# kcat/openal-soft

Hardware: AMD Instinct MI355X
Metric: mixed voices/sec @48kHz 1024-sample update, HRTF stereo; fraction of HBM roofline (higher is better)
Workload: dtype f32

## Files before the change

### include/oalgpu.h

```cpp
#ifndef OALGPU_H
#define OALGPU_H

#include <stddef.h>
#include <stdint.h>

#ifdef __cplusplus
extern "C" {
#endif
#if defined(__GNUC__)
#pragma GCC visibility push(default)
#endif

#define OALGPU_BUFFER_LINE_SIZE 1024
#define OALGPU_MAX_RESAMPLER_PADDING 48
#define OALGPU_MAX_RESAMPLER_EDGE 24
#define OALGPU_HRTF_HISTORY_LENGTH 64
#define OALGPU_HRIR_LENGTH 128
#define OALGPU_MAX_SENDS 6
#define OALGPU_MAX_OUTPUT_CHANNELS 32
#define OALGPU_MAX_AMBI_CHANNELS 25
#define OALGPU_MIXER_FRAC_BITS 16

typedef enum oalgpu_error {
    OALGPU_OK = 0,
// ... 23 lines not shown
typedef enum oalgpu_biquad_type {
    OALGPU_BIQUAD_HIGHSHELF, OALGPU_BIQUAD_LOWSHELF, OALGPU_BIQUAD_PEAKING, OALGPU_BIQUAD_LOWPASS,
    OALGPU_BIQUAD_HIGHPASS, OALGPU_BIQUAD_BANDPASS
} oalgpu_biquad_type;

typedef enum oalgpu_math_mode { OALGPU_MATH_EXACT = 0, OALGPU_MATH_FAST = 1 } oalgpu_math_mode;

const char *oalgpu_version(void);
const char *oalgpu_last_error(void);
int oalgpu_device_count(void);

typedef struct oalgpu_bsinc_table {
    float scaleBase, scaleRange;
    uint32_t m[16];
    uint32_t filterOffset[16];
    const float *tab;
    size_t tablen;
} oalgpu_bsinc_table;
int oalgpu_bsinc_table_get(int which , oalgpu_bsinc_table *out);
int oalgpu_cubic_table_get(int which , float *out);

typedef struct oalgpu_interp_state {
    int32_t kind;
    int32_t table;
    float sf;
    uint32_t m, l;
    uint32_t filter_offset;
} oalgpu_interp_state;
int oalgpu_prepare_resampler(int resampler, uint32_t increment, oalgpu_interp_state *out);

typedef struct oalgpu_biquad {
    float z1, z2;
    float b0, b1, b2, a1, a2;
    float tb0, tb1, tb2, ta1, ta2;
    int32_t counter;
} oalgpu_biquad;
void oalgpu_biquad_reset(oalgpu_biquad *f);
void oalgpu_biquad_set_params_from_slope(oalgpu_biquad *f, int type, float f0norm, float gain,
    float slope);

int oalgpu_resample(int device, int mode, int resampler, uint32_t increment, const float *src,
    size_t srclen, uint32_t frac, float *dst, size_t n);
int oalgpu_mix(int device, const float *in, size_t n, float *out, size_t nlines,
    float *current_gains, const float *target_gains, size_t counter, size_t outpos);
int oalgpu_mix_hrtf(int device, int mode, const float *in, float *accum, uint32_t irsize,
    const float *coeffs, const uint32_t delay[2], float gain, float gainstep, size_t n);
int oalgpu_mix_hrtf_blend(int device, int mode, const float *in, float *accum, uint32_t irsize,
    const float *oldcoeffs, const uint32_t olddelay[2], float oldgain, const float *newcoeffs,
    const uint32_t newdelay[2], float newgainstep, size_t n);
typedef struct oalgpu_splitter { float coeff, lp_z1, lp_z2, ap_z1; } oalgpu_splitter;
void oalgpu_splitter_init(oalgpu_splitter *s, float f0norm);
int oalgpu_mix_direct_hrtf(int device, int mode, float *left, float *right, const float *in,
    size_t nch, float *accum, oalgpu_splitter *splitters, const float *hfscales,
    const float *chan_coeffs, size_t irsize, size_t n);
int oalgpu_biquad_dual_process(int device, oalgpu_biquad *f0, oalgpu_biquad *f1, const float *src,
    float *dst, size_t n);

typedef struct oalgpu_context oalgpu_context;

typedef struct oalgpu_context_desc {
    int32_t  device;
    int32_t  math_mode;
    uint32_t sample_rate;
    uint32_t num_dry_channels;
    uint32_t num_real_channels;
    uint32_t num_aux_sends;
    uint32_t num_slots;
    uint32_t wet_channels;
    int32_t  hrtf;
    uint32_t max_voices;
    uint32_t max_buffers;
    uint32_t voices_per_group;
    uint32_t flags;
} oalgpu_context_desc;
#define OALGPU_CTX_FIR_VALU 1u
#define OALGPU_CTX_PROFILE  2u
#define OALGPU_CTX_STREAM_ROWS 8u
#define OALGPU_CTX_APPLY_IN_VOICE_KERNEL 16u
#define OALGPU_CTX_FUSED_REDUCE 32u
#define OALGPU_CTX_RESIDENT 64u
#define OALGPU_CTX_SLICE_LINES 128u
#define OALGPU_CTX_WAVE_PAIRS 256u
#define OALGPU_CTX_ROW_SLICES 512u
#define OALGPU_CTX_SERIAL   4u

int  oalgpu_context_create(const oalgpu_context_desc *desc, oalgpu_context **out);
void oalgpu_context_destroy(oalgpu_context *ctx);

int oalgpu_hrtf_load_mhr(oalgpu_context *ctx, const void *data, size_t size);
int oalgpu_hrtf_load_store(oalgpu_context *ctx, uint32_t sample_rate, uint32_t ir_size, const float *field_distance,
    const uint8_t *field_evcount, uint32_t num_fields, const uint16_t *elev_azcount, const uint16_t *elev_iroffset,
    uint32_t num_elevs, const float *coeffs, const uint8_t *delays, uint32_t num_irs);
typedef struct oalgpu_hrtf_info {
    uint32_t sample_rate, ir_size, num_fields, num_elevs, num_irs;
} oalgpu_hrtf_info;
int oalgpu_hrtf_info_get(oalgpu_context *ctx, oalgpu_hrtf_info *out);
int oalgpu_hrtf_raw(oalgpu_context *ctx, float *field_distance, uint8_t *field_evcount,
    uint16_t *elev_azcount, uint16_t *elev_iroffset, float *coeffs, uint8_t *delays);
int oalgpu_hrtf_get_coeffs(oalgpu_context *ctx, const float *dirs, size_t count, float *coeffs,
    uint32_t *delays);
int oalgpu_set_direct_hrtf(oalgpu_context *ctx, const float *chan_coeffs ,
    const float *hfscales, float xover_norm, uint32_t irsize);
int oalgpu_set_direct_hrtf_from_store(oalgpu_context *ctx, const float *points, const float *matrix, uint32_t num_points,
    const float *order_hf_gain, float xover_freq, uint32_t ir_size, int per_hrir_min);
int oalgpu_hrtf_parse_host(const void *mhr, size_t size, uint32_t device_rate, oalgpu_hrtf_info *info, float *coeffs, uint8_t *delays);
int oalgpu_hrtf_blend_host(const void *mhr, size_t size, uint32_t device_rate, const float *dirs, size_t count,
    uint32_t *idx, float *w, float *pass, uint32_t *delays);
int oalgpu_hrtf_build_direct_host(const void *mhr, size_t size, uint32_t device_rate, uint32_t ir_size, int per_hrir_min,
    const float *points, const float *matrix, uint32_t num_points, uint32_t num_chans, float xover_freq, const float *order_hf_gain,
    float *out_coeffs, float *out_hfscales, float *out_xover_norm, uint32_t *out_irsize);

int oalgpu_buffer_register(oalgpu_context *ctx, const void *data, int fmt_type,
    uint32_t frame_step, uint32_t sample_len, uint32_t loop_start, uint32_t loop_end);
int oalgpu_buffer_release(oalgpu_context *ctx, int buffer);
int oalgpu_buffer_info(oalgpu_context *ctx, int buffer, int32_t *live, int32_t *release_pending, uint32_t *references);

int oalgpu_buffer_channel_view(oalgpu_context *ctx, int buffer, uint32_t channel);

typedef struct oalgpu_voice_desc {
    int32_t  buffer;
    int32_t  looping;
    int32_t  position;
    uint32_t position_frac;
    uint32_t frequency;
} oalgpu_voice_desc;
int oalgpu_voice_init(oalgpu_context *ctx, uint32_t voice, const oalgpu_voice_desc *desc);
int oalgpu_context_set_nfc(oalgpu_context *ctx, float w1, const uint32_t channels_per_order[5]);
int oalgpu_voice_set_nfc(oalgpu_context *ctx, uint32_t voice, float w0);

int oalgpu_voice_set_ambi_scale(oalgpu_context *ctx, uint32_t voice, float xover_norm, float hf_scale,
    float lf_scale);

typedef struct oalgpu_filter_params {
    int32_t active;
    float gain_hf, hf_norm;
    float gain_lf, lf_norm;
} oalgpu_filter_params;

typedef struct oalgpu_voice_params {
    uint32_t step;
    int32_t  resampler;
    oalgpu_filter_params direct_filter;
    float    dry_gains[OALGPU_MAX_OUTPUT_CHANNELS];
    float    hrtf_ev, hrtf_az, hrtf_dist, hrtf_spread;
    float    hrtf_gain;
    int32_t  send_slot[OALGPU_MAX_SENDS];
    oalgpu_filter_params send_filter[OALGPU_MAX_SENDS];
    float    send_gains[OALGPU_MAX_SENDS][OALGPU_MAX_AMBI_CHANNELS];
} oalgpu_voice_params;
#define OALGPU_HRTF_KEEP_TARGET (-1.0f)
int oalgpu_voice_set_hrtf_targets(oalgpu_context *ctx, const uint32_t *voices, const float *coeffs, const uint32_t *delays,
    const float *gains, size_t count);

typedef struct oalgpu_voice_pan {
    float dir[3];
    float spread;
    float dry_gain;
    float send_gain[OALGPU_MAX_SENDS];
} oalgpu_voice_pan;
int oalgpu_context_set_ambi_map(oalgpu_context *ctx, const uint8_t *index, const float *scale);
int oalgpu_slot_set_ambi_map(oalgpu_context *ctx, uint32_t slot, const uint8_t *index, const float *scale);
int oalgpu_voice_set_pan(oalgpu_context *ctx, const uint32_t *voices, const oalgpu_voice_pan *pans, size_t count);

int oalgpu_buffer_queue_link(oalgpu_context *ctx, int buffer, int next_buffer);
int oalgpu_voice_init_queue(oalgpu_context *ctx, uint32_t voice, int first_buffer, int looping, int32_t position,
    uint32_t position_frac);
// ... 288 lines not shown
```

### openal-soft_amd/csrc/api.hip

```cpp
#include "api_context.hpp"
namespace oalgpu {

thread_local std::string gLastError;

int Fail(int code, const std::string &msg)
{
    gLastError = msg;
    return code;
}

void ParkResidentContexts(int device);

int UseDevice(int device)
{
    int count = 0;
    if(hipGetDeviceCount(&count) != hipSuccess || count <= 0)
        return Fail(OALGPU_ERR_NO_DEVICE, "no HIP device available (the product has no CPU path)");
    if(device < 0 || device >= count) return Fail(OALGPU_ERR_INVALID, "device ordinal out of range");
    HIP_TRY(hipSetDevice(device));
    ParkResidentContexts(device);
    return OALGPU_OK;
}

}
// ... 54 lines not shown
        cb.state = OALGPU_VOICE_STOPPED;
        cb.retired = true;
        c->cbOfVoice[voice] = -1;
    }
}

void NoteCallbackSteps(oalgpu_context *c, const uint32_t *voices, const oalgpu_voice_params *params, size_t count)
{
    if(c->cbVoices.empty()) return;
    for(size_t i = 0; i < count; ++i)
        if(voices[i] < c->cbOfVoice.size() && c->cbOfVoice[voices[i]] >= 0)
            c->cbVoices[size_t(c->cbOfVoice[voices[i]])].step = params[i].step;
}

int FlushInits(oalgpu_context *c)
{
    if(c->initPending.empty()) return OALGPU_OK;
    const size_t n = c->initPending.size();
    if(int rc = StageRecords(c->stream, c->initDev, c->initPending.data(), n)) return rc;
    LaunchInitVoices(c->stream, c->L, c->initDev.p, uint32_t(n));
    HIP_TRY(hipGetLastError());
    HIP_TRY(hipStreamSynchronize(c->stream));
    c->initPending.clear();
    return OALGPU_OK;
}

static void SetRowsGroups(oalgpu_context *c);

uint32_t DeviceComputeUnits(int device)
{
    hipDeviceProp_t prop{};
    if(hipGetDeviceProperties(&prop, device) == hipSuccess && prop.multiProcessorCount > 0) return uint32_t(prop.multiProcessorCount);
    (void)hipGetLastError();
    return 256u;
}

int oalgpu_context_create(const oalgpu_context_desc *desc, oalgpu_context **out)
{
    if(!desc || !out) return Fail(OALGPU_ERR_INVALID, "null argument");
    *out = nullptr;
    if(desc->max_voices == 0 || desc->num_dry_channels == 0 || desc->num_dry_channels > OALGPU_MAX_OUTPUT_CHANNELS
        || desc->num_aux_sends > OALGPU_MAX_SENDS || desc->wet_channels > OALGPU_MAX_AMBI_CHANNELS
        || (desc->num_aux_sends && (desc->num_slots == 0 || desc->wet_channels == 0)))
        return Fail(OALGPU_ERR_INVALID, "oalgpu_context_create: bad descriptor");
    const uint32_t mixLines = (desc->hrtf ? 0u : desc->num_dry_channels) + desc->num_slots * desc->wet_channels;
    if(mixLines > 32) return Fail(OALGPU_ERR_CAPACITY, "more than 32 mixing lines (dry + wet) are not supported yet");
    if(int rc = UseDevice(desc->device)) return rc;

    auto c = std::make_unique<oalgpu_context>();
    c->desc = *desc;
    c->exact = desc->math_mode == OALGPU_MATH_EXACT;
    int prioLeast = 0, prioGreatest = 0;
    HIP_TRY(hipDeviceGetStreamPriorityRange(&prioLeast, &prioGreatest));
    HIP_TRY(hipStreamCreateWithPriority(&c->stream, hipStreamDefault, prioGreatest));
    HIP_TRY(hipEventCreate(&c->evStart)); HIP_TRY(hipEventCreate(&c->evVoice)); HIP_TRY(hipEventCreate(&c->evEnd));
    HIP_TRY(hipStreamCreateWithPriority(&c->postStream, hipStreamDefault, prioLeast));
    for(hipEvent_t *e : {&c->evVoiceDone[0], &c->evVoiceDone[1], &c->evReduceDone[0], &c->evReduceDone[1], &c->evPostDone})
        HIP_TRY(hipEventCreateWithFlags(e, hipEventDisableTiming | hipEventDisableSystemFence));

    DeviceLayout &L = c->L;
    L.numVoices = desc->max_voices;
    L.numDry = desc->num_dry_channels; L.numReal = desc->num_real_channels;
    L.numSends = desc->num_aux_sends; L.numSlots = desc->num_slots; L.wetChannels = desc->wet_channels;
    L.hrtf = desc->hrtf ? 1u : 0u;
    L.irSize = 0; L.irStride = 8;
    L.mixLines = mixLines;
    c->slotConv.assign(desc->num_slots, nullptr);
    c->slotReverb.assign(desc->num_slots, nullptr);
    c->slotEffect.assign(desc->num_slots, nullptr);
    c->slotTarget.assign(desc->num_slots, -1);
    c->slotDepth.assign(desc->num_slots, 0u);
    c->slotOrder.resize(desc->num_slots);
    for(uint32_t i = 0; i < desc->num_slots; ++i) c->slotOrder[i] = i;
    HIP_TRY(c->reverbTicket.alloc(1)); HIP_TRY(c->reverbTicket.zero());
    uint32_t vpg = desc->voices_per_group;
    if(vpg == 0)
    {
        vpg = std::max<uint32_t>(2u, (desc->max_voices + 1023u) / 1024u);
    }
    L.voicesPerGroup = vpg;
    L.numGroups = std::max<uint32_t>(1u, (desc->max_voices + vpg - 1u) / vpg);
    L.waveVoices = 0;
    L.firMfma = (desc->flags & OALGPU_CTX_FIR_VALU) ? 0u : 1u;
    c->serialOnly = (desc->flags & OALGPU_CTX_SERIAL) != 0;
    c->res.enabled = (desc->flags & OALGPU_CTX_RESIDENT) != 0 && !(desc->flags & (OALGPU_CTX_PROFILE | OALGPU_CTX_SERIAL));
    c->useWave = WaveKernelApplies(c->exact, L);
    if(c->useWave)
    {
        L.waveVoices = desc->voices_per_group ? std::max<uint32_t>(1u, (desc->voices_per_group + 3u) / 4u)
            : std::max<uint32_t>(1u, (desc->max_voices + 2047u) / 2048u);
        L.numGroups = std::max<uint32_t>(1u, WaveKernelGroups(L));
    }
    const TableBlob &blob = Blob();
    HIP_TRY(c->tables.alloc(blob.data.size())); HIP_TRY(c->tables.upload(blob.data.data(), blob.data.size()));
    L.tables = c->tables.p;
    HIP_TRY(c->buffers.alloc(std::max<uint32_t>(desc->max_buffers, 1u))); HIP_TRY(c->buffers.zero());
    L.buffers = c->buffers.p;
    c->buf.reset(desc->max_buffers, desc->max_voices);
    c->cbOfVoice.assign(std::max<uint32_t>(desc->max_voices, 1u), -1);

    const size_t nv = desc->max_voices;
    HIP_TRY(c->ctl.alloc(nv)); HIP_TRY(c->ctl.zero()); L.ctl = c->ctl.p;
    HIP_TRY(c->prev.alloc(nv * kMaxPad)); HIP_TRY(c->prev.zero()); L.prev = c->prev.p;
    HIP_TRY(c->dfilt.alloc(nv * 2)); HIP_TRY(c->dfilt.zero()); L.dfilt = c->dfilt.p;
    HIP_TRY(c->hist.alloc(nv * kHist)); HIP_TRY(c->hist.zero()); L.hist = c->hist.p;
    HIP_TRY(c->gainCur.alloc(nv * L.numDry)); HIP_TRY(c->gainCur.zero()); L.gainCur = c->gainCur.p;
    HIP_TRY(c->gainTgt.alloc(nv * L.numDry)); HIP_TRY(c->gainTgt.zero()); L.gainTgt = c->gainTgt.p;
    HIP_TRY(c->sfilt.alloc(nv * L.numSends * 2)); HIP_TRY(c->sfilt.zero()); L.sfilt = c->sfilt.p;
    HIP_TRY(c->sendCur.alloc(nv * L.numSends * L.wetChannels)); HIP_TRY(c->sendCur.zero()); L.sendCur = c->sendCur.p;
    HIP_TRY(c->sendTgt.alloc(nv * L.numSends * L.wetChannels)); HIP_TRY(c->sendTgt.zero()); L.sendTgt = c->sendTgt.p;
    HIP_TRY(c->ambi.alloc(nv)); HIP_TRY(c->ambi.zero()); L.ambi = c->ambi.p;
    HIP_TRY(c->startDelay.alloc(nv)); HIP_TRY(c->startDelay.zero()); L.startDelay = c->startDelay.p;
    {
        std::vector<AmbiMapEntry> ident(std::max<size_t>(L.numDry, size_t{L.numSlots} * L.wetChannels) + 1);
        for(size_t i = 0; i < ident.size(); ++i) ident[i] = AmbiMapEntry{uint32_t(i < OALGPU_MAX_AMBI_CHANNELS ? i : 0), 1.0f};
        HIP_TRY(c->dryMap.alloc(L.numDry)); HIP_TRY(c->dryMap.upload(ident.data(), L.numDry));
        HIP_TRY(c->wetMaps.alloc(size_t{L.numSlots} * L.wetChannels));
        for(uint32_t s = 0; s < L.numSlots; ++s)
            HIP_TRY(hipMemcpy(c->wetMaps.p + size_t{s} * L.wetChannels, ident.data(), L.wetChannels * sizeof(AmbiMapEntry), hipMemcpyHostToDevice));
    }
    HIP_TRY(c->queueDone.alloc(nv)); HIP_TRY(c->queueDone.zero()); L.queueDone = c->queueDone.p;
    L.numLineGroups = L.numGroups;
    c->groupsAllocated = L.numGroups;
    if(c->useWave && L.hrtf && L.firMfma && !(desc->flags & OALGPU_CTX_WAVE_PAIRS))
    {
        const uint32_t w = Wave16WavesFor(desc->max_voices, DeviceComputeUnits(desc->device));
        c->groupsAllocated = std::max<uint32_t>(c->groupsAllocated, (desc->max_voices + w - 1u) / w);
    }
    L.streams = nullptr; L.lineGains = nullptr; L.lineStride = 0; L.streamsPerVoice = 0;
    L.nfc = nullptr; L.nfcOrders = 0;
    L.hrirs = nullptr;
    for(uint32_t &n : L.chansPerOrder) n = 0;
    L.accLines = 0;
    L.wave16 = 0;
    L.rows8 = 0; L.rowsVpg = 0;
    if(c->useWave && !(desc->flags & OALGPU_CTX_STREAM_ROWS))
    {
        L.accLines = WaveKernelAccLines(L);
        if(!L.accLines && RowsKernelApplies(L))
            L.rows8 = 1;
    }
    if(c->useWave && (!L.hrtf || L.numSends))
    {
        L.lineStride = L.mixLines <= 8 ? 8u : (L.mixLines <= 16 ? 16u : 32u);
        L.streamsPerVoice = 2u + L.numSends;
    }
    if(c->useWave && (!L.hrtf || L.numSends) && !L.accLines && !L.rows8) { if(int rc = AllocStreamRows(c.get())) return rc; }
    const size_t groups = c->groupsAllocated;
    HIP_TRY(c->partLines.alloc(groups * L.mixLines * kLine)); L.partLines = c->partLines.p;
    HIP_TRY(c->partLines2.alloc(c->useWave && (L.streams || L.accLines || L.rows8) ? groups * L.mixLines * kLine : 0));
    c->partLinesBuf[0] = c->partLines.p; c->partLinesBuf[1] = c->partLines2.p;
    HIP_TRY(c->partHrtf.alloc(L.hrtf ? groups * (kLine + kHrirLen) * 2 : 0)); L.partHrtf = c->partHrtf.p;
    HIP_TRY(c->partHrtf2.alloc(c->useWave && L.hrtf ? groups * (kLine + kHrirLen) * 2 : 0));
    c->partHrtfBuf[0] = c->partHrtf.p; c->partHrtfBuf[1] = c->partHrtf2.p;
    HIP_TRY(c->bus.alloc(BusFloats(L))); HIP_TRY(c->bus.zero()); L.bus = c->bus.p;
    if(desc->flags & OALGPU_CTX_PROFILE)
    {
        HIP_TRY(c->phaseTimes.alloc(nv * 16)); HIP_TRY(c->phaseTimes.zero());
        c->prof.times = c->phaseTimes.p;
    }
    L.hrtfOld = nullptr; L.hrtfTgt = nullptr;

    HIP_TRY(c->dSplit.alloc(L.numDry)); HIP_TRY(c->dSplit.zero());
    HIP_TRY(c->dSplit2.alloc(L.numDry)); HIP_TRY(c->dSplit2.zero());
    HIP_TRY(c->carryBuf.alloc(size_t{kLine + kHrirLen} * 2)); HIP_TRY(c->carryBuf.zero());
    HIP_TRY(c->postArrived.alloc(1)); HIP_TRY(c->postArrived.zero());
    HIP_TRY(c->dHfScale.alloc(L.numDry)); HIP_TRY(c->dHfScale.zero());
    HIP_TRY(c->dCoeffs.alloc(size_t{L.numDry} * kHrirLen * 2)); HIP_TRY(c->dCoeffs.zero());
    HIP_TRY(c->dTemp.alloc(size_t{L.numDry} * kLine + (kLine + kHrirLen) * 2));
    if(L.rows8) SetRowsGroups(c.get());
    *out = c.release();
    return OALGPU_OK;
}

static void DetachForDestroy(oalgpu_context *ctx);

void oalgpu_context_destroy(oalgpu_context *ctx)
{
    if(!ctx) return;
    (void)UseDevice(ctx->desc.device);
    if(ctx->attachedTo || !ctx->attached.empty()) DetachForDestroy(ctx);
    if(ctx->res.pendingBlock) { ctx->res.pendingBlock->heldBy = nullptr; ctx->res.pendingBlock = nullptr; }
    (void)FlushPendingMix(ctx);
    (void)hipStreamSynchronize(ctx->stream);
    if(ctx->res.reduceStream) (void)hipStreamSynchronize(ctx->res.reduceStream);
    if(ctx->postStream) (void)hipStreamSynchronize(ctx->postStream);
    delete ctx->comm;
    for(auto &cb : ctx->cbVoices)
        for(int k = 0; k < 2; ++k)
        {
            if(cb.pinned[k]) (void)hipHostFree(cb.pinned[k]);
            if(cb.copied[k]) (void)hipEventDestroy(cb.copied[k]);
        }
    delete ctx;
}

int AllocStreamRows(oalgpu_context *c)
{
    DeviceLayout &L = c->L;
    const size_t nv = L.numVoices;
    HIP_TRY(c->streams.alloc(nv * L.streamsPerVoice * kLine)); HIP_TRY(c->streams.zero()); L.streams = c->streams.p;
    HIP_TRY(c->lineGains.alloc(nv * L.streamsPerVoice * LineBlockDwords(L.lineStride))); HIP_TRY(c->lineGains.zero());
    L.lineGains = c->lineGains.p;
    return OALGPU_OK;
}

static float *SlotWetBus(const DeviceLayout &L, uint32_t slot) { return L.bus + BusWetOffset(L) + size_t{slot} * L.wetChannels * kLine; }
static float *SlotDestination(const oalgpu_context *c, uint32_t slot)
{
    const int32_t target = c->slotTarget[slot];
    return target >= 0 ? SlotWetBus(c->L, uint32_t(target)) : c->L.bus;
}
static int RunEffects(oalgpu_context *c, hipStream_t s, uint32_t samples_to_do)
{
    const DeviceLayout &L = c->L;
    for(uint32_t first = 0; first < L.numSlots; )
    {
        const uint32_t depth = c->slotDepth[c->slotOrder[first]];
        uint32_t last = first;
        while(last < L.numSlots && c->slotDepth[c->slotOrder[last]] == depth) ++last;
        for(uint32_t i = first; i < last; ++i)
        {
            const uint32_t slot = c->slotOrder[i];
            const float *wet = SlotWetBus(L, slot);
            if(oalgpu_convolution *conv = c->slotConv[slot])
            {
                if(int rc = oalgpu_convolution_process_device(conv, s, wet, SlotDestination(c, slot), samples_to_do)) return rc;
            }
            if(oalgpu_effect *fx = c->slotEffect[slot])
            {
                if(int rc = oalgpu_effect_process_device(fx, s, wet, SlotDestination(c, slot), samples_to_do)) return rc;
            }
        }
        oalgpu_reverb *revs[kRvBatchMax];
        const float *wets[kRvBatchMax];
        float *outs[kRvBatchMax];
        uint32_t count = 0;
        auto flush = [&]() -> int
        {
            if(!count) return OALGPU_OK;
            const int rc = oalgpu_reverb_process_batch_device(revs, wets, count, outs, samples_to_do, s, c->reverbTicket.p);
            count = 0;
            return rc;
        };
// ... 926 lines not shown
```

### openal-soft_amd/csrc/api_context.hpp

```cpp
#pragma once
#include "../../include/oalgpu.h"
#ifdef OALGPU_MEASUREMENT
#include "../../tools/measure/oalgpu_measure.h"
#endif

#include <hip/hip_runtime.h>
#include <hip/hip_ext.h>
#include <rccl/rccl.h>
#include <dlfcn.h>
#include <fcntl.h>
#include <sys/mman.h>
#include <sys/stat.h>
#include <unistd.h>

#include <algorithm>
#include <atomic>
#include <chrono>
#include <functional>
#include <thread>
#include <cstdio>
#include <cstdlib>
#include <cstring>
#include <memory>
#include <mutex>
// ... 38 lines not shown
    }
    uint32_t filterBase(const oalgpu_interp_state &st) const
    {
        switch(st.kind)
        {
        case 2: return cubicBase[st.table ? 1 : 0];
        case 3: case 4: return bsincBase[st.table == 12 ? 0 : st.table == 24 ? 1 : 2] + st.filter_offset;
        default: return 0;
        }
    }
};
inline const TableBlob &Blob() { static const TableBlob b; return b; }

}

enum class PostKind : uint32_t { None, AmbiDec, Stabilizer, Bs2b, Uhj, Tsme };

struct BusTransport;
struct oalgpu_context {
    oalgpu_context_desc desc{};
    bool exact{true};
    hipStream_t stream{nullptr};
    bool ownStream{true};
    hipEvent_t evStart{nullptr}, evVoice{nullptr}, evEnd{nullptr};
    hipStream_t postStream{nullptr};
    hipEvent_t evVoiceDone[2]{nullptr, nullptr}, evReduceDone[2]{nullptr, nullptr}, evPostDone{nullptr};
    uint32_t parity{0};
    bool postPending{false};
    struct { bool active{false}; uint32_t samples{0}; int post{0}; } pendingMix;
    static constexpr uint32_t kIoSlots = 4;
    oalgpu_voice_move *panHost[kIoSlots]{};
    size_t panCap{0};
    hipEvent_t panApplied[kIoSlots]{};
    uint32_t panNext{0};
    float *outHost[kIoSlots]{};
    hipEvent_t outDone[kIoSlots]{};
    uint32_t outNext{0};
    size_t outFloats{0};
    bool panInBar{false};
    static constexpr uint32_t kEvCap = 1024;
    uint32_t *evHost[kIoSlots]{};
    hipEvent_t evDone[kIoSlots]{};
    uint32_t evNext{0};
    DevBuf<uint32_t> evSnapshot, evCounters;
    bool outRing{false}, outRingWritten{false};
    bool outViaRing[kIoSlots]{};
    uint32_t outSeq{0}, outSlotSeq[kIoSlots]{};
    uint32_t outArrivedTotal{0};
    bool fuseReduce{false}, reduceHeld{false};
    DeviceLayout heldL{};
    uint32_t heldParity{0};
    DevBuf<uint32_t> reducedCount;
    uint32_t reducedEpoch{0};
    hipEvent_t lastPostEvent{nullptr};
    uint64_t updatesSubmitted{0}, updatesKnownDone{0};
    uint64_t reduceUpdate[2]{0, 0}, panUpdate[kIoSlots]{}, outUpdate[kIoSlots]{};
    uint32_t *outFlags{nullptr};
    DevBuf<uint32_t> outArrived;
    float *partHrtfBuf[2]{nullptr, nullptr};
    float *partLinesBuf[2]{nullptr, nullptr};
    bool timing{false}, timed{false};
    DeviceLayout L{};
    HrtfStoreDev hrtfDev{};
    HrtfData hrtfHost;
    bool hrtfLoaded{false};
    uint32_t hrtfGeneration{0};
    bool carryAccum{true};
    bool useWave{false};
    uint32_t groupsAllocated{0};
    std::vector<oalgpu_convolution*> slotConv;
    std::vector<oalgpu_reverb*> slotReverb;
    std::vector<oalgpu_effect*> slotEffect;
    DevBuf<uint32_t> reverbTicket;
    std::vector<int32_t> slotTarget;
    std::vector<uint32_t> slotOrder, slotDepth;

    DevBuf<float> tables;
    DevBuf<BufferItem> buffers;
    DevBuf<uint32_t> startDelay;
    DevBuf<uint32_t> queueDone;
    BufferTable buf;
    DevBuf<VoiceCtl> ctl;
    DevBuf<float> prev, hrtfOld, hrtfTgt, hist, gainCur, gainTgt, sendCur, sendTgt;
    DevBuf<BiquadSlot> dfilt, sfilt;
    DevBuf<float> partLines, partLines2, partHrtf, partHrtf2, bus, streams;
    DevBuf<uint32_t> lineGains;
    DevBuf<AmbiScaleState> ambi;
    DevBuf<NfcState> nfc;
    NfcDesign nfcDevice{};
    DevBuf<unsigned long long> phaseTimes;
    WaveProf prof{nullptr, 0u};
    const WaveProf *profArg() const { return prof.times ? &prof : nullptr; }
    DevBuf<AmbiMapEntry> dryMap, wetMaps;
    DevBuf<PanRecord> panRecs;
    std::vector<VoiceCtl> ctlHost;
    std::vector<uint32_t> doneHost;
    DevBuf<TargetRecord> tgtRecs;
    DevBuf<float> tgtCoeffs;
    bool serialOnly{false};
    struct BusTransport *comm{nullptr};
    int commRank{0}, commWorld{1};
    oalgpu_context *attachedTo{nullptr};
    std::vector<int32_t> attachMap;
    hipEvent_t evBusFinal{nullptr};
    std::vector<oalgpu_context*> attached;
    DevBuf<BusMergeHead> mergeHeads;
    DevBuf<BusMergeRow> mergeRows;
    uint32_t mergeLines{0};
    hipEvent_t evMerged{nullptr};
    bool mergeInFlight{false};
    PostKind post{PostKind::None};
    bool decDual{false};
    uint32_t decOut{0};
    DevBuf<float> decGainsHf, decGainsLf, decBands;
    DevBuf<SplitterState> decSplit;
    int outType{6};
    float ditherDepth{0.0f};
    uint32_t ditherSeed{22222};
    bool limOn{false};
    LimiterConsts lim{};
    DevBuf<float> limState;
    int encQuality{-1};
    DevBuf<float> encTaps, encState;
    uint32_t stabLeft{0}, stabRight{0}, stabCenter{0};
    StabilizerConsts stab{};
    DevBuf<float> stabState;
    uint32_t cfLeft{0}, cfRight{0};
    CrossfeedConsts cf{};
    DevBuf<float> cfState;
    uint32_t distLines{0};
    DevBuf<uint32_t> distDelays;
    DevBuf<float> distGains, distHist;
    DevBuf<unsigned char> pcm;
    DevBuf<float> hFieldDist, hCoeffs;
    DevBuf<uint8_t> hEvCount, hDelays;
    DevBuf<uint16_t> hAzCount, hIrOffset;
    DevBuf<SplitterState> dSplit, dSplit2;
    uint32_t dSplitCur{0};
    DevBuf<float> carryBuf;
    float dSplitCoeff{0.0f};
    float runPower[4]{1.0f, 0.0f, 1.0f, 1.0f};
    uint32_t runPowerSeg{0};
    DevBuf<uint32_t> postArrived;
    uint32_t postEpoch{0};
    const ParamRecord *nextRecs{nullptr};
    const int32_t *nextMap{nullptr};
    const float *nextRows{nullptr};
    bool carryInBuf{false};
    DevBuf<float> dHfScale, dCoeffs, dTemp;
    uint32_t dIrSize{0};
    bool directSet{false};
    DevBuf<ParamRecord> paramDev;
    std::vector<ParamRecord> paramHost;
    DevBuf<VoiceInitRecord> initDev;
    std::vector<VoiceInitRecord> initPending;
    struct CbVoice {
        uint32_t voice{0}; int32_t buffer{-1}; uint32_t frameBytes{4}, capacityFrames{0};
        oalgpu_callback_fn fn{nullptr}; void *user{nullptr};
        std::vector<char> data;
        uint32_t numBlocks{0}, blockOffset{0};
        bool stopped{false};
        int32_t position{0}; uint32_t frac{0}, step{0};
        int state{OALGPU_VOICE_PLAYING}; bool hasBuffer{true};
        char *pinned[2]{nullptr, nullptr}; hipEvent_t copied[2]{nullptr, nullptr}; uint32_t slot{0};
        size_t allocBytes{0};
        bool retired{false};
// ... 115 lines not shown
```

### openal-soft_amd/csrc/api_hrtf.hip

```cpp
#include "api_context.hpp"

static uint32_t ChooseWave16(const oalgpu_context *c, const DeviceLayout &T)
{
    const bool want16 = !(c->desc.flags & OALGPU_CTX_WAVE_PAIRS) && Wave16Applies(T)
        && (T.numSends == 0 || !(c->desc.flags & (OALGPU_CTX_STREAM_ROWS | OALGPU_CTX_PROFILE)));
    if(!want16) return 0u;
    if(!c->desc.voices_per_group) return Wave16WavesFor(T.numVoices, DeviceComputeUnits(c->desc.device));
    for(uint32_t w : {4u, 8u, 16u})
        if((T.numVoices + w - 1u) / w <= c->groupsAllocated) return w;
    return 0u;
}

static int InstallHrtfData(oalgpu_context *c, HrtfData &&parsed)
{
    if(parsed.sampleRate != c->desc.sample_rate) ResampleHrtfData(parsed, c->desc.sample_rate);
    DeviceLayout T = c->L;
    T.irSize = parsed.irSize;
    T.irStride = (parsed.irSize + 15u) & ~15u;
    const bool toStreamRows = T.accLines && WaveKernelAccLines(T) == 0;
    if(toStreamRows) T.accLines = 0;
    if(c->useWave)
    {
        T.wave16 = ChooseWave16(c, T);
        if(std::max<uint32_t>(1u, WaveKernelGroups(T)) > c->groupsAllocated)
            return Fail(OALGPU_ERR_INVALID, "internal: the voice kernel's grid outgrew the partial buses");
    }
    if(int rc = oalgpu_sync(c)) return rc;
    c->hrtfHost = std::move(parsed);
    const HrtfData &h = c->hrtfHost;
    HIP_TRY(c->hFieldDist.alloc(h.fieldDistance.size())); HIP_TRY(c->hFieldDist.upload(h.fieldDistance.data(), h.fieldDistance.size()));
    HIP_TRY(c->hEvCount.alloc(h.fieldEvCount.size())); HIP_TRY(c->hEvCount.upload(h.fieldEvCount.data(), h.fieldEvCount.size()));
    HIP_TRY(c->hAzCount.alloc(h.elevAzCount.size())); HIP_TRY(c->hAzCount.upload(h.elevAzCount.data(), h.elevAzCount.size()));
    HIP_TRY(c->hIrOffset.alloc(h.elevIrOffset.size())); HIP_TRY(c->hIrOffset.upload(h.elevIrOffset.data(), h.elevIrOffset.size()));
    HIP_TRY(c->hCoeffs.alloc(h.coeffs.size())); HIP_TRY(c->hCoeffs.upload(h.coeffs.data(), h.coeffs.size()));
    HIP_TRY(c->hDelays.alloc(h.delays.size())); HIP_TRY(c->hDelays.upload(h.delays.data(), h.delays.size()));
    HrtfStoreDev &d = c->hrtfDev;
    d.irSize = h.irSize; d.numFields = uint32_t(h.fieldDistance.size()); d.numElevs = uint32_t(h.elevAzCount.size());
    d.numIrs = h.numIrs();
    d.fieldDistance = c->hFieldDist.p; d.fieldEvCount = c->hEvCount.p; d.elevAzCount = c->hAzCount.p;
    d.elevIrOffset = c->hIrOffset.p; d.coeffs = c->hCoeffs.p; d.delays = c->hDelays.p;
    c->hrtfLoaded = true;
    ++c->hrtfGeneration;

    DeviceLayout &L = c->L;
    L.hrirs = c->hCoeffs.p;
    L.irSize = h.irSize;
    L.irStride = T.irStride;
    if(L.hrtf)
    {
        const size_t n = size_t{L.numVoices} * L.irStride * 2;
        HIP_TRY(c->hrtfOld.alloc(n)); HIP_TRY(c->hrtfOld.zero()); L.hrtfOld = c->hrtfOld.p;
        HIP_TRY(c->hrtfTgt.alloc(n)); HIP_TRY(c->hrtfTgt.zero()); L.hrtfTgt = c->hrtfTgt.p;
        if(!c->directSet) c->dIrSize = h.irSize;
    }
    if(toStreamRows)
    {
        L.accLines = 0;
        if(int rc = AllocStreamRows(c)) return rc;
    }
    if(c->useWave)
    {
        L.wave16 = T.wave16;
        if(L.wave16 && L.numSends)
        {
            L.accLines = 0;
            if(!L.streams) { if(int rc = AllocStreamRows(c)) return rc; }
        }
        const uint32_t groups = std::max<uint32_t>(1u, WaveKernelGroups(L));
        L.numGroups = groups; L.numLineGroups = groups;
        if(L.wave16 && (L.wave16 != 16u || L.numSends)) c->res.enabled = false;
    }
    return OALGPU_OK;
}

int oalgpu_hrtf_load_mhr(oalgpu_context *c, const void *data, size_t size)
{
    if(!c || !data) return Fail(OALGPU_ERR_INVALID, "null argument");
    if(int rc = UseCtx(c)) return rc;
    HrtfData parsed;
    const std::string err = ParseMhr(data, size, parsed);
    if(!err.empty()) return Fail(OALGPU_ERR_INVALID, "mhr: " + err);
    return InstallHrtfData(c, std::move(parsed));
}

int oalgpu_hrtf_load_store(oalgpu_context *c, uint32_t sample_rate, uint32_t ir_size, const float *field_distance,
    const uint8_t *field_evcount, uint32_t num_fields, const uint16_t *elev_azcount, const uint16_t *elev_iroffset,
    uint32_t num_elevs, const float *coeffs, const uint8_t *delays, uint32_t num_irs)
{
    if(!c || !field_distance || !field_evcount || !elev_azcount || !elev_iroffset || !coeffs || !delays)
        return Fail(OALGPU_ERR_INVALID, "null argument");
    if(sample_rate == 0 || ir_size < 8 || ir_size > kHrirLen || num_fields == 0 || num_elevs == 0 || num_irs == 0)
        return Fail(OALGPU_ERR_INVALID, "oalgpu_hrtf_load_store: bad sizes");
    uint32_t evs = 0;
    for(uint32_t f = 0; f < num_fields; ++f)
    {
        if(field_evcount[f] < 2) return Fail(OALGPU_ERR_INVALID, "oalgpu_hrtf_load_store: a field needs at least two elevations");
        evs += field_evcount[f];
    }
    if(evs != num_elevs) return Fail(OALGPU_ERR_INVALID, "oalgpu_hrtf_load_store: the fields' elevation counts do not add up to num_elevs");
    for(uint32_t e = 0; e < num_elevs; ++e)
        if(elev_azcount[e] == 0 || uint32_t(elev_iroffset[e]) + elev_azcount[e] > num_irs)
            return Fail(OALGPU_ERR_INVALID, "oalgpu_hrtf_load_store: an elevation's HRIRs lie outside the store");
    if(int rc = UseCtx(c)) return rc;
    HrtfData h;
    h.sampleRate = sample_rate; h.irSize = ir_size;
    h.fieldDistance.assign(field_distance, field_distance + num_fields);
    h.fieldEvCount.assign(field_evcount, field_evcount + num_fields);
    h.elevAzCount.assign(elev_azcount, elev_azcount + num_elevs);
    h.elevIrOffset.assign(elev_iroffset, elev_iroffset + num_elevs);
    h.coeffs.assign(coeffs, coeffs + size_t{num_irs} * kHrirLen * 2);
    h.delays.assign(delays, delays + size_t{num_irs} * 2);
    return InstallHrtfData(c, std::move(h));
}

int oalgpu_hrtf_info_get(oalgpu_context *c, oalgpu_hrtf_info *out)
{
    if(!c || !out) return Fail(OALGPU_ERR_INVALID, "null argument");
    if(!c->hrtfLoaded) return Fail(OALGPU_ERR_NO_HRTF, "no HRTF data set loaded");
    const HrtfData &h = c->hrtfHost;
    out->sample_rate = h.sampleRate; out->ir_size = h.irSize;
    out->num_fields = uint32_t(h.fieldDistance.size()); out->num_elevs = uint32_t(h.elevAzCount.size());
    out->num_irs = h.numIrs();
    return OALGPU_OK;
}

int oalgpu_hrtf_raw(oalgpu_context *c, float *field_distance, uint8_t *field_evcount, uint16_t *elev_azcount,
    uint16_t *elev_iroffset, float *coeffs, uint8_t *delays)
{
    if(!c) return Fail(OALGPU_ERR_INVALID, "null argument");
    if(!c->hrtfLoaded) return Fail(OALGPU_ERR_NO_HRTF, "no HRTF data set loaded");
    const HrtfData &h = c->hrtfHost;
    std::copy(h.fieldDistance.begin(), h.fieldDistance.end(), field_distance);
    std::copy(h.fieldEvCount.begin(), h.fieldEvCount.end(), field_evcount);
    std::copy(h.elevAzCount.begin(), h.elevAzCount.end(), elev_azcount);
    std::copy(h.elevIrOffset.begin(), h.elevIrOffset.end(), elev_iroffset);
// ... 125 lines not shown
```

### openal-soft_amd/csrc/api_voices.hip

```cpp
#include "api_context.hpp"

int BeginVoiceCall(oalgpu_context *c, bool argsOk, const char *who, bool sync)
{
    if(!argsOk) return Fail(OALGPU_ERR_INVALID, std::string(who) + ": bad arguments");
    if(int rc = UseCtx(c)) return rc;
    if(int rc = FlushInits(c)) return rc;
    return sync ? oalgpu_sync(c) : OALGPU_OK;
}

void PendStart(oalgpu_context *c, const VoiceInitRecord &rec)
{
    auto &p = c->initPending;
    p.erase(std::remove_if(p.begin(), p.end(), [&](const VoiceInitRecord &r) { return r.voice == rec.voice; }), p.end());
    p.push_back(rec);
}

static int StartVoice(oalgpu_context *c, const char *who, bool queue, uint32_t voice, int buffer, int looping, int32_t position,
    uint32_t position_frac)
{
    if(c) { if(int rc = FlushPendingMix(c)) return rc; }
    if(c && c->res.pendingBlock) { if(int rc = UseCtx(c)) return rc; }
    if(!VoiceOk(c, voice) || !c->buf.usable(buffer) || position_frac >= kFracOne)
        return Fail(OALGPU_ERR_INVALID, std::string(who) + ": bad arguments");
    if(c->L.hrtf && !c->hrtfLoaded) return Fail(OALGPU_ERR_NO_HRTF, "HRTF context without a data set");
// ... 151 lines not shown
            std::memcpy(r.sendGains[s], p.send_gains[s], sizeof(r.sendGains[s]));
        }
        r.hrtfDir[0] = p.hrtf_ev; r.hrtfDir[1] = p.hrtf_az; r.hrtfDir[2] = p.hrtf_dist; r.hrtfDir[3] = p.hrtf_spread;
        r.hrtfGain = p.hrtf_gain;
        if(c->L.hrtf && p.hrtf_dist < 0.0f && p.hrtf_dist != OALGPU_HRTF_KEEP_TARGET)
            return Fail(OALGPU_ERR_INVALID, "voice parameters: hrtf_dist < 0 is reserved (OALGPU_HRTF_KEEP_TARGET = -1)");
        r.keepHrtf = (c->L.hrtf && p.hrtf_dist == OALGPU_HRTF_KEEP_TARGET) ? 1u : 0u;
        if(c->L.hrtf && c->hrtfLoaded && !r.keepHrtf)
        {
            const HrirBlend b = HrtfBlendFor(hostStore, p.hrtf_ev, p.hrtf_az, p.hrtf_dist, p.hrtf_spread);
            for(int k = 0; k < 4; ++k) { r.hrtfIdx[k] = b.idx[k]; r.hrtfW[k] = b.w[k]; }
            r.hrtfPass = b.passthru;
            r.hrtfDelay[0] = b.delay[0]; r.hrtfDelay[1] = b.delay[1];
        }
        std::memcpy(r.dryGains, p.dry_gains, sizeof(r.dryGains));
    }
    return OALGPU_OK;
}

int oalgpu_voice_set_params(oalgpu_context *c, const uint32_t *voices, const oalgpu_voice_params *params, size_t count)
{
    if(!c || !voices || !params) return Fail(OALGPU_ERR_INVALID, "null argument");
    if(count == 0) return OALGPU_OK;
    if(c->L.hrtf && !c->hrtfLoaded) return Fail(OALGPU_ERR_NO_HRTF, "HRTF context without a data set");
    if(int rc = BeginVoiceCall(c)) return rc;
    if(int rc = BuildParamRecords(c, voices, params, count, c->paramHost)) return rc;
    NoteCallbackSteps(c, voices, params, count);
    if(int rc = StageRecords(c->stream, c->paramDev, c->paramHost.data(), count)) return rc;
    LaunchApplyParams(c->stream, c->L, c->paramDev.p, uint32_t(count));
    HIP_TRY(hipGetLastError());
    HIP_TRY(hipStreamSynchronize(c->stream));
    return OALGPU_OK;
}

int oalgpu_voice_set_hrtf_targets(oalgpu_context *c, const uint32_t *voices, const float *coeffs, const uint32_t *delays,
    const float *gains, size_t count)
{
    if(!c || !voices || !coeffs || !delays || !gains) return Fail(OALGPU_ERR_INVALID, "null argument");
    if(count == 0) return OALGPU_OK;
    if(!c->L.hrtf) return Fail(OALGPU_ERR_INVALID, "oalgpu_voice_set_hrtf_targets: HRTF contexts only");
    if(!c->hrtfLoaded) return Fail(OALGPU_ERR_NO_HRTF, "HRTF context without a data set");
    if(int rc = BeginVoiceCall(c)) return rc;
    std::vector<TargetRecord> recs(count);
    for(size_t i = 0; i < count; ++i)
    {
        if(voices[i] >= c->L.numVoices || delays[2 * i] > 63u || delays[2 * i + 1] > 63u)
            return Fail(OALGPU_ERR_INVALID, "oalgpu_voice_set_hrtf_targets: bad voice index or delay (MaxHrirDelay = 63)");
        recs[i] = TargetRecord{voices[i], {delays[2 * i], delays[2 * i + 1]}, gains[i]};
    }
    if(int rc = StageRecords(c->stream, c->tgtRecs, recs.data(), count)) return rc;
    if(int rc = StageRecords(c->stream, c->tgtCoeffs, coeffs, count * kHrirLen * 2)) return rc;
    LaunchApplyTargets(c->stream, c->L, c->tgtRecs.p, c->tgtCoeffs.p, uint32_t(count));
    HIP_TRY(hipGetLastError());
    HIP_TRY(hipStreamSynchronize(c->stream));
    return OALGPU_OK;
}

int oalgpu_param_block_create(oalgpu_context *c, const uint32_t *voices, const oalgpu_voice_params *params,
    size_t count, oalgpu_param_block **out)
{
    if(!c || !voices || !params || !out || count == 0) return Fail(OALGPU_ERR_INVALID, "oalgpu_param_block_create: bad arguments");
    *out = nullptr;
    if(c->L.hrtf && !c->hrtfLoaded) return Fail(OALGPU_ERR_NO_HRTF, "oalgpu_param_block_create: HRTF context without a data set");
    if(int rc = UseCtx(c)) return rc;
    std::vector<ParamRecord> recs;
    if(int rc = BuildParamRecords(c, voices, params, count, recs)) return rc;
    auto b = std::make_unique<oalgpu_param_block>();
    b->count = uint32_t(count);
    b->device = c->desc.device;
    b->hrtfGeneration = c->hrtfGeneration;
    HIP_TRY(b->recs.alloc(count));
    HIP_TRY(b->recs.upload(recs.data(), count));
    {
        std::vector<int32_t> map(c->L.numVoices, -1);
        bool unique = true;
        for(size_t i = 0; i < count; ++i) { unique = unique && map[voices[i]] < 0; map[voices[i]] = int32_t(i); }
        if(unique)
        {
            HIP_TRY(b->voiceToRec.alloc(map.size()));
            HIP_TRY(b->voiceToRec.upload(map.data(), map.size()));
            b->mapVoices = uint32_t(map.size());
            if((c->res.enabled || (c->desc.flags & OALGPU_CTX_APPLY_IN_VOICE_KERNEL)) && c->L.hrtf && c->L.hrirs && c->L.irStride <= 64u)
            {
                HIP_TRY(b->rows.alloc(count * size_t{c->L.irStride} * 2));
                HIP_TRY(b->rows.zero());
                LaunchBlendRows(c->stream, c->L, b->recs.p, uint32_t(count), b->rows.p);
                HIP_TRY(hipGetLastError());
                HIP_TRY(hipStreamSynchronize(c->stream));
            }
        }
    }
    for(size_t i = 0; i < count; ++i)
        if(c->cbOfVoice[voices[i]] >= 0) b->cbSteps.emplace_back(voices[i], params[i].step);
    *out = b.release();
    return OALGPU_OK;
}

int oalgpu_param_block_apply(oalgpu_context *c, oalgpu_param_block *b)
{
    if(!c || !b) return Fail(OALGPU_ERR_INVALID, "null argument");
    if(c->L.hrtf && !c->hrtfLoaded) return Fail(OALGPU_ERR_NO_HRTF, "HRTF context without a data set");
    if(c->L.hrtf && b->hrtfGeneration != c->hrtfGeneration)
        return Fail(OALGPU_ERR_INVALID, "oalgpu_param_block_apply: the block was built against another HRTF data set (its HRIR indices are that store's); create it again");
    if(!c->res.cooldown && ResidentWanted(c, 1) && !c->res.pendingBlock && b->mapVoices == c->L.numVoices && b->cbSteps.empty() && b->rows.p)
    {
        c->res.pendingBlock = b;
        b->heldBy = c;
        return OALGPU_OK;
    }
    if(c->pendingMix.active && b->mapVoices == c->L.numVoices && WaveKernelAppliesRecords(c->L) && c->initPending.empty())
    {
        if(int rc = UseDevice(c->desc.device)) return rc;
        if(int rc = FlushPendingMix(c, b)) return rc;
    }
    else
    {
    if(int rc = BeginVoiceCall(c)) return rc;
    LaunchApplyParams(c->stream, c->L, b->recs.p, b->count);
    HIP_TRY(hipGetLastError());
    }
    for(const auto &vs : b->cbSteps)
        if(vs.first < c->cbOfVoice.size() && c->cbOfVoice[vs.first] >= 0) c->cbVoices[size_t(c->cbOfVoice[vs.first])].step = vs.second;
    return OALGPU_OK;
}

void oalgpu_param_block_destroy(oalgpu_param_block *b)
{
    if(!b) return;
    (void)UseDevice(b->device);
    if(b->heldBy && b->heldBy->res.pendingBlock == b) (void)FlushResidentBlock(b->heldBy);
    delete b;
}

namespace {
__global__ void ProbeReadKernel(const uint32_t *src, uint32_t *dst, uint32_t n)
{
    const uint32_t i = threadIdx.x;
    if(i < n) dst[i] = src[i] + __hip_atomic_load(src + i, __ATOMIC_RELAXED, __HIP_MEMORY_SCOPE_SYSTEM);
}
bool HostCanTouch(void *p, size_t bytes)
{
    int fd[2];
    if(pipe(fd) != 0) return false;
    bool ok = write(fd[1], p, bytes) == ssize_t(bytes);
    if(ok) ok = read(fd[0], p, bytes) == ssize_t(bytes);
    close(fd[0]); close(fd[1]);
    return ok;
}
}
bool HostStoresReachDevice(oalgpu_context *c)
{
    hipDeviceProp_t prop{};
    if(hipGetDeviceProperties(&prop, c->desc.device) != hipSuccess || !prop.isLargeBar) return false;
    uint32_t *probe = nullptr, *seen = nullptr;
    if(hipExtMallocWithFlags(reinterpret_cast<void**>(&probe), 256, hipDeviceMallocFinegrained) != hipSuccess) { (void)hipGetLastError(); return false; }
    if(hipMalloc(reinterpret_cast<void**>(&seen), 256) != hipSuccess) { (void)hipGetLastError(); (void)hipFree(probe); return false; }
    bool ok = HostCanTouch(probe, 256);
    for(uint32_t round = 0; ok && round < 2; ++round)
    {
        const uint32_t pat = round ? 0xc0de0000u : 0x5eed0000u;
        for(uint32_t i = 0; i < 64; ++i) probe[i] = pat + i;
        __builtin_ia32_sfence();
        uint32_t back[64] = {};
        hipLaunchKernelGGL(ProbeReadKernel, dim3(1), dim3(64), 0, c->stream, probe, seen, 64u);
        if(hipGetLastError() != hipSuccess || hipMemcpyAsync(back, seen, sizeof(back), hipMemcpyDeviceToHost, c->stream) != hipSuccess
            || hipStreamSynchronize(c->stream) != hipSuccess) { (void)hipGetLastError(); ok = false; }
        for(uint32_t i = 0; ok && i < 64; ++i) ok = back[i] == 2u * (pat + i);
// ... 104 lines not shown
```

### openal-soft_amd/csrc/dev_wave.hpp

```cpp
#pragma once
#include "kernels.hpp"

#pragma clang fp contract(off)

namespace oalgpu {

typedef float f2 __attribute__((ext_vector_type(2)));
typedef const f2 __attribute__((address_space(4))) cf2;
typedef const uint32_t __attribute__((address_space(4))) cu32;
typedef float f16 __attribute__((ext_vector_type(16)));
typedef const f16 __attribute__((address_space(4))) cf16;

#if defined(__HIP_DEVICE_COMPILE__)
#define OALGPU_SINGLE_DS_OPS __attribute__((target("no-load-store-opt")))
#else
#define OALGPU_SINGLE_DS_OPS
#endif

__device__ __forceinline__ f2 pkfma(f2 a, f2 b, f2 c) { return __builtin_elementwise_fma(a, b, c); }
__device__ __forceinline__ f2 splat(float v) { f2 r = {v, v}; return r; }

__device__ __forceinline__ void WaveSync()
{
    __builtin_amdgcn_fence(__ATOMIC_RELEASE, "wavefront");
    __builtin_amdgcn_wave_barrier();
    __builtin_amdgcn_fence(__ATOMIC_ACQUIRE, "wavefront");
}

typedef uint32_t u4 __attribute__((ext_vector_type(4)));
typedef const u4 __attribute__((address_space(4))) cu4;

__device__ __forceinline__ VoiceCtl LoadCtlScalar(const VoiceCtl *p)
{
    union { VoiceCtl c; u4 q[sizeof(VoiceCtl) / 16]; } u;
    cu4 *src = (cu4*)(uintptr_t)p;
#pragma unroll
    for(size_t k = 0; k < sizeof(VoiceCtl) / 16; ++k) u.q[k] = src[k];
    return u.c;
}


struct Sp3 { float a, b, c; };

template<bool HFONLY>
__device__ __forceinline__ float SplitStep(Sp3 &s, float x, float apCoeff, float lpCoeff, float hf, float lf)
{
    const float d0 = (x - s.a) * lpCoeff;
    const float lpY0 = s.a + d0;
    s.a = HFONLY ? __builtin_fmaf(d0, lpCoeff, lpY0) : lpY0 + d0;
    const float d1 = (lpY0 - s.b) * lpCoeff;
    const float lpY1 = s.b + d1;
    s.b = lpY1 + d1;
    const float apY = __builtin_fmaf(x, apCoeff, s.c);
    s.c = __builtin_fmaf(-apY, apCoeff, x);
    return __builtin_fmaf(apY - lpY1, hf, HFONLY ? lpY1 : lpY1 * lf);
}

struct Mat3 { Sp3 c0, c1, c2; };
__device__ __forceinline__ Sp3 MatVec3(const Mat3 &m, const Sp3 &v)
{
    Sp3 r;
    r.a = __builtin_fmaf(m.c2.a, v.c, __builtin_fmaf(m.c1.a, v.b, m.c0.a * v.a));
    r.b = __builtin_fmaf(m.c2.b, v.c, __builtin_fmaf(m.c1.b, v.b, m.c0.b * v.a));
    r.c = __builtin_fmaf(m.c2.c, v.c, __builtin_fmaf(m.c1.c, v.b, m.c0.c * v.a));
    return r;
}
__device__ __forceinline__ Mat3 MatMul3(const Mat3 &a, const Mat3 &b)
{ return Mat3{MatVec3(a, b.c0), MatVec3(a, b.c1), MatVec3(a, b.c2)}; }

template<bool HFONLY>
__device__ __forceinline__ void SplitterScan(SplitterState &st, float *buf, uint32_t n, float hf, float lf, uint32_t lane)
{
    const float apCoeff = st.coeff, lpCoeff = st.coeff * 0.5f + 0.5f;
    const uint32_t seg = ((n + 63u) / 64u) | 1u;
    const uint32_t begin = lane * seg < n ? lane * seg : n;
    const uint32_t end = (begin + seg < n) ? begin + seg : n;
    Mat3 M{{1, 0, 0}, {0, 1, 0}, {0, 0, 1}};
    for(uint32_t i = 0; i < seg; ++i)
    {
        SplitStep<HFONLY>(M.c0, 0.0f, apCoeff, lpCoeff, hf, lf); SplitStep<HFONLY>(M.c1, 0.0f, apCoeff, lpCoeff, hf, lf);
        SplitStep<HFONLY>(M.c2, 0.0f, apCoeff, lpCoeff, hf, lf);
    }
    Sp3 q{0, 0, 0};
    for(uint32_t i = begin; i < end; ++i) SplitStep<HFONLY>(q, buf[i], apCoeff, lpCoeff, hf, lf);
    Sp3 e = q;
    Sp3 s0{st.lpZ1, st.lpZ2, st.apZ1};
    Mat3 P = M;
#pragma unroll
    for(int step = 0; step < 6; ++step)
    {
        const int d = 1 << step;
        Sp3 o;
        o.a = __shfl_up(e.a, d); o.b = __shfl_up(e.b, d); o.c = __shfl_up(e.c, d);
        const Sp3 mo = MatVec3(P, o);
        if(int(lane) >= d) { e.a += mo.a; e.b += mo.b; e.c += mo.c; }
        const Sp3 ms = MatVec3(P, s0);
        if(lane & uint32_t(d)) s0 = ms;
        if(step < 5) P = MatMul3(P, P);
    }
    Sp3 prevE;
    prevE.a = __shfl_up(e.a, 1); prevE.b = __shfl_up(e.b, 1); prevE.c = __shfl_up(e.c, 1);
    Sp3 start = s0;
    if(lane > 0) { start.a += prevE.a; start.b += prevE.b; start.c += prevE.c; }
    for(uint32_t i = begin; i < end; ++i) buf[i] = SplitStep<HFONLY>(start, buf[i], apCoeff, lpCoeff, hf, lf);
    const int lastLane = int((n - 1u) / seg);
    st.lpZ1 = __shfl(start.a, lastLane); st.lpZ2 = __shfl(start.b, lastLane); st.apZ1 = __shfl(start.c, lastLane);
}

struct Tri3 { float p, q, r, s; };
__device__ __forceinline__ Sp3 TriVec(const Tri3 &m, const Sp3 &v)
{ return Sp3{m.p * v.a, __builtin_fmaf(m.q, v.a, m.r * v.b), m.s * v.c}; }
// ... 90 lines not shown
    st.apZ1 = __builtin_bit_cast(float, __builtin_amdgcn_readlane(__builtin_bit_cast(int, start.c), lastLane));
}

template<int R, int TAPS, typename X>
__device__ __forceinline__ void FirMainPk(f2 (&acc)[R], const X *xw, cf16 *co16)
{
    static_assert(TAPS % 8 == 0, "taps come in blocks of 8");
    X w[R + 3];
#pragma unroll
    for(int k = 0; k < R + 3; ++k) w[k] = xw[k - 3];
    X wn[4];
#pragma unroll
    for(int k = 0; k < 4; ++k) wn[k] = (TAPS > 4) ? xw[-4 - 3 + k] : w[k];
    f16 cnext = co16[0];
#pragma unroll
    for(int b8 = 0; b8 < TAPS / 8; ++b8)
    {
        const f16 c16 = cnext;
        if(b8 + 1 < TAPS / 8) cnext = co16[b8 + 1];
#pragma unroll
        for(int h = 0; h < 2; ++h)
        {
            const int b = 2 * b8 + h;
            X wnn[4];
#pragma unroll
            for(int k = 0; k < 4; ++k) wnn[k] = (b + 2 < TAPS / 4) ? xw[-4 * (b + 2) - 3 + k] : wn[k];
#pragma unroll
            for(int jj = 0; jj < 4; ++jj)
            {
                const f2 c = {c16[(4 * h + jj) * 2], c16[(4 * h + jj) * 2 + 1]};
#pragma unroll
                for(int r = 0; r < R; ++r)
                {
                    if constexpr(sizeof(X) == sizeof(f2)) acc[r] = pkfma(c, w[r + 3 - jj], acc[r]);
                    else acc[r] = pkfma(c, splat(w[r + 3 - jj]), acc[r]);
                }
            }
            if(b + 1 < TAPS / 4)
            {
#pragma unroll
                for(int k = R + 2; k >= 4; --k) w[k] = w[k - 4];
#pragma unroll
                for(int k = 0; k < 4; ++k) { w[k] = wn[k]; wn[k] = wnn[k]; }
            }
        }
    }
}

typedef float f4 __attribute__((ext_vector_type(4)));
typedef _Float16 h8 __attribute__((ext_vector_type(8)));

constexpr int kXhHalves = 64 + 1024 + 80;
constexpr int kXhDw = kXhHalves / 2;
constexpr int kHrHalves = 120;
constexpr int kHrDw = kHrHalves / 2;
static_assert(kXhDw % 4 == 0 && kHrDw % 4 == 0, "16-byte rows");

__device__ __forceinline__ void HalfScale(uint32_t maxBits, float &scale, float &inv)
{
    int32_t sb = 268 - int32_t(maxBits >> 23);
    sb = sb < 67 ? 67 : (sb > 187 ? 187 : sb);
    scale = __builtin_bit_cast(float, uint32_t(sb) << 23);
    inv = __builtin_bit_cast(float, uint32_t(254 - sb) << 23);
}
__device__ __forceinline__ void SplitHalf2(float v0, float v1, uint32_t &hi, uint32_t &lo)
{
    const auto h = __builtin_amdgcn_cvt_pkrtz(v0, v1);
    hi = __builtin_bit_cast(uint32_t, h);
    lo = __builtin_bit_cast(uint32_t, __builtin_amdgcn_cvt_pkrtz(__builtin_fmaf(float(h[0]), -1.0f, v0), __builtin_fmaf(float(h[1]), -1.0f, v1)));
}
__device__ __forceinline__ uint32_t WaveMaxBits(uint32_t v)
{
#define OALGPU_DPP_MAX(ctrl) do { const uint32_t o = uint32_t(__builtin_amdgcn_update_dpp(0, int(v), ctrl, 0xF, 0xF, true)); v = o > v ? o : v; } while(0)
    OALGPU_DPP_MAX(0xB1);
    OALGPU_DPP_MAX(0x4E);
    OALGPU_DPP_MAX(0x141);
    OALGPU_DPP_MAX(0x140);
#undef OALGPU_DPP_MAX
    const uint32_t a = uint32_t(__builtin_amdgcn_readlane(int(v), 0)), b = uint32_t(__builtin_amdgcn_readlane(int(v), 16));
    const uint32_t c = uint32_t(__builtin_amdgcn_readlane(int(v), 32)), d = uint32_t(__builtin_amdgcn_readlane(int(v), 48));
    const uint32_t ab = a > b ? a : b, cd = c > d ? c : d;
    return ab > cd ? ab : cd;
}

constexpr int kBqSeg = 17;
struct S2 { float a, b; };

__device__ __forceinline__ float BqStep(S2 &s, float x, float b0, float b1, float b2, float a1, float a2)
{
    const float y = __builtin_fmaf(x, b0, s.a);
    s.a = __builtin_fmaf(x, b1, __builtin_fmaf(-y, a1, s.b));
    s.b = __builtin_fmaf(x, b2, -y * a2);
    return y;
}
__device__ __forceinline__ S2 Mv2(S2 c0, S2 c1, S2 v)
{ return S2{__builtin_fmaf(c1.a, v.b, c0.a * v.a), __builtin_fmaf(c1.b, v.b, c0.b * v.a)}; }

__device__ __forceinline__ float DppRowShr(float v, int d)
{
    const int x = __builtin_bit_cast(int, v);
    int r;
    switch(d)
    {
    case 1: r = __builtin_amdgcn_update_dpp(0, x, 0x111, 0xF, 0xF, true); break;
    case 2: r = __builtin_amdgcn_update_dpp(0, x, 0x112, 0xF, 0xF, true); break;
    case 4: r = __builtin_amdgcn_update_dpp(0, x, 0x114, 0xF, 0xF, true); break;
    default: r = __builtin_amdgcn_update_dpp(0, x, 0x118, 0xF, 0xF, true); break;
    }
    return __builtin_bit_cast(float, r);
}
__device__ __forceinline__ float DppRowShrF(float v, int d) { return DppRowShr(v, d); }
__device__ __forceinline__ S2 ScanLinear2Row(S2 e, S2 m0, S2 m1, uint32_t lane, S2 &q0, S2 &q1)
{
    S2 p0 = m0, p1 = m1;
    q0 = S2{1.0f, 0.0f}; q1 = S2{0.0f, 1.0f};
    const uint32_t exp = (lane & 15u) + 1u;
#pragma unroll
    for(int step = 0; step < 4; ++step)
    {
        const int d = 1 << step;
        const S2 o{DppRowShr(e.a, d), DppRowShr(e.b, d)};
        const S2 mo = Mv2(p0, p1, o);
        e.a += mo.a; e.b += mo.b;
        const S2 r0 = Mv2(p0, p1, q0), r1 = Mv2(p0, p1, q1);
        if(exp & uint32_t(d)) { q0 = r0; q1 = r1; }
        const S2 n0 = Mv2(p0, p1, p0), n1 = Mv2(p0, p1, p1); p0 = n0; p1 = n1;
    }
    if(exp == 16u) { q0 = p0; q1 = p1; }
    return e;
}
__device__ __forceinline__ S2 ScanLinear2(S2 e, S2 m0, S2 m1, uint32_t lane)
{
    S2 q0, q1;
    e = ScanLinear2Row(e, m0, m1, lane, q0, q1);
#pragma unroll
    for(int r = 1; r < 4; ++r)
    {
        const S2 c{__builtin_bit_cast(float, __builtin_amdgcn_readlane(__builtin_bit_cast(int, e.a), 16 * r - 1)),
            __builtin_bit_cast(float, __builtin_amdgcn_readlane(__builtin_bit_cast(int, e.b), 16 * r - 1))};
        const S2 mc = Mv2(q0, q1, c);
        if((lane >> 4) == uint32_t(r)) { e.a += mc.a; e.b += mc.b; }
    }
    return e;
}


template<int TILES = 5, bool LOW8 = false, bool AHEAD = true>
__device__ __forceinline__ void FirMfmaH(f4 (&acc)[2][5], const uint32_t (&xh)[2][2][kXhDw], const uint32_t (&hr)[2][2][kHrDw],
    float inv, uint32_t lane)
{
    const uint32_t i = lane & 15u, g = lane >> 4;
    const uint32_t u0 = 16u - i + 8u * g, shift = (u0 & 1u) * 2u, ud = u0 >> 1;
    const f4 vinv = {inv, inv, inv, inv};
#pragma unroll
    for(int e = 0; e < 2; ++e)
    {
        if constexpr (!AHEAD) __builtin_amdgcn_sched_barrier(0);
        h8 A[2][3];
#pragma unroll
        for(int s = 0; s < 2; ++s)
#pragma unroll
            for(int c = 0; c < 3; ++c)
            {
                const uint32_t *p = hr[e][s] + ud + 16 * c;
                const uint32_t q0 = p[0], q1 = p[1], q2 = p[2], q3 = p[3], q4 = p[4];
                const u4 q = {__builtin_amdgcn_alignbyte(q1, q0, shift), __builtin_amdgcn_alignbyte(q2, q1, shift),
// ... 51 lines not shown
```

### openal-soft_amd/csrc/kernels.hpp

```cpp
#pragma once
#include <hip/hip_runtime.h>
#include <stdint.h>

#include "dev_hrtf.hpp"
#include "dev_mix.hpp"
#include "dev_resample.hpp"
#include "dev_voice.hpp"
#include "../host/limiter_params.hpp"
#include "../host/uhj_params.hpp"
#include "../host/stabilizer_params.hpp"
#include "../host/crossfeed_params.hpp"

namespace oalgpu {

enum VoiceFlagBits : uint32_t {
    kFlagFading = 1u << 0,
    kFlagHasHrtf = 1u << 1,
    kFlagDirectFilter = 1u << 2,
    kFlagHrtfDirty = 1u << 3,
    kFlagAmbiScale = 1u << 4,
    kFlagNfc = 1u << 5,
    kFlagQueue = 1u << 7,
    kFlagDelayed = 1u << 6,
    kFlagSendFilterShift = 8
};

struct alignas(16) VoiceCtl {
    int32_t playState;
    int32_t position;
    uint32_t positionFrac;
    int32_t curBuffer;
    int32_t loopBuffer;
    uint32_t step;
    int32_t rsKind;
    uint32_t rsM, rsL;
    float rsSf;
    uint32_t rsFilterOffset;
    uint32_t flags;
    int32_t sendSlot[6];
    uint32_t hrtfOldDelay[2];
    float hrtfOldGain;
    uint32_t hrtfTgtDelay[2];
    float hrtfTgtGain;
    BufferItem buf;
};
static_assert(sizeof(VoiceCtl) == 128, "VoiceCtl is one 128-byte line");

struct alignas(16) AmbiScaleState { float coeff, lpZ1, lpZ2, apZ1, hfScale, lfScale; uint32_t pad[2]; };

struct alignas(16) NfcState { float a[5][5], b[5][5], z[5][4]; uint32_t pad[10]; };
static_assert(sizeof(NfcState) == 320, "NfcState");

struct alignas(16) BiquadSlot { BiquadState f; uint32_t pad[3]; };
static_assert(sizeof(BiquadSlot) == 64, "BiquadSlot");

__host__ __device__ inline uint32_t LineBlockDwords(uint32_t lineStride) { return 3u * lineStride + 8u; }

struct ParamRecord {
    uint32_t voice;
    uint32_t step;
    int32_t rsKind;
    uint32_t rsM, rsL;
    float rsSf;
    uint32_t rsFilterOffset;
    uint32_t flags;
    int32_t sendSlot[6];
    float dirLp[5], dirHp[5];
    float sendLp[6][5], sendHp[6][5];
    float hrtfDir[4];
    float hrtfGain;
    float dryGains[32];
    float sendGains[6][25];
    uint32_t hrtfIdx[4];
    float hrtfW[4];
    float hrtfPass;
    uint32_t hrtfDelay[2];
    uint32_t keepHrtf;
};

struct DeviceLayout {
    uint32_t numVoices, numDry, numReal, numSends, numSlots, wetChannels;
    uint32_t hrtf, irSize, irStride;
    uint32_t voicesPerGroup, numGroups;
    uint32_t waveVoices;
    uint32_t firMfma;
    uint32_t mixLines;
    uint32_t accLines;
    uint32_t rows8, rowsVpg;
    uint32_t wave16;
    const float *tables;
    const BufferItem *buffers;
    VoiceCtl *ctl;
    float *prev;
    BiquadSlot *dfilt;
    float *hrtfOld, *hrtfTgt, *hist;
    float *gainCur, *gainTgt;
    BiquadSlot *sfilt;
    float *sendCur, *sendTgt;
    AmbiScaleState *ambi;
    uint32_t *startDelay;
    uint32_t *queueDone;
    NfcState *nfc;
    uint32_t chansPerOrder[5];
    uint32_t nfcOrders;
    float *partLines, *partHrtf;
    float *streams;
    uint32_t *lineGains;
    uint32_t numLineGroups;
    uint32_t lineStride;
    uint32_t streamsPerVoice;
    float *bus;
    const float *hrirs;
};

__host__ __device__ inline size_t BusWetOffset(const DeviceLayout &L) { return size_t{L.numDry + L.numReal} * kLine; }
__host__ __device__ inline size_t BusAccumOffset(const DeviceLayout &L)
{ return BusWetOffset(L) + size_t{L.numSlots} * L.wetChannels * kLine; }
__host__ __device__ inline size_t BusFloats(const DeviceLayout &L)
{ return BusAccumOffset(L) + size_t{kLine + kHrirLen} * 2; }

__device__ __forceinline__ void ApplyHrtfTargetWave(const DeviceLayout &L, uint32_t v, const uint32_t (&idx)[4], const float (&w)[4],
    float pass, uint32_t lane)
{
    const uint32_t i0 = idx[0], i1 = idx[1], i2 = idx[2], i3 = idx[3];
    const float w0 = w[0], w1 = w[1], w2 = w[2], w3 = w[3];
    const uint32_t live = ((L.irSize + 1u) & ~1u) * 2u;
    for(uint32_t e = lane; e < L.irStride * 2; e += 64)
    {
        float x = (e < 2) ? pass : 0.0f;
        x = L.hrirs[size_t{i0} * (kHrirLen * 2) + e] * w0 + x;
        x = L.hrirs[size_t{i1} * (kHrirLen * 2) + e] * w1 + x;
        x = L.hrirs[size_t{i2} * (kHrirLen * 2) + e] * w2 + x;
        x = L.hrirs[size_t{i3} * (kHrirLen * 2) + e] * w3 + x;
        __builtin_nontemporal_store((e < live) ? x : 0.0f, &L.hrtfTgt[size_t{v} * L.irStride * 2 + e]);
    }
}

__device__ __forceinline__ void ApplyRecordWave(const DeviceLayout &L, const ParamRecord &r, uint32_t lane)
{
    const uint32_t v = r.voice;
    VoiceCtl &ctl = L.ctl[v];
    if(lane == 0)
    {
        ctl.step = r.step;
        ctl.rsKind = r.rsKind; ctl.rsM = r.rsM; ctl.rsL = r.rsL; ctl.rsSf = r.rsSf;
        ctl.rsFilterOffset = r.rsFilterOffset;
        const uint32_t keep = ctl.flags & (kFlagFading | kFlagHasHrtf | kFlagAmbiScale | kFlagNfc | kFlagDelayed | kFlagQueue
            | (r.keepHrtf ? uint32_t(kFlagHrtfDirty) : 0u));
        ctl.flags = keep | (r.flags & ~(kFlagFading | kFlagHasHrtf | kFlagHrtfDirty | kFlagAmbiScale | kFlagNfc | kFlagDelayed | kFlagQueue))
            | (L.hrtf ? (kFlagHasHrtf | (r.keepHrtf ? 0u : uint32_t(kFlagHrtfDirty))) : 0u);
        for(int i = 0; i < 6; ++i) ctl.sendSlot[i] = (uint32_t(i) < L.numSends) ? r.sendSlot[i] : -1;
        if(L.hrtf && !r.keepHrtf)
        {
            ctl.hrtfTgtDelay[0] = r.hrtfDelay[0]; ctl.hrtfTgtDelay[1] = r.hrtfDelay[1];
            ctl.hrtfTgtGain = r.hrtfGain;
        }
    }
    if(lane == 1) BiquadSetTarget(L.dfilt[size_t{v} * 2 + 0].f, r.dirLp);
    if(lane == 2) BiquadSetTarget(L.dfilt[size_t{v} * 2 + 1].f, r.dirHp);
    if(lane >= 8 && lane < 8 + 2 * L.numSends)
    {
        const uint32_t i = (lane - 8) >> 1, hp = (lane - 8) & 1u;
        BiquadSetTarget(L.sfilt[(size_t{v} * L.numSends + i) * 2 + hp].f, hp ? r.sendHp[i] : r.sendLp[i]);
    }
    if(L.hrtf) { if(!r.keepHrtf) ApplyHrtfTargetWave(L, v, r.hrtfIdx, r.hrtfW, r.hrtfPass, lane); }
    else if(lane < L.numDry)
        L.gainTgt[size_t{v} * L.numDry + lane] = r.dryGains[lane];
    for(uint32_t k = lane; k < L.numSends * L.wetChannels; k += 64)
        L.sendTgt[size_t{v} * L.numSends * L.wetChannels + k] = r.sendGains[k / L.wetChannels][k % L.wetChannels];
}

struct VoiceInitRecord { uint32_t voice; int32_t buffer, looping, position; uint32_t positionFrac; int32_t queue; };

constexpr uint32_t kResidentSets = 4;
constexpr uint32_t kResidentSlots = 16;
constexpr uint32_t kResidentDepth = 8;
constexpr unsigned long long kResidentWatchdogTicks = 200000000ull;

struct ResidentSlot { unsigned long long recs, map, rows; uint32_t samples, pad; };
struct alignas(64) ResidentDoor {
    uint32_t seq;
    uint32_t exitSeq[4];
    uint32_t pad[11];
    ResidentSlot slot[kResidentSlots];
};
enum ResidentCounter : uint32_t {
    kRcArrive0 = 0,
    kRcRedRead = 4,
    kRcRedDone = 5,
    kRcPostDone = 6,
    kRcStarted = 7,
    kRcWaitDoor = 8,
    kRcWaitRed = 9,
    kRcWaitArrive = 10,
    kRcWaitPost = 11,
    kRcWaitRedDone = 12,
    kRcWaitSplit = 13,
    kRcInstall = 14,
    kRcBusy = 15,
    kRcTop = 16,
    kRcCount = 17
};
enum ResidentHostFlag : uint32_t { kRhResident = 0, kRhError = 1, kRhProgress = 2,
    kRhFault = 3,
    kRhCount = 4 };
struct ResidentArgs {
    const ResidentDoor *door;
    uint32_t *counters;
    uint32_t *hostFlags;
    float *partBase;
    uint32_t setStride;
    uint32_t base, endSeq;
    uint32_t redPerUpdate;
    uint32_t startedTarget, launchId;
};

void LaunchResample(hipStream_t s, bool exact, const ResampleSpec &spec, const float *src, uint32_t frac,
    uint32_t increment, float *dst, uint32_t n);
// ... 188 lines not shown
```

### openal-soft_amd/csrc/voice_kernel.hip

```cpp
#include <hip/hip_ext.h>
#include "kernels.hpp"

#pragma clang fp contract(off)

namespace oalgpu {
namespace {

constexpr int kThreads = 256;
constexpr int kWaves = kThreads / 64;
constexpr int kInLen = kHist + kLine;
constexpr int kXPad = 128;
constexpr int kXLen = kXPad + kLine + kXPad;
constexpr int kXOldLen = kXPad + 256;
constexpr int kTabFloats = 3328;

struct alignas(16) SharedMem {
    float rdata[kResampleDataSize + 8];
    float in[kInLen];
    float filt[kWaves][kInLen];
    float xl[kXLen], xr[kXLen];
    float xol[kXOldLen], xor_[kXOldLen];
    float tab[kTabFloats];
    float coT[kHrirLen * 2], coO[kHrirLen * 2];
    float gCur[7][32], gTgt[7][32];
    int32_t sendSlot[8];
    int32_t best;
};

}

__global__ void __launch_bounds__(64) ApplyParamsKernel(DeviceLayout L, const ParamRecord *__restrict__ recs)
{
    ApplyRecordWave(L, recs[blockIdx.x], threadIdx.x);
}

__global__ void SetAmbiScaleKernel(DeviceLayout L, uint32_t v, AmbiScaleState st)
{
    L.ambi[v] = st;
    L.ctl[v].flags |= kFlagAmbiScale;
}

__global__ void SetStartDelayKernel(DeviceLayout L, uint32_t v, uint32_t samples)
{
    L.startDelay[v] = samples;
    if(samples) L.ctl[v].flags |= kFlagDelayed;
    else L.ctl[v].flags &= ~kFlagDelayed;
}

__global__ void SetVoiceWindowKernel(DeviceLayout L, uint32_t v, int32_t buffer, uint32_t sampleLen, int32_t position)
{
    const_cast<BufferItem*>(L.buffers)[buffer].sampleLen = sampleLen;
    L.ctl[v].buf.sampleLen = sampleLen;
    L.ctl[v].position = position;
}

void LaunchSetVoiceWindow(hipStream_t s, const DeviceLayout &L, uint32_t voice, int32_t buffer, uint32_t sampleLen, int32_t position)
{ hipLaunchKernelGGL(SetVoiceWindowKernel, dim3(1), dim3(1), 0, s, L, voice, buffer, sampleLen, position); }

__global__ void __launch_bounds__(256) VoiceEventsKernel(DeviceLayout L, uint32_t *snapshot, uint32_t *hostSlot, uint32_t capacity, uint32_t *counters)
{
    const uint32_t v = blockIdx.x * 256u + threadIdx.x;
    if(v < L.numVoices)
    {
        const VoiceCtl &c = L.ctl[v];
        const uint32_t st = uint32_t(c.playState), cb = uint32_t(c.curBuffer), qd = L.queueDone[v];
        uint32_t *snap = snapshot + size_t{v} * 3;
        if(snap[0] != st || snap[1] != cb || snap[2] != qd)
        {
            const bool started = st == uint32_t(OALGPU_VOICE_PLAYING) && int32_t(cb) >= 0 && snap[0] != uint32_t(OALGPU_VOICE_PLAYING);
            const bool idle = st == uint32_t(OALGPU_VOICE_STOPPED) && snap[0] == uint32_t(OALGPU_VOICE_STOPPED);
            snap[0] = st; snap[1] = cb; snap[2] = qd;
            const uint32_t idx = (started || idle) ? 0xffffffffu : atomicAdd(&counters[0], 1u);
            if(idx < capacity)
            {
                uint32_t *e = hostSlot + 4u + size_t{idx} * 8u;
                e[0] = v; e[1] = st; e[2] = cb; e[3] = qd; e[4] = uint32_t(c.position); e[5] = c.positionFrac;
                e[6] = (c.flags & kFlagFading) ? 1u : 0u; e[7] = 0u;
            }
        }
    }
    __syncthreads();
    if(threadIdx.x == 0)
    {
        __threadfence_system();
        const uint32_t done = atomicAdd(&counters[1], 1u);
        if(done + 1u == gridDim.x)
        {
            const uint32_t n = atomicExch(&counters[0], 0u);
            counters[1] = 0u;
            hostSlot[0] = n;
            __threadfence_system();
        }
    }
}

void LaunchVoiceEvents(hipStream_t s, const DeviceLayout &L, uint32_t *snapshot, uint32_t *hostSlot, uint32_t capacity, uint32_t *counters)
{
    hipLaunchKernelGGL(VoiceEventsKernel, dim3((L.numVoices + 255u) / 256u), dim3(256), 0, s, L, snapshot, hostSlot, capacity, counters);
}

void LaunchSetStartDelay(hipStream_t s, const DeviceLayout &L, uint32_t voice, uint32_t samples)
{ hipLaunchKernelGGL(SetStartDelayKernel, dim3(1), dim3(1), 0, s, L, voice, samples); }

void LaunchSetAmbiScale(hipStream_t s, const DeviceLayout &L, uint32_t voice, const AmbiScaleState &st)
{ hipLaunchKernelGGL(SetAmbiScaleKernel, dim3(1), dim3(1), 0, s, L, voice, st); }

__global__ void SetNfcKernel(DeviceLayout L, uint32_t v, NfcState st)
{
    const uint32_t t = threadIdx.x;
    float *dst = reinterpret_cast<float*>(&L.nfc[v]);
    const float *src = reinterpret_cast<const float*>(&st);
    if(t < 50) dst[t] = src[t];
    if(t == 0) L.ctl[v].flags |= kFlagNfc;
}

void LaunchSetNfc(hipStream_t s, const DeviceLayout &L, uint32_t voice, const NfcState &coeffs)
{ hipLaunchKernelGGL(SetNfcKernel, dim3(1), dim3(64), 0, s, L, voice, coeffs); }

__global__ void __launch_bounds__(64) InitVoicesKernel(DeviceLayout L, const VoiceInitRecord *__restrict__ recs)
{
    const VoiceInitRecord r = recs[blockIdx.x];
    const uint32_t v = r.voice, t = threadIdx.x;
    BiquadState def{};
    def.b0 = 1.0f; def.tb0 = 1.0f; def.counter = -1;
    if(t == 0)
    {
        VoiceCtl c{};
        c.playState = OALGPU_VOICE_PLAYING;
        c.position = r.position;
        c.positionFrac = r.positionFrac;
        c.curBuffer = r.buffer;
        c.loopBuffer = r.looping ? r.buffer : -1;
        c.flags = (L.hrtf ? kFlagHasHrtf : 0u) | (r.queue ? kFlagQueue : 0u);
        L.queueDone[v] = 0u;
        for(int i = 0; i < 6; ++i) c.sendSlot[i] = -1;
        if(r.buffer >= 0) c.buf = L.buffers[r.buffer];
        L.ctl[v] = c;
        L.dfilt[size_t{v} * 2 + 0].f = def;
        L.dfilt[size_t{v} * 2 + 1].f = def;
    }
    if(t < kMaxPad) L.prev[size_t{v} * kMaxPad + t] = 0.0f;
    if(L.nfc && t < 20) reinterpret_cast<float*>(L.nfc[v].z)[t] = 0.0f;
    if(L.hrtf)
    {
        L.hist[size_t{v} * kHist + t] = 0.0f;
        for(uint32_t k = t; k < L.irStride * 2; k += 64)
        {
            L.hrtfOld[size_t{v} * L.irStride * 2 + k] = 0.0f;
            L.hrtfTgt[size_t{v} * L.irStride * 2 + k] = 0.0f;
        }
    }
    else if(t < L.numDry)
    {
        L.gainCur[size_t{v} * L.numDry + t] = 0.0f;
        L.gainTgt[size_t{v} * L.numDry + t] = 0.0f;
    }
    if(t < L.numSends * 2) L.sfilt[size_t{v} * L.numSends * 2 + t].f = def;
    for(uint32_t k = t; k < L.numSends * L.wetChannels; k += 64)
    {
        L.sendCur[size_t{v} * L.numSends * L.wetChannels + k] = 0.0f;
        L.sendTgt[size_t{v} * L.numSends * L.wetChannels + k] = 0.0f;
    }
}

void LaunchInitVoices(hipStream_t s, const DeviceLayout &L, const VoiceInitRecord *recs, uint32_t count)
{
    if(count) hipLaunchKernelGGL(InitVoicesKernel, dim3(count), dim3(64), 0, s, L, recs);
}

__global__ void __launch_bounds__(64) BlendRowsKernel(DeviceLayout L, const ParamRecord *__restrict__ recs, float *__restrict__ rows)
{
    const ParamRecord &r = recs[blockIdx.x];
    if(r.keepHrtf) return;
    const uint32_t lane = threadIdx.x;
    const uint32_t i0 = r.hrtfIdx[0], i1 = r.hrtfIdx[1], i2 = r.hrtfIdx[2], i3 = r.hrtfIdx[3];
    const float w0 = r.hrtfW[0], w1 = r.hrtfW[1], w2 = r.hrtfW[2], w3 = r.hrtfW[3];
    const uint32_t live = ((L.irSize + 1u) & ~1u) * 2u;
    for(uint32_t e = lane; e < L.irStride * 2; e += 64)
    {
        float x = (e < 2) ? r.hrtfPass : 0.0f;
        x = L.hrirs[size_t{i0} * (kHrirLen * 2) + e] * w0 + x;
        x = L.hrirs[size_t{i1} * (kHrirLen * 2) + e] * w1 + x;
        x = L.hrirs[size_t{i2} * (kHrirLen * 2) + e] * w2 + x;
        x = L.hrirs[size_t{i3} * (kHrirLen * 2) + e] * w3 + x;
        rows[size_t{blockIdx.x} * L.irStride * 2 + e] = (e < live) ? x : 0.0f;
    }
}
void LaunchBlendRows(hipStream_t s, const DeviceLayout &L, const ParamRecord *recs, uint32_t count, float *rows)
{
    if(count) hipLaunchKernelGGL(BlendRowsKernel, dim3(count), dim3(64), 0, s, L, recs, rows);
}

void LaunchApplyParams(hipStream_t s, const DeviceLayout &L, const ParamRecord *recs, uint32_t count)
{
    if(count) hipLaunchKernelGGL(ApplyParamsKernel, dim3(count), dim3(64), 0, s, L, recs);
}

struct RawMove { uint32_t voice; float ev, az, dist, spread, gain; };
static_assert(sizeof(RawMove) == sizeof(oalgpu_voice_move), "RawMove mirrors oalgpu_voice_move");
__global__ void __launch_bounds__(64) ApplyMovesKernel(DeviceLayout L, HrtfStoreDev st, const RawMove *__restrict__ moves)
{
    const RawMove m = moves[blockIdx.x];
    const uint32_t v = m.voice, lane = threadIdx.x;
    const HrirBlend b = HrtfBlendFor(st, m.ev, m.az, m.dist, m.spread);
    if(lane == 0)
    {
        VoiceCtl &ctl = L.ctl[v];
        ctl.flags |= kFlagHasHrtf | kFlagHrtfDirty;
        ctl.hrtfTgtDelay[0] = b.delay[0]; ctl.hrtfTgtDelay[1] = b.delay[1];
        ctl.hrtfTgtGain = m.gain;
    }
    ApplyHrtfTargetWave(L, v, b.idx, b.w, b.passthru, lane);
}

void LaunchApplyMoves(hipStream_t s, const DeviceLayout &L, const HrtfStoreDev &st, const void *moves, uint32_t count, hipEvent_t evDone)
{
    if(count) hipExtLaunchKernelGGL(ApplyMovesKernel, dim3(count), dim3(64), 0, s, nullptr, evDone, 0u, L, st, static_cast<const RawMove*>(moves));
}

__global__ void __launch_bounds__(64) ApplyTargetsKernel(DeviceLayout L, const TargetRecord *__restrict__ recs,
    const float *__restrict__ coeffs)
{
    const TargetRecord &r = recs[blockIdx.x];
    const uint32_t v = r.voice, lane = threadIdx.x;
    if(lane == 0)
    {
        VoiceCtl &ctl = L.ctl[v];
        ctl.flags |= kFlagHasHrtf | kFlagHrtfDirty;
        ctl.hrtfTgtDelay[0] = r.delay[0]; ctl.hrtfTgtDelay[1] = r.delay[1];
        ctl.hrtfTgtGain = r.gain;
    }
    const uint32_t live = ((L.irSize + 1u) & ~1u) * 2u;
    const float *src = coeffs + size_t{blockIdx.x} * (kHrirLen * 2);
    for(uint32_t e = lane; e < L.irStride * 2; e += 64)
        L.hrtfTgt[size_t{v} * L.irStride * 2 + e] = (e < live) ? src[e] : 0.0f;
}

void LaunchApplyTargets(hipStream_t s, const DeviceLayout &L, const TargetRecord *recs, const float *coeffs, uint32_t count)
{
    if(count) hipLaunchKernelGGL(ApplyTargetsKernel, dim3(count), dim3(64), 0, s, L, recs, coeffs);
}

namespace {

__device__ __forceinline__ bool TableFitsLds(int kind, uint32_t m)
{
    if(kind == 2) return true;
    if(kind == 3) return 32u * (2u * m + 4u) <= uint32_t(kTabFloats);
    if(kind == 4) return 64u * (2u * m + 4u) <= uint32_t(kTabFloats);
    return false;
}

__device__ __forceinline__ TabLayout LdsTabLayout(uint32_t m) { return TabLayout{2u * m + 4u, 32u * (2u * m + 4u), 12u}; }

__device__ __forceinline__ void StageTable(SharedMem &sm, const float *__restrict__ filter, int kind, uint32_t m)
{
    const uint32_t t = threadIdx.x;
    if(kind == 2)
    {
        for(uint32_t k = t; k < 256u; k += kThreads) sm.tab[(k >> 3) * 12u + (k & 7u)] = filter[k];
    }
    else
    {
        const uint32_t row = 2u * m, stride = row + 4u;
        const uint32_t blocks = kind == 4 ? 2u : 1u;
        for(uint32_t b = 0; b < blocks; ++b)
            for(uint32_t k = t; k < 32u * row; k += kThreads)
                sm.tab[b * 32u * stride + (k / row) * stride + (k % row)] = filter[b * 32u * row + k];
    }
}

template<bool EXACT>
__device__ __forceinline__ void LoadResampled(SharedMem &sm, const DeviceLayout &L, uint32_t v, const VoiceCtl &ctl,
    bool playing, int32_t intPos, uint32_t fracPos, uint32_t increment, uint32_t samplesToLoad,
    uint32_t samplesToMix, int32_t bufferItem, bool looping, uint32_t &stagedTable, uint32_t mixOffset = 0)
{
    const uint32_t t = threadIdx.x;
    float *rdata = sm.rdata;
    float *srcBuffer = rdata + kMaxEdge;
    float *mixing = sm.in + kHist + mixOffset;
    if(t < kMaxPad) rdata[t] = L.prev[size_t{v} * kMaxPad + t];
    const float *filter = L.tables + ctl.rsFilterOffset;
    const int kind = ctl.rsKind;
    const uint32_t rsM = ctl.rsM, rsL = ctl.rsL;
    const float rsSf = ctl.rsSf;
    const bool resamples = !(increment == kFracOne && fracPos == 0) || samplesToLoad > 1200u;
    const bool useLds = kind >= 2 && TableFitsLds(kind, rsM);
    const uint32_t tableKey = ctl.rsFilterOffset * 8u + uint32_t(kind);
    if(useLds && resamples && stagedTable != tableKey)
    {
        __syncthreads();
        StageTable(sm, filter, kind, rsM);
        stagedTable = tableKey;
    }
    __syncthreads();

    for(uint32_t loaded = 0; loaded < samplesToLoad;)
    {
        uint32_t bdst, bsrc;
        CalcBufferSize(fracPos, increment, samplesToLoad - loaded, bdst, bsrc);
        uint32_t srcDelay = 0;
        bool silent = false;
        if(intPos < 0)
        {
            srcDelay = uint32_t(-intPos);
            if(srcDelay >= bsrc)
            {
                for(uint32_t k = t; k < bdst; k += kThreads) mixing[loaded + k] = 0.0f;
                for(uint32_t k = t; k < bsrc; k += kThreads) srcBuffer[k] = 0.0f;
                silent = true;
            }
            else
                for(uint32_t k = t; k < srcDelay; k += kThreads) srcBuffer[k] = 0.0f;
        }
        if(silent)
        {
            __syncthreads();
            loaded += bdst;
// ... 377 lines not shown
                    const float oldGain = counter ? ctl.hrtfOldGain : ctl.hrtfTgtGain;
                    uint32_t fademix = 0;
                    float blendGain = targetGain;
                    if(counter)
                    {
                        fademix = N < counter ? N : counter;
                        if(counter > fademix)
                            blendGain = lerpf(oldGain, targetGain, float(fademix) / float(counter));
                    }
                    const float newStep = fademix ? blendGain / float(fademix) : 0.0f;
                    const float gainAfterBlend = fademix ? blendGain : oldGain;
                    const uint32_t todo = N - fademix;
                    float endGain = targetGain;
                    if(todo && counter > N)
                        endGain = lerpf(gainAfterBlend, targetGain, float(todo) / float(counter - fademix));
                    const float mainStep = todo ? (endGain - gainAfterBlend) / float(todo) : 0.0f;
                    const bool oldOn = fademix && oldGain > kGainSilence;
                    const bool newOn = fademix && newStep * float(fademix) > kGainSilence;
                    const uint32_t odL = ctl.hrtfOldDelay[0], odR = ctl.hrtfOldDelay[1];
                    const uint32_t dL = ctl.hrtfTgtDelay[0], dR = ctl.hrtfTgtDelay[1];
                    const float *oldCo = sm.coO;
                    const float *tgtCo = sm.coT;

                    if constexpr(EXACT)
                    {
#pragma unroll
                        for(int k = 0; k < 5; ++k)
                        {
                            const uint32_t o = t + 256u * k;
                            if(o >= kLine + kHrirLen) continue;
                            if(oldOn)
                                HrtfGatherFrame<true, kGainOldFade>(eL[k], eR[k], inbuf, oldCo, irEff, odL, odR, 0.0f,
                                    oldGain / float(fademix), fademix, o);
                            if(newOn)
                                HrtfGatherFrame<true, kGainNewFade>(eL[k], eR[k], inbuf, tgtCo, irEff, dL, dR, 0.0f, newStep,
                                    fademix, o);
                            if(todo && o >= fademix)
                                HrtfGatherFrame<true, kGainRamp>(eL[k], eR[k], inbuf + fademix, tgtCo, irEff, dL, dR,
                                    gainAfterBlend, mainStep, todo, o - fademix);
                        }
                    }
                    else
                    {
                        for(uint32_t i = t; i < N; i += kThreads)
                        {
                            float g;
                            if(i < fademix) g = newOn ? newStep * float(i) : 0.0f;
                            else g = gainAfterBlend + mainStep * float(i - fademix);
                            sm.xl[kXPad + i] = inbuf[kHist - dL + i] * g;
                            sm.xr[kXPad + i] = inbuf[kHist - dR + i] * g;
                        }
                        if(t < 64)
                        {
                            float lv = 0.0f, rv = 0.0f;
                            if(oldOn && t < fademix)
                            {
                                const float g = (oldGain / float(fademix)) * float(fademix - t);
                                lv = inbuf[kHist - odL + t] * g;
                                rv = inbuf[kHist - odR + t] * g;
                            }
                            sm.xol[kXPad + t] = lv;
                            sm.xor_[kXPad + t] = rv;
                        }
                        __syncthreads();
                        FirMain(hL, hR, sm.xl, sm.xr, tgtCo, irStride, 4 * t);
                        {
                            const uint32_t ear = t >> 7, fr = t & 127;
                            const float *xe = ear ? sm.xr : sm.xl;
                            hTail = FirOne(hTail, xe + kXPad + kLine + fr, tgtCo, irStride, ear);
                            if(oldOn)
                            {
                                const float *xo = ear ? sm.xor_ : sm.xol;
                                hOld0 = FirOne(hOld0, xo + kXPad + fr, oldCo, irStride, ear);
                                if(irStride > 64) hOld1 = FirOne(hOld1, xo + kXPad + 128 + fr, oldCo, irStride, ear);
                            }
                        }
                    }
                    __syncthreads();
                    if((counter == 0 || fademix) && t < irStride * 2)
                        L.hrtfOld[size_t{v} * irStride * 2 + t] = tgtCo[t];
                    if(t == 0)
                    {
                        VoiceCtl &c = L.ctl[v];
                        if(counter == 0 || fademix) { c.hrtfOldDelay[0] = dL; c.hrtfOldDelay[1] = dR; }
                        c.hrtfOldGain = todo ? endGain : gainAfterBlend;
                    }
                    continue;
                }

                const float *curSnap = sm.gCur[tg2], *tgtSnap = sm.gTgt[tg2];
                auto mixOnto = [&](const float *src, uint32_t lineBase, uint32_t nlines, uint32_t gainOff, float *cur)
                {
                    float s4[4];
#pragma unroll
                    for(int k = 0; k < 4; ++k) s4[k] = (t + 256u * k < N) ? src[t + 256u * k] : 0.0f;
#pragma unroll
                    for(int c = 0; c < LINES; ++c)
                    {
                        const uint32_t rel = uint32_t(c) - lineBase;
                        if(uint32_t(c) < lineBase || rel >= nlines) continue;
                        const float tg = playing ? tgtSnap[gainOff + rel] : 0.0f;
                        const float cu = counter ? curSnap[gainOff + rel] : tg;
                        const MixLineGain g = PrepareMixLine(cu, tg, counter, N);
#pragma unroll
                        for(int k = 0; k < 4; ++k)
                        {
                            const uint32_t p = t + 256u * k;
                            if(p < N && MixLineActive(g, p)) lineAcc[c][k] = lineAcc[c][k] + MixLineValue(g, s4[k], p);
                        }
                        if(t == 0) cur[gainOff + rel] = g.newCur;
                    }
                };
                if(isDirect)
                {
                    float *cur = L.gainCur + size_t{v} * numDry;
                    const bool nfcV = L.nfc && (ctl.flags & kFlagNfc);
                    mixOnto(samples, 0u, nfcV ? 1u : numDry, 0u, cur);
                    if(nfcV)
                    {
                        uint32_t line = 1;
                        for(uint32_t o = 1; o <= L.nfcOrders; ++o)
                        {
                            const uint32_t cnt = L.chansPerOrder[o];
                            __syncthreads();
                            if(t == 0) NfcSerial(L.nfc[v], o, samples, sm.xl, N);
                            __syncthreads();
                            mixOnto(sm.xl, line, cnt, line, cur);
                            line += cnt;
                        }
                    }
                }
                else
                {
                    const int32_t slot = sm.sendSlot[si];
                    if(slot < 0) continue;
                    mixOnto(samples, (L.hrtf ? 0u : numDry) + uint32_t(slot) * wetCh, wetCh, 0u,
                        L.sendCur + (size_t{v} * numSends + si) * wetCh);
                }
            }
            __syncthreads();
        }

        if(t == 0)
        {
            VoiceCtl &c = L.ctl[v];
            c.flags = (ctl.flags | kFlagFading) & ~(((counter == 0 || N) ? kFlagHrtfDirty : 0u) | kFlagDelayed);
            if(!playing) c.playState = OALGPU_VOICE_STOPPED;
            else
            {
                bufPosFrac += increment * samplesToMix;
                const uint32_t samplesDone = bufPosFrac >> kFracBits;
                bufPosInt = AddSat(bufPosInt, int32_t(samplesDone));
                bufPosFrac &= kFracMask;
                if(bufferItem >= 0 && bufPosInt > 0 && (ctl.flags & kFlagQueue))
                {
                    uint32_t buffersDone = 0;
                    const int32_t before = bufferItem;
                    AdvanceQueue(L.buffers, bufferItem, ctl.loopBuffer, bufPosInt, buffersDone);
                    if(buffersDone) L.queueDone[v] += buffersDone;
                    if(bufferItem >= 0 && bufferItem != before) c.buf = L.buffers[bufferItem];
                }
                else if(bufferItem >= 0 && bufPosInt > 0)
                {
                    const BufferItem &b = L.buffers[bufferItem];
                    if(loopItem >= 0)
                    {
                        uint32_t pos = uint32_t(bufPosInt);
// ... 222 lines not shown
```

### openal-soft_amd/csrc/voice_wave.hip

```cpp
#include <hip/hip_ext.h>
#include "wave_common.hpp"

#pragma clang fp contract(off)

#ifndef OALGPU_WAVE_MIN_WG
#define OALGPU_WAVE_MIN_WG 2
#endif

namespace oalgpu {
namespace {
struct RowLineGain {
    float gain{0.0f}, cur{0.0f}, step{0.0f};
    uint32_t fadeLen{0};
    __device__ __forceinline__ void add(const MixLineGain &g)
    {
        const float constant = g.steady ? g.tgt : 0.0f;
        gain += constant;
        if(g.fadeLen) { cur += g.cur; step += g.step; fadeLen = g.fadeLen; }
        else cur += constant;
    }
};
__device__ __forceinline__ void StoreRowBlock(uint32_t *blk, uint32_t ls, uint32_t lane, const RowLineGain &r, bool live)
{
    uint32_t maxFade = r.fadeLen;
// ... 113 lines not shown
                rrN[k] = __builtin_amdgcn_readfirstlane(list[(b + k < nLive) ? b + k : (nLive ? nLive - 1u : 0u)]);
                sN[k] = *reinterpret_cast<const float4*>(rows + size_t{rrN[k]} * kLine);
            }
        };
        if(nLive) loadBatch(0u);
        for(uint32_t b = 0; b < nLive; b += kRowBatch)
        {
            uint32_t rr[kRowBatch];
            float4 s[kRowBatch];
#pragma unroll
            for(uint32_t k = 0; k < kRowBatch; ++k) { rr[k] = rrN[k]; s[k] = sN[k]; }
            if(b + kRowBatch < nLive) loadBatch(b + kRowBatch);
#pragma unroll
            for(uint32_t k = 0; k < kRowBatch; ++k)
            {
                if(b + k >= nLive) break;
                const uint32_t *blk = gl + rr[k] * kBlk;
                const uint2 fl = *reinterpret_cast<const uint2*>(blk + 3u * S);
                const uint32_t mask = __builtin_amdgcn_readfirstlane(fl.x), len = __builtin_amdgcn_readfirstlane(fl.y);
                const float sv[4] = {s[k].x, s[k].y, s[k].z, s[k].w};
#pragma unroll
                for(int z = 0; z < S / 8; ++z)
                {
                    if(!((mask >> z) & 1u)) continue;
                    const float4 g0 = *reinterpret_cast<const float4*>(blk + 8 * z), g1 = *reinterpret_cast<const float4*>(blk + 8 * z + 4);
                    const float gv[8] = {g0.x, g0.y, g0.z, g0.w, g1.x, g1.y, g1.z, g1.w};
#pragma unroll
                    for(int c = 0; c < 8; ++c)
#pragma unroll
                        for(int j = 0; j < 4; ++j) acc[8 * z + c][j] = __builtin_fmaf(sv[j], gv[c], acc[8 * z + c][j]);
                    if(wave == 0u && len != 0u)
                    {
                        const float4 a0 = *reinterpret_cast<const float4*>(blk + S + 8 * z), a1 = *reinterpret_cast<const float4*>(blk + S + 8 * z + 4);
                        const float4 b0 = *reinterpret_cast<const float4*>(blk + 2 * S + 8 * z), b1 = *reinterpret_cast<const float4*>(blk + 2 * S + 8 * z + 4);
                        const float av[8] = {a0.x, a0.y, a0.z, a0.w, a1.x, a1.y, a1.z, a1.w};
                        const float bv[8] = {b0.x, b0.y, b0.z, b0.w, b1.x, b1.y, b1.z, b1.w};
#pragma unroll
                        for(int j = 0; j < 4; ++j)
                        {
                            const uint32_t fr = 4u * t + uint32_t(j);
                            const float sr = (fr < len) ? sv[j] : 0.0f;
                            const float ff = float(fr);
#pragma unroll
                            for(int c = 0; c < 8; ++c) acc[8 * z + c][j] = __builtin_fmaf(sr, av[c] + bv[c] * ff, acc[8 * z + c][j]);
                        }
                    }
                }
            }
        }
    }
    float *pl = L.partLines + size_t{group} * L.mixLines * kLine + 4u * t;
#pragma unroll
    for(int c = 0; c < S; ++c)
    {
        if(uint32_t(c) >= L.mixLines) continue;
        float4 o;
        o.x = (4u * t < N) ? acc[c][0] : 0.0f; o.y = (4u * t + 1u < N) ? acc[c][1] : 0.0f;
        o.z = (4u * t + 2u < N) ? acc[c][2] : 0.0f; o.w = (4u * t + 3u < N) ? acc[c][3] : 0.0f;
        StorePartial(reinterpret_cast<f4*>(pl + size_t(c) * kLine), f4{o.x, o.y, o.z, o.w});
    }
}

template<int S>
__global__ void __launch_bounds__(kWThreads) StreamRowsMixKernel(DeviceLayout L, uint32_t samplesToDo, uint32_t vpg)
{
    __shared__ uint32_t lds[kMixListMax + 4u + kMixGainDwords];
    const uint32_t group = blockIdx.x, v0 = group * vpg;
    const uint32_t nv = v0 < L.numVoices ? ((L.numVoices - v0 < vpg) ? L.numVoices - v0 : vpg) : 0u;
    WgMixRows<S, 4u>(lds, L, group, v0, nv, threadIdx.x, samplesToDo);
}

struct WaveArgsHrtf {
    uint32_t numVoices, waveVoices, irStride, pad;
    const float *tables;
    const BufferItem *buffers;
    VoiceCtl *ctl;
    float *prev;
    BiquadSlot *dfilt;
    float *hrtfOld, *hrtfTgt, *hist;
    AmbiScaleState *ambi;
    uint32_t *startDelay, *queueDone;
    float *partHrtf;
    const float *hrirs;
    explicit WaveArgsHrtf(const DeviceLayout &L) : numVoices{L.numVoices}, waveVoices{L.waveVoices}, irStride{L.irStride}, pad{L.irSize},
        tables{L.tables}, buffers{L.buffers}, ctl{L.ctl}, prev{L.prev}, dfilt{L.dfilt}, hrtfOld{L.hrtfOld}, hrtfTgt{L.hrtfTgt},
        hist{L.hist}, ambi{L.ambi}, startDelay{L.startDelay}, queueDone{L.queueDone}, partHrtf{L.partHrtf}, hrirs{L.hrirs} { }
};

struct NextBlock { const ParamRecord *recs; const int32_t *map; const float *rows; ResidentArgs res; };

[[maybe_unused]] __device__ __forceinline__ uint32_t ResLoadSys(const uint32_t *p) { return __hip_atomic_load(p, __ATOMIC_RELAXED, __HIP_MEMORY_SCOPE_SYSTEM); }
[[maybe_unused]] __device__ __forceinline__ unsigned long long ResLoadSys(const unsigned long long *p) { return __hip_atomic_load(p, __ATOMIC_RELAXED, __HIP_MEMORY_SCOPE_SYSTEM); }
[[maybe_unused]] __device__ __forceinline__ uint32_t ResLoadDev(const uint32_t *p) { return __hip_atomic_load(p, __ATOMIC_RELAXED, __HIP_MEMORY_SCOPE_AGENT); }
[[maybe_unused]] __device__ __forceinline__ void StorePartialCoherent(f2 *p, f2 v)
{
    __hip_atomic_store(reinterpret_cast<unsigned long long*>(p), __builtin_bit_cast(unsigned long long, v), __ATOMIC_RELAXED, __HIP_MEMORY_SCOPE_AGENT);
}
template<class F>
__device__ __forceinline__ bool ResWait(F ready, uint32_t *waited = nullptr)
{
    if(ready()) return true;
    const unsigned long long t0 = __builtin_amdgcn_s_memrealtime();
    bool ok = false;
    for(uint32_t spins = 0;; ++spins)
    {
        if(spins < 32u) __builtin_amdgcn_s_sleep(2); else __builtin_amdgcn_s_sleep(24);
        if(ready()) { ok = true; break; }
        if((spins & 15u) == 15u && __builtin_amdgcn_s_memrealtime() - t0 > kResidentWatchdogTicks) break;
    }
    if(waited) __hip_atomic_fetch_add(waited, uint32_t(__builtin_amdgcn_s_memrealtime() - t0), __ATOMIC_RELAXED, __HIP_MEMORY_SCOPE_AGENT);
    return ok;
}
__device__ __forceinline__ void ApplyRecordLean(const WaveArgsHrtf &L, const ParamRecord &r, uint32_t lane)
{
    const uint32_t v = r.voice;
    VoiceCtl &ctl = L.ctl[v];
    if(lane == 0)
    {
        ctl.step = r.step;
        ctl.rsKind = r.rsKind; ctl.rsM = r.rsM; ctl.rsL = r.rsL; ctl.rsSf = r.rsSf;
        ctl.rsFilterOffset = r.rsFilterOffset;
        const uint32_t keep = ctl.flags & (kFlagFading | kFlagHasHrtf | kFlagAmbiScale | kFlagNfc | kFlagDelayed | kFlagQueue
            | (r.keepHrtf ? uint32_t(kFlagHrtfDirty) : 0u));
        ctl.flags = keep | (r.flags & ~(kFlagFading | kFlagHasHrtf | kFlagHrtfDirty | kFlagAmbiScale | kFlagNfc | kFlagDelayed | kFlagQueue))
            | kFlagHasHrtf | (r.keepHrtf ? 0u : uint32_t(kFlagHrtfDirty));
        for(int i = 0; i < 6; ++i) ctl.sendSlot[i] = -1;
        if(!r.keepHrtf)
        {
            ctl.hrtfTgtDelay[0] = r.hrtfDelay[0]; ctl.hrtfTgtDelay[1] = r.hrtfDelay[1];
            ctl.hrtfTgtGain = r.hrtfGain;
        }
    }
    if(lane == 1) BiquadSetTarget(L.dfilt[size_t{v} * 2 + 0].f, r.dirLp);
    if(lane == 2) BiquadSetTarget(L.dfilt[size_t{v} * 2 + 1].f, r.dirHp);
    if(!r.keepHrtf)
    {
        const uint32_t i0 = r.hrtfIdx[0], i1 = r.hrtfIdx[1], i2 = r.hrtfIdx[2], i3 = r.hrtfIdx[3];
        const float w0 = r.hrtfW[0], w1 = r.hrtfW[1], w2 = r.hrtfW[2], w3 = r.hrtfW[3], pass = r.hrtfPass;
        const uint32_t live = ((L.pad + 1u) & ~1u) * 2u;
        for(uint32_t e = lane; e < L.irStride * 2; e += 64)
        {
            float x = (e < 2) ? pass : 0.0f;
            x = L.hrirs[size_t{i0} * (kHrirLen * 2) + e] * w0 + x;
            x = L.hrirs[size_t{i1} * (kHrirLen * 2) + e] * w1 + x;
            x = L.hrirs[size_t{i2} * (kHrirLen * 2) + e] * w2 + x;
            x = L.hrirs[size_t{i3} * (kHrirLen * 2) + e] * w3 + x;
            L.hrtfTgt[size_t{v} * L.irStride * 2 + e] = (e < live) ? x : 0.0f;
        }
    }
}
__device__ __forceinline__ void ApplyNextRecord(const WaveArgsHrtf &L, const ParamRecord &r, uint32_t lane) { ApplyRecordLean(L, r, lane); }
__device__ __forceinline__ void ApplyNextRecord(const DeviceLayout &L, const ParamRecord &r, uint32_t lane) { ApplyRecordWave(L, r, lane); }

struct RecScalars {
    uint32_t step; int32_t rsKind; uint32_t rsM, rsL; float rsSf; uint32_t rsFilterOffset, flags, keepHrtf, delay0, delay1; float gain;
    float lp[5], hp[5];
};
__device__ __forceinline__ RecScalars LoadRecScalars(const ParamRecord &r)
{
    RecScalars o;
    o.step = r.step; o.rsKind = r.rsKind; o.rsM = r.rsM; o.rsL = r.rsL; o.rsSf = r.rsSf; o.rsFilterOffset = r.rsFilterOffset;
    o.flags = r.flags; o.keepHrtf = r.keepHrtf; o.delay0 = r.hrtfDelay[0]; o.delay1 = r.hrtfDelay[1]; o.gain = r.hrtfGain;
#pragma unroll
    for(int k = 0; k < 5; ++k) { o.lp[k] = r.dirLp[k]; o.hp[k] = r.dirHp[k]; }
    return o;
}
__device__ __forceinline__ void InstallPair(const WaveArgsHrtf &L, const int32_t *__restrict__ map, const ParamRecord *__restrict__ recs,
    const float *__restrict__ rows, uint32_t vA, uint32_t vB, bool hasB, uint32_t lane)
{
    const int32_t mA = map[vA], mB = map[hasB ? vB : vA];
    const int32_t riA = __builtin_amdgcn_readfirstlane(mA), riBr = __builtin_amdgcn_readfirstlane(mB);
    const int32_t riB = hasB ? riBr : -1;
    if(riA < 0 && riB < 0) return;
    const bool doA = riA >= 0, doB = riB >= 0;
    const uint32_t irStride = L.irStride;
    RecScalars sA{}, sB{};
    f2 rowA = {0.0f, 0.0f}, rowB = {0.0f, 0.0f};
    uint32_t flA = 0u, flB = 0u;
    if(doA)
    {
        sA = LoadRecScalars(recs[riA]);
        if(lane < irStride) rowA = reinterpret_cast<const f2*>(rows + size_t{uint32_t(riA)} * irStride * 2u)[lane];
        if(lane == 0) flA = L.ctl[vA].flags;
    }
    if(doB)
    {
        sB = LoadRecScalars(recs[riB]);
        if(lane < irStride) rowB = reinterpret_cast<const f2*>(rows + size_t{uint32_t(riB)} * irStride * 2u)[lane];
        if(lane == 0) flB = L.ctl[vB].flags;
    }
    const bool fLane = lane >= 1u && lane <= 4u;
    const bool fB = lane >= 3u, fHp = ((lane - 1u) & 1u) != 0u;
    const bool fOn = fLane && (fB ? doB : doA);
    BiquadState *fp = &L.dfilt[size_t{fB ? vB : vA} * 2u + (fHp ? 1u : 0u)].f;
    float tb0 = 0.0f, tb1 = 0.0f, tb2 = 0.0f, ta1 = 0.0f, ta2 = 0.0f;
    int32_t fcounter = 0;
    if(fOn) { tb0 = fp->tb0; tb1 = fp->tb1; tb2 = fp->tb2; ta1 = fp->ta1; ta2 = fp->ta2; fcounter = fp->counter; }
    auto installCtl = [&](uint32_t v, const RecScalars &r, uint32_t flagsOld, f2 row)
    {
        VoiceCtl &ctl = L.ctl[v];
        if(lane == 0)
        {
            ctl.step = r.step;
            ctl.rsKind = r.rsKind; ctl.rsM = r.rsM; ctl.rsL = r.rsL; ctl.rsSf = r.rsSf;
            ctl.rsFilterOffset = r.rsFilterOffset;
            const uint32_t keep = flagsOld & (kFlagFading | kFlagHasHrtf | kFlagAmbiScale | kFlagNfc | kFlagDelayed | kFlagQueue
                | (r.keepHrtf ? uint32_t(kFlagHrtfDirty) : 0u));
            ctl.flags = keep | (r.flags & ~(kFlagFading | kFlagHasHrtf | kFlagHrtfDirty | kFlagAmbiScale | kFlagNfc | kFlagDelayed | kFlagQueue))
                | kFlagHasHrtf | (r.keepHrtf ? 0u : uint32_t(kFlagHrtfDirty));
            for(int i = 0; i < 6; ++i) ctl.sendSlot[i] = -1;
            if(!r.keepHrtf)
            {
                ctl.hrtfTgtDelay[0] = r.delay0; ctl.hrtfTgtDelay[1] = r.delay1;
                ctl.hrtfTgtGain = r.gain;
            }
        }
        if(!r.keepHrtf && lane < irStride) reinterpret_cast<f2*>(L.hrtfTgt + size_t{v} * irStride * 2u)[lane] = row;
    };
    if(doA) installCtl(vA, sA, flA, rowA);
    if(doB) installCtl(vB, sB, flB, rowB);
    if(fOn)
    {
        float c[5];
#pragma unroll
        for(int k = 0; k < 5; ++k) c[k] = fB ? (fHp ? sB.hp[k] : sB.lp[k]) : (fHp ? sA.hp[k] : sA.lp[k]);
        bool changed = !(fabsf(c[0] - tb0) <= 0.015625f);
        changed |= !(fabsf(c[1] - tb1) <= 0.015625f);
        changed |= !(fabsf(c[2] - tb2) <= 0.015625f);
        changed |= !(fabsf(c[3] - ta1) <= 0.015625f);
        changed |= !(fabsf(c[4] - ta2) <= 0.015625f);
        fp->tb0 = c[0]; fp->tb1 = c[1]; fp->tb2 = c[2]; fp->ta1 = c[3]; fp->ta2 = c[4];
        const bool snap = changed ? !(fcounter >= 0) : (fcounter <= 0);
        if(changed && fcounter >= 0) fp->counter = 256;
        if(snap) { fp->counter = 0; fp->b0 = c[0]; fp->b1 = c[1]; fp->b2 = c[2]; fp->a1 = c[3]; fp->a2 = c[4]; }
    }
}

template<int R, int TAPS, int NL, bool SENDS, bool MF = false, bool PROF = false, class LT = DeviceLayout, int ACCL = 0, bool RES = false>
__global__ void OALGPU_SINGLE_DS_OPS __launch_bounds__(kWThreads, OALGPU_WAVE_MIN_WG) VoiceWaveKernel(LT L, uint32_t samplesToDo, WaveProf prof, NextBlock next)
{
    static_assert(!RES || (MF && NL == 0 && !SENDS && !PROF && ACCL == 0 && std::is_same<LT, WaveArgsHrtf>::value), "the resident launch is the HRTF hot path's");
    static_assert(std::is_same<LT, DeviceLayout>::value || (NL == 0 && !SENDS), "the lean argument block is the HRTF variants'");
    static_assert(ACCL == 0 || NL > 0 || SENDS, "line accumulators belong to kernels that mix onto lines");
    static_assert(!MF || (R == 17 && TAPS == 64 && NL == 0), "the matrix-pipe FIR is the 64-tap HRTF form");
    using WL = WaveLds<R, TAPS, MF>;
    __shared__ WgLds<R, TAPS, MF> sm;
    const uint32_t t = threadIdx.x;
    const uint32_t lane0 = t & 63u;
    const uint32_t wave = __builtin_amdgcn_readfirstlane(t >> 6);
    const uint32_t group = blockIdx.x;
    const uint32_t vpw = L.waveVoices;
    const uint32_t irStride = L.irStride;
    WL &w = sm.w[wave];
    uint32_t N = samplesToDo;
    if constexpr (std::is_same<LT, WaveArgsHrtf>::value)
        asm volatile("; argument block resident" :: "s"(L.tables), "s"(L.buffers), "s"(L.ctl), "s"(L.prev), "s"(L.dfilt), "s"(L.hrtfOld),
            "s"(L.hrtfTgt), "s"(L.hist), "s"(L.ambi), "s"(L.startDelay), "s"(L.queueDone), "s"(L.partHrtf), "s"(L.hrirs),
            "s"(next.recs), "s"(next.map), "s"(L.numVoices), "s"(L.waveVoices), "s"(L.irStride), "s"(L.pad), "s"(samplesToDo), "s"(gridDim.x));

    const uint32_t vBegin = group * kWWaves * vpw + (wave & 1u) + 2u * (wave >> 1) * vpw;
    const uint32_t vEnd = (vBegin + 2u * vpw < L.numVoices) ? vBegin + 2u * vpw : L.numVoices;
    const uint32_t vCount = vBegin < vEnd ? (vEnd - vBegin + 1u) / 2u : 0u;
    auto waveStamp = [&](int slot)
    {
        if constexpr (PROF)
        {
            if(prof.times && lane0 == 0)
                prof.times[size_t{L.numVoices} * 8 + size_t{group * kWWaves + wave} * 8 + slot] = __builtin_readcyclecounter();
        }
    };
    const uint32_t ablate = PROF ? prof.ablate : 0u;
    waveStamp(0);
    const bool rev = group >= (gridDim.x + 1u) / 2u;
    auto voiceAt = [&](uint32_t j) { return vBegin + 2u * (rev ? vCount - 1u - j : j); };

    uint32_t upd = 0u, updBase = 0u;
    if constexpr (RES)
    {
        const ResidentArgs &RA = next.res;
        upd = updBase = RA.base;
        if(t == 0)
        {
            const uint32_t old = __hip_atomic_fetch_add(RA.counters + 16u * kRcStarted, 1u, __ATOMIC_RELAXED, __HIP_MEMORY_SCOPE_AGENT);
            if(old + 1u == RA.startedTarget)
                __hip_atomic_store(RA.hostFlags + 16u * kRhResident, RA.launchId, __ATOMIC_RELAXED, __HIP_MEMORY_SCOPE_SYSTEM);
        }
    }
    for(;;)
    {
    uint32_t tU = t, laneU = lane0;
    if constexpr (RES) asm volatile("" : "+v"(tU), "+v"(laneU));
    const uint32_t t = tU, lane0 = laneU;
    bool stageRows = true;
    if constexpr (RES)
    {
        const ResidentArgs &RA = next.res;
        if(t == 0)
        {
            const unsigned long long tTop = __builtin_amdgcn_s_memrealtime();
            uint32_t go = 0u, fault = 0u;
            unsigned long long recs = 0ull, map = 0ull, rowsP = 0ull;
            uint32_t smp = 0u;
            if(upd != RA.endSeq)
// ... 702 lines not shown
                        const f2 xi = w.xo[i];
#pragma unroll
                        for(int q = 0; q < WL::kQ; ++q) accO[q] = pkfma(w.cold[64 + lane + 64 * q - i], xi, accO[q]);
                    }
                }
            }
        }

        if(haveNext)
        {
            WaveSync();
            if(planN.prefetch)
            {
                const bool isShort = bufN.fmt == OALGPU_FMT_SHORT;
                if(lane < kMaxPad) { w.rd[lane] = prevN; if(lane) w.rd2[lane - 1u] = prevN; }
#pragma unroll
                for(int i = 0; i < kPre; ++i)
                {
                    const float sv = GatherDecode(preN[i], isShort);
                    w.rd[kMaxEdge + lane + 64u * uint32_t(i)] = sv;
                    w.rd2[kMaxEdge - 1u + lane + 64u * uint32_t(i)] = sv;
                }
            }
            if constexpr (NL == 0)
            {
                w.in[lane] = histN;
                if constexpr (MF)
                {
                    float sh;
                    HalfScale(WaveMaxBits(__builtin_bit_cast(uint32_t, __builtin_fmaxf(__builtin_fabsf(hN.x), __builtin_fabsf(hN.y)))), sh, invH);
                    invH = __builtin_bit_cast(float, __builtin_amdgcn_readfirstlane(__builtin_bit_cast(int, invH)));
                    uint32_t hi, lo;
                    SplitHalf2(hN.x * sh, hN.y * sh, hi, lo);
                    uint16_t *hz = reinterpret_cast<uint16_t*>(&w.hr[0][0][0]);
                    const uint32_t u = 80u - lane;
                    hz[0 * kHrHalves + u] = uint16_t(hi); hz[1 * kHrHalves + u] = uint16_t(lo);
                    hz[2 * kHrHalves + u] = uint16_t(hi >> 16); hz[3 * kHrHalves + u] = uint16_t(lo >> 16);
                }
                if(dirtyN)
                {
                    if constexpr (MF)
                    {
                        float sh;
                        HalfScale(WaveMaxBits(__builtin_bit_cast(uint32_t, __builtin_fmaxf(__builtin_fabsf(oldN[0].x), __builtin_fabsf(oldN[0].y)))), sh, invHO);
                        invHO = __builtin_bit_cast(float, __builtin_amdgcn_readfirstlane(__builtin_bit_cast(int, invHO)));
                        uint32_t hi, lo;
                        SplitHalf2(oldN[0].x * sh, oldN[0].y * sh, hi, lo);
                        uint16_t *hz = reinterpret_cast<uint16_t*>(&w.hro[0][0][0]);
                        const uint32_t u = 80u - lane;
                        hz[0 * kHrHalves + u] = uint16_t(hi); hz[1 * kHrHalves + u] = uint16_t(lo);
                        hz[2 * kHrHalves + u] = uint16_t(hi >> 16); hz[3 * kHrHalves + u] = uint16_t(lo >> 16);
                    }
                    else
                    {
#pragma unroll
                    for(int q = 0; q < TAPS / 64; ++q) w.cold[64 + lane + 64 * q] = oldN[q];
                    }
                }
            }
            if constexpr (SENDS) fstC = fstN;
            else if(lane < 32u) w.fst[lane] = fstN;
            {
                const uint32_t li = lane & 15u;
                const uint32_t bits = __builtin_bit_cast(uint32_t, fstN);
                const float ahead = __builtin_bit_cast(float, __builtin_amdgcn_update_dpp(0, int(bits), 0x105, 0xF, 0xF, true));
                bool ok = true;
                if(li < 2u) ok = fstN == 0.0f;
                else if(li < 7u) ok = fstN == ahead;
                else if(li == 12u) ok = bits == 0u;
                fstClean = __ballot(!ok && lane < 32u) == 0ull;
            }
            WaveSync();
        }

        if(first) waveStamp(1);
        if(active)
        {
            stamp(5);
            if(NL == 0 && dirty && (counter == 0 || fademix))
            {
                const float *tg = L.hrtfTgt + size_t{v} * irStride * 2;
                float *od = L.hrtfOld + size_t{v} * irStride * 2;
                for(uint32_t k = lane; k < irStride * 2; k += 64) od[k] = tg[k];
            }
            if(lane == 0)
            {
                VoiceCtl &c = L.ctl[v];
                if(NL == 0)
                {
                    if(counter == 0 || fademix) { c.hrtfOldDelay[0] = tail.tgtDelay[0]; c.hrtfOldDelay[1] = tail.tgtDelay[1]; }
                    c.hrtfOldGain = todo ? endGain : gainAfterBlend;
                }
                uint32_t flags = (head.flags | kFlagFading) & ~kFlagDelayed;
                if(NL > 0 || counter == 0 || fademix) flags &= ~kFlagHrtfDirty;
                c.flags = flags;
                if(!playing) c.playState = OALGPU_VOICE_STOPPED;
                else
                {
                    int32_t bufPosInt = head.position;
                    uint32_t bufPosFrac = head.positionFrac + head.step * (N - outPos);
                    const uint32_t samplesDone = bufPosFrac >> kFracBits;
                    bufPosInt = AddSat(bufPosInt, int32_t(samplesDone));
                    bufPosFrac &= kFracMask;
                    if(bufferItem >= 0 && bufPosInt > 0 && (head.flags & kFlagQueue))
                    {
                        uint32_t buffersDone = 0;
                        const int32_t before = bufferItem;
                        AdvanceQueue(L.buffers, bufferItem, head.loopBuffer, bufPosInt, buffersDone);
                        if(buffersDone) L.queueDone[v] += buffersDone;
                        if(bufferItem >= 0 && bufferItem != before) c.buf = L.buffers[bufferItem];
                    }
                    else if(bufferItem >= 0 && bufPosInt > 0)
                    {
                        if(looping)
                        {
                            uint32_t pos = uint32_t(bufPosInt);
                            if(pos >= buf.loopEnd)
                            {
                                pos = ((pos - buf.loopStart) % (buf.loopEnd - buf.loopStart)) + buf.loopStart;
                                bufPosInt = int32_t(pos);
                            }
                        }
                        else if(uint32_t(bufPosInt) >= buf.sampleLen)
                            bufferItem = -1;
                    }
                    c.position = bufPosInt;
                    c.positionFrac = bufPosFrac;
                    c.curBuffer = bufferItem;
                    if(bufferItem < 0)
                    {
                        c.loopBuffer = -1;
                        c.playState = OALGPU_VOICE_STOPPING;
                    }
                }
            }
            WaveSync();
            stamp(6);
        }
    }

    waveStamp(2);
    auto mixRows = [&]()
    {
        if constexpr (NL > 0 || SENDS)
        {
        static_assert(sizeof(sm) >= (kMixListMax + 4u + kMixGainDwords) * sizeof(uint32_t), "the row mix stages its gain blocks in the voices' LDS");
        uint32_t *lds = reinterpret_cast<uint32_t*>(&sm);
        const uint32_t vWg = group * kWWaves * vpw;
        const uint32_t nvWg = vWg < L.numVoices ? ((vWg + kWWaves * vpw < L.numVoices) ? kWWaves * vpw : L.numVoices - vWg) : 0u;
        if(L.lineStride <= 8u) WgMixRows<8>(lds, L, group, vWg, nvWg, t, N);
        else if(L.lineStride <= 16u) WgMixRows<16>(lds, L, group, vWg, nvWg, t, N);
        else WgMixRows<32>(lds, L, group, vWg, nvWg, t, N);
        waveStamp(3);
        }
    };
    auto dumpLines = [&]()
    {
        if constexpr (ACCL > 0)
        {
        auto areaOf = [&](int ww) { return MF ? reinterpret_cast<f2*>(&sm.w[ww].xh[0][0][0]) : sm.w[ww].x2; };
        static_assert(!MF || sizeof(w.xh) >= size_t(WL::kFrames) * sizeof(f2), "a line pair fits in the FIR-input area");
        const uint32_t nlines = L.mixLines;
        float *pl = L.partLines + size_t{group} * nlines * kLine;
#pragma unroll
        for(int c = 0; c < ACCL; c += 2)
        {
// ... 226 lines not shown
```

### openal-soft_amd/csrc/voice_wave16.hip

```cpp
#define OALGPU_WAVE_NO_LAUNCHER
#include "voice_wave.hip"

#pragma clang fp contract(off)

namespace oalgpu {
namespace {

constexpr int kW16Outs = kLine / 64;

constexpr int kW16Rd = 1184;
constexpr int kW16Rd2 = kMaxEdge + kPre * 64 + 8;
constexpr int kW16Area = kResampleDataSize + kLine;
static_assert(kW16Rd % 64 == 32 && kW16Rd >= kMaxPad + kPre * 64 + 8, "rd2 sits half the banks away from rd");
static_assert(kW16Rd + kW16Rd2 <= kW16Area, "the twice-parked window fits");
static_assert(kResampleDataSize >= kLine + 64, "a send's filter scan parks the unfiltered samples in the window's area");
constexpr int kW16DumpF2 = 64 * 17 + 68;
static_assert(kW16DumpF2 * 2 <= kW16Area, "the dump fits");
struct W16PhaseB {
    uint32_t xh[2][kXhDw];
    uint32_t hr[2][kHrDw];
    uint32_t hro[2][kHrDw];
    float in0[2 * kHist];
};
static_assert(sizeof(W16PhaseB) <= size_t(kW16Area) * 4, "phase B fits the area (nothing of it is written before the sample line is back in registers)");
// ... 54 lines not shown
#pragma unroll
            for(int q = 0; q < NP; ++q) S[set][q] = f2{s[2 * (g * NP + q)], s[2 * (g * NP + q) + 1]};
        }
    };
    const uint32_t tb = frac0 + lane * increment;
    load(0, tb, 0);
#pragma unroll
    for(int j = 0; j < kW16Outs; ++j)
    {
        outs[j] = 0.0f;
        if(uint32_t(64 * j) < bdst)
        {
            const uint32_t tt0 = tb + uint32_t(j) * tstep;
            const uint32_t tt = tt0 < tlast ? tt0 : tlast;
            const f2 pf = splat(float(tt & 2047u) * (1.0f / 2048.0f));
            f2 r0 = {0.0f, 0.0f}, r1 = {0.0f, 0.0f};
#pragma unroll
            for(int g = 0; g < G; ++g)
            {
                const int u = j * G + g, nx = u + 1;
                if(nx < kW16Outs * G) load(nx & 1, tb + uint32_t(nx / G) * tstep, nx % G);
#pragma unroll
                for(int q = 0; q < NP; ++q)
                {
                    const f2 c = pkfma(pf, P[u & 1][q], F[u & 1][q]);
                    if(q & 1) r1 = pkfma(c, S[u & 1][q], r1);
                    else r0 = pkfma(c, S[u & 1][q], r0);
                }
            }
            outs[j] = (r0.x + r0.y) + (r1.x + r1.y);
        }
    }
}

template<int TILES, bool LOW8>
__device__ __forceinline__ void FirMfmaEar(f4 (&acc)[5], const uint32_t (&xh)[2][kXhDw], const uint32_t (&hr)[2][kHrDw], float inv, uint32_t lane)
{
    const uint32_t i = lane & 15u, g = lane >> 4;
    const uint32_t u0 = 16u - i + 8u * g, shift = (u0 & 1u) * 2u, ud = u0 >> 1;
    const f4 vinv = {inv, inv, inv, inv};
    h8 A[2][3];
#pragma unroll
    for(int s = 0; s < 2; ++s)
#pragma unroll
        for(int c = 0; c < 3; ++c)
        {
            const uint32_t *p = hr[s] + ud + 16 * c;
            const uint32_t q0 = p[0], q1 = p[1], q2 = p[2], q3 = p[3], q4 = p[4];
            const u4 q = {__builtin_amdgcn_alignbyte(q1, q0, shift), __builtin_amdgcn_alignbyte(q2, q1, shift),
                __builtin_amdgcn_alignbyte(q3, q2, shift), __builtin_amdgcn_alignbyte(q4, q3, shift)};
            A[s][c] = __builtin_bit_cast(h8, q);
        }
#pragma unroll
    for(int T = 0; T < TILES; ++T)
    {
        __builtin_amdgcn_sched_barrier(0);
        const uint32_t j = (T == 4 && i > 3u) ? 3u : i;
        h8 B[2][3];
#pragma unroll
        for(int s = 0; s < 2; ++s)
        {
            const u4 *p = reinterpret_cast<const u4*>(xh[s]) + 32 * T + 2u * j + g;
#pragma unroll
            for(int c = 0; c < 3; ++c) B[s][c] = __builtin_bit_cast(h8, p[4 * c]);
        }
        f4 ta = {0.0f, 0.0f, 0.0f, 0.0f}, tb = ta, tc = ta;
#pragma unroll
        for(int c = 0; c < 3; ++c)
        {
            ta = __builtin_amdgcn_mfma_f32_16x16x32_f16(A[1][c], B[0][c], ta, 0, 0, 0);
            tb = __builtin_amdgcn_mfma_f32_16x16x32_f16(A[0][c], B[1][c], tb, 0, 0, 0);
            tc = __builtin_amdgcn_mfma_f32_16x16x32_f16(A[0][c], B[0][c], tc, 0, 0, 0);
        }
        f4 sum = __builtin_elementwise_fma((ta + tb) + tc, vinv, acc[T]);
        asm volatile("" : "+v"(sum));
        if(!LOW8 || i < 8u) acc[T] = sum;
        __builtin_amdgcn_sched_barrier(0);
    }
}

__device__ __forceinline__ float W16ReadLaneF(float v, int l)
{ return __builtin_bit_cast(float, __builtin_amdgcn_readlane(__builtin_bit_cast(int, v), l)); }

__device__ __forceinline__ float W16StageResponse(uint32_t (&hr)[2][kHrDw], float h, uint32_t lane)
{
    float sh, inv;
    HalfScale(WaveMaxBits(__builtin_bit_cast(uint32_t, __builtin_fabsf(h))), sh, inv);
    uint32_t hi, lo;
    SplitHalf2(h * sh, 0.0f, hi, lo);
    uint32_t *hz32 = &hr[0][0];
    for(uint32_t k = lane; k < uint32_t(2 * kHrDw); k += 64) hz32[k] = 0u;
    uint16_t *hz = reinterpret_cast<uint16_t*>(&hr[0][0]);
    const uint32_t u = 80u - lane;
    hz[0 * kHrHalves + u] = uint16_t(hi); hz[1 * kHrHalves + u] = uint16_t(lo);
    return __builtin_bit_cast(float, __builtin_amdgcn_readfirstlane(__builtin_bit_cast(int, inv)));
}

__device__ __forceinline__ uint32_t W16VoiceOf(uint32_t group, uint32_t wave, uint32_t waves)
{
    const uint32_t a = wave >> 2, b = wave & 3u;
    return group * waves + 4u * a + ((a + b) & 3u);
}

struct Next16 { const ParamRecord *recs; const int32_t *map; const float *rows; ResidentArgs res; };
struct W16Sends {
    BiquadSlot *sfilt; const float *sendTgt; float *sendCur; float *streams; uint32_t *lineGains;
    uint32_t numSends, wetCh, lineStride, spv;
};

template<bool PROF, int WAVES, bool SENDS = false, bool RES = false>
__global__ void OALGPU_SINGLE_DS_OPS __launch_bounds__(WAVES * 64) VoiceWave16Kernel(WaveArgsHrtf L, uint32_t samplesToDo, Next16 next, WaveProf prof, W16Sends S)
{
    unsigned long long tEntry = 0;
    if constexpr (PROF) tEntry = __builtin_readcyclecounter();
    constexpr uint32_t kW16Waves = uint32_t(WAVES), kW16Threads = uint32_t(WAVES) * 64u;
    __shared__ W16Wg<WAVES> sm;
    const uint32_t t = threadIdx.x;
    uint32_t lane = t & 63u;
    const uint32_t wave = __builtin_amdgcn_readfirstlane(t >> 6);
    const uint32_t group = blockIdx.x;
    const uint32_t irStride = L.irStride;
    uint32_t N = samplesToDo;
    W16Lds &w = sm.w[wave];
    asm volatile("; argument block resident" :: "s"(L.tables), "s"(L.buffers), "s"(L.ctl), "s"(L.prev), "s"(L.dfilt), "s"(L.hrtfOld),
        "s"(L.hrtfTgt), "s"(L.hist), "s"(L.ambi), "s"(L.startDelay), "s"(L.queueDone), "s"(L.partHrtf), "s"(L.hrirs),
        "s"(next.recs), "s"(next.map), "s"(L.numVoices), "s"(L.irStride), "s"(L.pad), "s"(samplesToDo));

    const uint32_t vRaw = W16VoiceOf(group, wave, kW16Waves);
    const bool haveVoice = vRaw < L.numVoices;
    const uint32_t lastVoice = L.numVoices - 1u;
    const uint32_t v = haveVoice ? vRaw : lastVoice;
    const uint32_t keyVoice = group * uint32_t(kW16Waves);

    uint32_t upd = 0u, updBase = 0u;
    if constexpr (RES)
    {
        const ResidentArgs &RA = next.res;
        upd = updBase = RA.base;
        if(t == 0)
        {
            const uint32_t old = __hip_atomic_fetch_add(RA.counters + 16u * kRcStarted, 1u, __ATOMIC_RELAXED, __HIP_MEMORY_SCOPE_AGENT);
            if(old + 1u == RA.startedTarget)
                __hip_atomic_store(RA.hostFlags + 16u * kRhResident, RA.launchId, __ATOMIC_RELAXED, __HIP_MEMORY_SCOPE_SYSTEM);
        }
    }
    for(;;)
    {
    uint32_t tU = threadIdx.x;
    if constexpr (RES) { asm volatile("" : "+v"(tU)); lane = tU & 63u; }
    const uint32_t t = tU;
    if constexpr (RES)
    {
        const ResidentArgs &RA = next.res;
        if(t == 0)
        {
            const unsigned long long tTop = __builtin_amdgcn_s_memrealtime();
            uint32_t go = 0u, fault = 0u;
            unsigned long long recs = 0ull, map = 0ull, rowsP = 0ull;
            uint32_t smp = 0u;
            if(upd != RA.endSeq)
            {
                const ResidentDoor *door = RA.door;
                const uint32_t *exitp = &door->exitSeq[RA.launchId & 3u];
                const uint32_t *rr = RA.counters + 16u * kRcRedRead;
                const bool needRed = int32_t(upd - kResidentSets) >= 0;
                const uint32_t want = (upd - kResidentSets + 1u) * RA.redPerUpdate;
                unsigned long long t0 = 0ull;
                uint32_t waitedFor = 0u;
                for(uint32_t spins = 0;; ++spins)
                {
                    const uint32_t ex = ResLoadSys(exitp), sq = ResLoadSys(&door->seq), rd = needRed ? ResLoadDev(rr) : want;
                    if(int32_t(ex - upd) <= 0) break;
                    const bool rung = int32_t(sq - upd) > 0, redOk = int32_t(rd - want) >= 0;
                    if(rung && redOk) { go = 1u; break; }
                    if(spins == 0u) { t0 = __builtin_amdgcn_s_memrealtime(); waitedFor = rung ? 2u : 1u; }
                    else if((spins & 15u) == 15u && __builtin_amdgcn_s_memrealtime() - t0 > kResidentWatchdogTicks)
                    {
                        fault = 1u;
                        uint32_t *fi = RA.hostFlags + 16u * kRhFault;
                        fi[0] = upd; fi[1] = sq; fi[2] = ex; fi[3] = rd; fi[4] = want; fi[5] = group; fi[6] = RA.launchId;
                        fi[7] = uint32_t(__builtin_amdgcn_s_memrealtime() - t0);
                        break;
                    }
                    if(spins < 32u) __builtin_amdgcn_s_sleep(2); else __builtin_amdgcn_s_sleep(24);
                }
                if(waitedFor && (group & 127u) == 0u)
                    __hip_atomic_fetch_add(RA.counters + 16u * (waitedFor == 1u ? kRcWaitDoor : kRcWaitRed), uint32_t(__builtin_amdgcn_s_memrealtime() - t0),
                        __ATOMIC_RELAXED, __HIP_MEMORY_SCOPE_AGENT);
                if(go)
                {
                    const ResidentSlot *sl = &door->slot[upd % kResidentSlots];
                    recs = ResLoadSys(&sl->recs); map = ResLoadSys(&sl->map); rowsP = ResLoadSys(&sl->rows); smp = ResLoadSys(&sl->samples);
                }
            }
            if(fault) __hip_atomic_store(RA.hostFlags + 16u * kRhError, 1u, __ATOMIC_RELAXED, __HIP_MEMORY_SCOPE_SYSTEM);
            if((group & 127u) == 0u)
                __hip_atomic_fetch_add(RA.counters + 16u * kRcTop, uint32_t(__builtin_amdgcn_s_memrealtime() - tTop), __ATOMIC_RELAXED, __HIP_MEMORY_SCOPE_AGENT);
            sm.res[0] = go; sm.res[1] = smp;
            sm.res[2] = uint32_t(recs); sm.res[3] = uint32_t(recs >> 32); sm.res[4] = uint32_t(map); sm.res[5] = uint32_t(map >> 32);
            sm.res[8] = uint32_t(rowsP); sm.res[9] = uint32_t(rowsP >> 32);
        }
        __syncthreads();
        const unsigned long long tSeen = __builtin_amdgcn_s_memrealtime();
        if(__builtin_amdgcn_readfirstlane(sm.res[0]) == 0u) break;
        N = __builtin_amdgcn_readfirstlane(sm.res[1]);
        const unsigned long long recsU = (uint64_t{uint32_t(__builtin_amdgcn_readfirstlane(sm.res[3]))} << 32) | uint32_t(__builtin_amdgcn_readfirstlane(sm.res[2]));
        const unsigned long long mapU = (uint64_t{uint32_t(__builtin_amdgcn_readfirstlane(sm.res[5]))} << 32) | uint32_t(__builtin_amdgcn_readfirstlane(sm.res[4]));
        if(mapU && haveVoice)
        {
            const unsigned long long rowsU = (uint64_t{uint32_t(__builtin_amdgcn_readfirstlane(sm.res[9]))} << 32) | uint32_t(__builtin_amdgcn_readfirstlane(sm.res[8]));
            InstallPair(L, reinterpret_cast<const int32_t*>(mapU), reinterpret_cast<const ParamRecord*>(recsU), reinterpret_cast<const float*>(rowsU), v, v, false, lane);
        }
        asm volatile("s_waitcnt vmcnt(0) lgkmcnt(0)" ::: "memory");
        __syncthreads();
        __builtin_amdgcn_s_dcache_inv();
        asm volatile("s_waitcnt lgkmcnt(0)" ::: "memory");
        if(t == 0)
        {
            const unsigned long long tIn = __builtin_amdgcn_s_memrealtime();
            if((group & 127u) == 0u)
                __hip_atomic_fetch_add(RA.counters + 16u * kRcInstall, uint32_t(tIn - tSeen), __ATOMIC_RELAXED, __HIP_MEMORY_SCOPE_AGENT);
            sm.res[6] = uint32_t(tIn);
        }
    }
    auto stamp = [&](int slot)
    {
        if constexpr (PROF) { if(prof.times && haveVoice && (t & 63u) == 0u) prof.times[size_t{v} * 8 + slot] = __builtin_readcyclecounter(); }
    };
    if constexpr (PROF) { if(prof.times && haveVoice && (t & 63u) == 0u) prof.times[size_t{v} * 8 + 0] = tEntry; }
    auto stamp2 = [&](int slot)
    {
        if constexpr (PROF) { if(prof.times && haveVoice && (t & 63u) == 0u) prof.times[size_t{L.numVoices} * 8 + size_t{v} * 8 + slot] = __builtin_readcyclecounter(); }
    };
    const VoiceHead head = LoadHeadScalar(L.ctl + v);
    const BufferItem buf = LoadCtlBufferScalar(L.ctl + v);
    const VoiceTail tail = LoadTailScalar(L.ctl + v);
    asm volatile("" ::: "memory");
    const VoiceHead headK = LoadHeadScalar(L.ctl + (keyVoice < L.numVoices ? keyVoice : lastVoice));
    asm volatile("" ::: "memory");
    const int psK = headK.playState, kK = headK.rsKind;
    const uint32_t mK = kK == 2 ? 4u : headK.rsM, lK = kK == 2 ? 1u : headK.rsL, offK = headK.rsFilterOffset;

    const bool eligK = keyVoice < L.numVoices && (kK == 2 || (kK == 3 && (mK == 12 || mK == 24)))
        && (psK == OALGPU_VOICE_PLAYING || psK == OALGPU_VOICE_STOPPING);
    bool stageRows = true;
    if constexpr (RES) { if(upd != updBase) stageRows = !(eligK && sm.tabKey == offK * 8u + uint32_t(kK) && sm.tabM == mK); }
    if constexpr (RES) __syncthreads();
    if(eligK && stageRows)
    {
        typedef const __attribute__((address_space(1))) void *gvoidp;
        typedef __attribute__((address_space(3))) void *lvoidp;
        const float *src = L.tables + offK + size_t{lane >> 1} * (2u * mK) + (lane & 1u);
        for(uint32_t pp = wave; pp < mK / 2u; pp += uint32_t(kW16Waves))
        {
            __builtin_amdgcn_global_load_lds((gvoidp)(src + 2u * pp), (lvoidp)&sm.tabF[32u * pp], 4, 0, 0);
            __builtin_amdgcn_global_load_lds((gvoidp)(src + mK + 2u * pp), (lvoidp)&sm.tabP[32u * pp], 4, 0, 0);
        }
        if(t == 0) { sm.tabKey = offK * 8u + uint32_t(kK); sm.tabM = mK; sm.tabL = lK; }
    }

    const int vstate = head.playState;
    const bool mixes = haveVoice && (vstate == OALGPU_VOICE_PLAYING || vstate == OALGPU_VOICE_STOPPING);
    const bool playing = haveVoice && vstate == OALGPU_VOICE_PLAYING;
    bool active = mixes && head.step >= 1u;
    const bool dirty = (head.flags & kFlagHrtfDirty) != 0;
    SrcPlan plan = PlanSource(head, N);
    bool looping = false;
    if(head.curBuffer >= 0)
    {
        looping = head.loopBuffer >= 0 && ((head.flags & kFlagQueue) || !(head.position >= 0 && uint32_t(head.position) >= buf.loopEnd));
        plan.prefetch = plan.prefetch && GatherCovers(plan.bsrc, buf, looping, uint32_t(head.position));
    }
    if(head.flags & (kFlagDelayed | kFlagQueue)) plan.prefetch = false;
    const uint32_t sM = head.rsKind == 2 ? 4u : head.rsM, sL = head.rsKind == 2 ? 1u : head.rsL;
    const bool regPath = active && plan.prefetch && eligK && (head.rsKind == 2 || head.rsKind == 3)
        && head.rsFilterOffset * 8u + uint32_t(head.rsKind) == offK * 8u + uint32_t(kK) && sM == mK
        && !(head.step == kFracOne && head.positionFrac == 0u);
    float pre[kPre];
#pragma unroll
    for(int i = 0; i < kPre; ++i) pre[i] = 0.0f;
    float prevv = 0.0f;
    if(regPath)
    {
        GatherStatic(pre, plan.bsrc, buf, looping, uint32_t(head.position), lane);
        prevv = (lane < kMaxPad) ? L.prev[size_t{v} * kMaxPad + lane] : 0.0f;
    }

    if(!eligK)
    {
        if(wave == 0)
        {
            const uint32_t cand = keyVoice + lane;
            bool eligible = false;
            uint32_t off = 0, m = 0, l = 0;
            int kind = 0;
            if(lane < uint32_t(kW16Waves) && cand < L.numVoices)
            {
                const VoiceCtl &c = L.ctl[cand];
                kind = c.rsKind; off = c.rsFilterOffset; m = c.rsM; l = c.rsL;
                if(kind == 2) { m = 4; l = 1; }
                eligible = (kind == 2 || (kind == 3 && (m == 12 || m == 24)))
                    && (c.playState == OALGPU_VOICE_PLAYING || c.playState == OALGPU_VOICE_STOPPING);
            }
            const unsigned long long mask = __ballot(eligible);
            if(mask)
            {
                const int firstLane = __ffsll((long long)mask) - 1;
                const uint32_t key = uint32_t(__shfl(int(off * 8u + uint32_t(kind)), firstLane));
                const uint32_t fm = uint32_t(__shfl(int(m), firstLane)), fl = uint32_t(__shfl(int(l), firstLane));
                if(lane == 0) { sm.tabKey = key; sm.tabM = fm; sm.tabL = fl; }
            }
            else if(lane == 0) { sm.tabKey = 0xffffffffu; sm.tabM = 0; sm.tabL = 0; }
        }
        __syncthreads();
        const uint32_t key = sm.tabKey, m = sm.tabM;
        if(key != 0xffffffffu)
        {
            const float *filter = L.tables + (key >> 3);
            for(uint32_t idx = t; idx < (m / 2u) * 32u; idx += uint32_t(kW16Threads))
            {
                const uint32_t p = idx >> 5, pi = idx & 31u;
                const float *row = filter + pi * 2u * m;
                sm.tabF[idx] = f2{row[2u * p], row[2u * p + 1u]};
                sm.tabP[idx] = f2{row[m + 2u * p], row[m + 2u * p + 1u]};
            }
        }
    }
    if(regPath)
    {
        const bool isShort = buf.fmt == OALGPU_FMT_SHORT;
        if(lane < kMaxPad) { w.a.rd[lane] = prevv; if(lane) w.a.rd2[lane - 1u] = prevv; }
#pragma unroll
        for(int i = 0; i < kPre; ++i)
        {
            const float sv = GatherDecode(pre[i], isShort);
            w.a.rd[kMaxEdge + lane + 64u * uint32_t(i)] = sv;
            w.a.rd2[kMaxEdge - 1u + lane + 64u * uint32_t(i)] = sv;
        }
    }
    asm volatile("s_waitcnt vmcnt(0)" ::: "memory");
    __syncthreads();
    stamp(7);
    __builtin_amdgcn_s_setprio(2);

    uint32_t outPos = 0;
    if(mixes && !active && !playing && lane == 0) L.ctl[v].playState = OALGPU_VOICE_STOPPED;
    if(active && (head.flags & kFlagDelayed))
    {
        const uint32_t d = L.startDelay[v];
        if(!playing)
        {
            if(lane == 0) { L.ctl[v].playState = OALGPU_VOICE_STOPPED; L.ctl[v].flags = head.flags & ~kFlagDelayed; L.startDelay[v] = 0u; }
            active = false;
        }
        else if(d >= N) { if(lane == 0) L.startDelay[v] = d - N; active = false; }
        else
        {
            outPos = d;
            if(lane == 0) L.startDelay[v] = 0u;
            for(uint32_t k = lane; k < outPos; k += 64) w.g.smp[k] = 0.0f;
        }
    }

    f4 accM[2][5];
#pragma unroll
    for(int e = 0; e < 2; ++e)
#pragma unroll
        for(int b = 0; b < 5; ++b) accM[e][b] = f4{0.0f, 0.0f, 0.0f, 0.0f};

    uint32_t counter = 0, fademix = 0, todo = 0;
    float endGain = 0.0f, gainAfterBlend = 0.0f;
    float fstv = 0.0f, histv = 0.0f;
    f2 hT = {0.0f, 0.0f};
    int32_t bufferItem = head.curBuffer;
    if constexpr (SENDS)
    {
        if(haveVoice && !active && lane < S.spv)
            S.lineGains[(size_t{v} * S.spv + lane) * LineBlockDwords(S.lineStride) + 3u * S.lineStride] = 0u;
    }
    if(active)
    {
        float outs[kW16Outs];
        if(regPath)
        {
            WaveSync();
            const float *rdb = w.a.rd + (kMaxEdge - sL), *rd2b = w.a.rd2 + (kMaxEdge - sL);
            const uint32_t rdbIndex = uint32_t(kMaxEdge) - sL;
            if(sM == 24u) ResampleRingRegs<24, true>(sm.tabF, sm.tabP, rdb, head.positionFrac, head.step, N, outs, lane, rd2b, rdbIndex);
            else if(sM == 12u) ResampleRingRegs<12, true>(sm.tabF, sm.tabP, rdb, head.positionFrac, head.step, N, outs, lane, rd2b, rdbIndex);
            else ResampleRingRegs<4, false>(sm.tabF, sm.tabP, rdb, head.positionFrac, head.step, N, outs, lane, nullptr, 0u);
            asm volatile("" : "+v"(lane));
            if(playing)
            {
                const uint32_t srcOffset = uint32_t((uint64_t{N} * head.step + head.positionFrac) >> kFracBits);
                if(lane < kMaxPad) L.prev[size_t{v} * kMaxPad + lane] = w.a.rd[srcOffset + lane];
            }
        }
        else
        {
            W16GenView gv{w.g.rd, w.g.smp - kHist, nullptr, w.best, w.pad};
            LoadResampledWave<true, false>(sm, gv, L, v, lane, head, playing, N - outPos, N - outPos, bufferItem, looping,
                SrcPlan{false, plan.bdst, plan.bsrc}, outPos);
            asm volatile("" : "+v"(lane));
            WaveSync();
#pragma unroll
            for(int j = 0; j < kW16Outs; ++j) outs[j] = w.g.smp[lane + 64u * uint32_t(j)];
        }
        if(N < uint32_t(kLine))
        {
#pragma unroll
            for(int j = 0; j < kW16Outs; ++j) if(lane + 64u * uint32_t(j) >= N) outs[j] = 0.0f;
        }
        stamp(1);
        __builtin_amdgcn_s_setprio(1);
        fstv = (lane < 32u) ? reinterpret_cast<const float*>(L.dfilt + size_t{v} * 2)[lane] : 0.0f;
        histv = L.hist[size_t{v} * kHist + lane];
        hT = (lane < irStride) ? reinterpret_cast<const f2*>(L.hrtfTgt + size_t{v} * irStride * 2)[lane] : f2{0.0f, 0.0f};
        WaveSync();

        auto toLine = [&]()
        {
#pragma unroll
            for(int j = 0; j < kW16Outs; ++j) w.g.smp[lane + 64u * uint32_t(j)] = outs[j];
            WaveSync();
        };
        auto fromLine = [&]()
        {
            WaveSync();
#pragma unroll
            for(int j = 0; j < kW16Outs; ++j) outs[j] = w.g.smp[lane + 64u * uint32_t(j)];
            WaveSync();
        };
        auto doPair = [&](float fv, BiquadSlot *slots, bool on)
        {
            BiquadState f0, f1;
            {
                float a[13], b[13];
#pragma unroll
                for(int k = 0; k < 13; ++k) { a[k] = W16ReadLaneF(fv, k); b[k] = W16ReadLaneF(fv, 16 + k); }
                f0 = BiquadState{a[0], a[1], a[2], a[3], a[4], a[5], a[6], a[7], a[8], a[9], a[10], a[11], __builtin_bit_cast(int32_t, a[12])};
                f1 = BiquadState{b[0], b[1], b[2], b[3], b[4], b[5], b[6], b[7], b[8], b[9], b[10], b[11], __builtin_bit_cast(int32_t, b[12])};
            }
            if(on)
            {
                if(f0.counter <= 0 && f1.counter <= 0)
                {
                    BiquadDualWaveScan(f0, f1, w.g.smp + outPos, N - outPos, lane);
                    if(lane == 0) { slots[0].f.z1 = f0.z1; slots[0].f.z2 = f0.z2; slots[1].f.z1 = f1.z1; slots[1].f.z2 = f1.z2; }
                }
                else
                {
                    if(lane == 0) BiquadDualInterp(f0, f1, w.g.smp + outPos, w.g.smp + outPos, N - outPos);
                    if(lane == 0) { slots[0].f = f0; slots[1].f = f1; }
                }
            }
            else
            {
                const bool clean0 = f0.z1 == 0.0f && f0.z2 == 0.0f && f0.counter == 0 && f0.b0 == f0.tb0 && f0.b1 == f0.tb1
                    && f0.b2 == f0.tb2 && f0.a1 == f0.ta1 && f0.a2 == f0.ta2;
                const bool clean1 = f1.z1 == 0.0f && f1.z2 == 0.0f && f1.counter == 0 && f1.b0 == f1.tb0 && f1.b1 == f1.tb1
                    && f1.b2 == f1.tb2 && f1.a1 == f1.ta1 && f1.a2 == f1.ta2;
                if(!(clean0 && clean1) && lane == 0)
                {
                    BiquadClear(f0); BiquadClear(f1);
                    slots[0].f = f0; slots[1].f = f1;
                }
            }
        };
        if(head.flags & kFlagAmbiScale)
        {
            const AmbiScaleState a = L.ambi[v];
            SplitterState sp{a.coeff, a.lpZ1, a.lpZ2, a.apZ1};
            toLine();
            SplitterScan<false>(sp, w.g.smp + outPos, N - outPos, a.hfScale, a.lfScale, lane);
            fromLine();
            if(lane == 0) { L.ambi[v].lpZ1 = sp.lpZ1; L.ambi[v].lpZ2 = sp.lpZ2; L.ambi[v].apZ1 = sp.apZ1; }
        }
        counter = (head.flags & kFlagFading) ? (N < 64u ? N : 64u) : 0u;

        if constexpr (SENDS)
        {
            const uint32_t ls = S.lineStride, spv = S.spv, numSends = S.numSends, wetCh = S.wetCh;
            float *rowsV = S.streams + size_t{v} * spv * kLine;
            uint32_t *blkV = S.lineGains + size_t{v} * spv * LineBlockDwords(ls);
            int32_t sendSlots[6];
            {
                static_assert(offsetof(VoiceCtl, sendSlot) == 48, "VoiceCtl::sendSlot follows the head");
                cu4 *src = (cu4*)(uintptr_t)(L.ctl + v);
                const u4 a = src[3], b = src[4];
                sendSlots[0] = int32_t(a.x); sendSlots[1] = int32_t(a.y); sendSlots[2] = int32_t(a.z); sendSlots[3] = int32_t(a.w);
                sendSlots[4] = int32_t(b.x); sendSlots[5] = int32_t(b.y);
            }
            RowLineGain row0;
            bool row0Live = false;
            for(uint32_t si = 0; si < numSends; ++si)
            {
                int32_t slot = sendSlots[0];
#pragma unroll
                for(int k = 1; k < 6; ++k) slot = (si == uint32_t(k)) ? sendSlots[k] : slot;
                uint32_t *blkS = blkV + size_t{2u + si} * LineBlockDwords(ls);
// ... 39 lines not shown
                    if(mine) r.add(g);
                    float *dst = rowsV + size_t{2u + si} * kLine;
#pragma unroll
                    for(int j = 0; j < kW16Outs; ++j)
                    {
                        const uint32_t k = lane + 64u * uint32_t(j);
                        dst[k] = (k < N) ? w.g.smp[k] : 0.0f;
                    }
                    StoreRowBlock(blkS, ls, lane, r, true);
                    WaveSync();
                }
                else
                {
                    if(mine) row0.add(g);
                    row0Live = true;
                    if(lane == 0) blkS[3u * ls] = 0u;
                }
            }
            if(row0Live)
            {
#pragma unroll
                for(int j = 0; j < kW16Outs; ++j) rowsV[lane + 64u * uint32_t(j)] = outs[j];
            }
            StoreRowBlock(blkV, ls, lane, row0, row0Live);
            WaveSync();
        }

        {
            const bool directFilter = (head.flags & kFlagDirectFilter) != 0;
            BiquadSlot *slots = &L.dfilt[size_t{v} * 2];
            if(directFilter)
            {
                toLine();
                doPair(fstv, slots, true);
                fromLine();
            }
            else doPair(fstv, slots, false);
        }

        stamp(2);
        __builtin_amdgcn_s_setprio(0);
        {
            const uint32_t q = N + lane;
            float hv;
            if(N == uint32_t(kLine)) hv = outs[kW16Outs - 1];
            else
            {
                const uint32_t k = q - uint32_t(kHist);
                const uint32_t j0 = (N - uint32_t(kHist)) >> 6;
                float lo = 0.0f, hi2 = 0.0f;
#pragma unroll
                for(int j = 0; j < kW16Outs; ++j) { if(uint32_t(j) == j0) lo = outs[j]; if(uint32_t(j) == j0 + 1u) hi2 = outs[j]; }
                const float sLo = __shfl(lo, int(k & 63u)), sHi = __shfl(hi2, int(k & 63u));
                const float smpv = (N >= uint32_t(kHist)) ? (((k >> 6) == j0) ? sLo : sHi) : __shfl(outs[0], int(k & 63u));
                const float old = __shfl(histv, int(q & 63u));
                hv = (q >= uint32_t(kHist)) ? smpv : old;
            }
            if(playing) __builtin_nontemporal_store(hv, &L.hist[size_t{v} * kHist + lane]);
        }
        w.b.in0[lane] = histv;
        w.b.in0[kHist + lane] = outs[0];

        const float targetGain = tail.tgtGain * (playing ? 1.0f : 0.0f);
        const float oldGain = counter ? tail.oldGain : tail.tgtGain;
        float blendGain = targetGain;
        if(counter)
        {
            fademix = N < counter ? N : counter;
            if(counter > fademix)
                blendGain = lerpf(oldGain, targetGain, float(fademix) / float(counter));
        }
        const float newStep = fademix ? blendGain / float(fademix) : 0.0f;
        gainAfterBlend = fademix ? blendGain : oldGain;
        todo = N - fademix;
        endGain = targetGain;
        if(todo && counter > N)
            endGain = lerpf(gainAfterBlend, targetGain, float(todo) / float(counter - fademix));
        const float mainStep = todo ? (endGain - gainAfterBlend) / float(todo) : 0.0f;
        const bool oldOn = fademix && oldGain > kGainSilence;
        const bool newOn = fademix && newStep * float(fademix) > kGainSilence;
        const float oldStep = fademix ? oldGain / float(fademix) : 0.0f;
        const bool merged = !dirty;
        const bool oldPass = !merged && oldOn;
        const f2 hO = (oldPass && lane < irStride) ? reinterpret_cast<const f2*>(L.hrtfOld + size_t{v} * irStride * 2)[lane] : f2{0.0f, 0.0f};
        const float gbase = gainAfterBlend - mainStep * float(fademix);
        auto gainAt = [&](uint32_t i, bool mayFade)
        {
            float g = __builtin_fmaf(mainStep, float(i), gbase);
            if(mayFade && i < fademix)
            {
                float gf = newOn ? newStep * float(i) : 0.0f;
                if(merged && oldOn) gf += oldStep * float(fademix - i);
                g = gf;
            }
            return g;
        };
        WaveSync();
        stamp2(0);

        float sx, invX;
        {
            float mxo = __builtin_fabsf(histv);
#pragma unroll
            for(int j = 0; j < kW16Outs; ++j) mxo = __builtin_fmaxf(__builtin_fabsf(outs[j]), mxo);
            const float mxw = __builtin_bit_cast(float, WaveMaxBits(__builtin_bit_cast(uint32_t, mxo)));
            const float gmax = __builtin_fmaxf(__builtin_fmaxf(__builtin_fabsf(blendGain) + __builtin_fabsf(oldGain), __builtin_fabsf(gainAfterBlend)),
                __builtin_fabsf(endGain));
            HalfScale(__builtin_bit_cast(uint32_t, mxw * gmax), sx, invX);
            invX = __builtin_bit_cast(float, __builtin_amdgcn_readfirstlane(__builtin_bit_cast(int, invX)));
            sx = __builtin_bit_cast(float, __builtin_amdgcn_readfirstlane(__builtin_bit_cast(int, sx)));
        }
        const float step64 = mainStep * 64.0f * sx;
        auto buildEar = [&](uint32_t d, auto fullTag)
        {
            constexpr bool FULL = decltype(fullTag)::value;
            if(lane < 32u) { w.b.xh[0][lane] = 0u; w.b.xh[1][lane] = 0u; }
            for(uint32_t dw = 32u + (N >> 1) + lane; dw < uint32_t(kXhDw); dw += 64u) { w.b.xh[0][dw] = 0u; w.b.xh[1][dw] = 0u; }
            WaveSync();
            uint16_t *xz = reinterpret_cast<uint16_t*>(&w.b.xh[0][0]) + 64u + lane + d;
            if(lane < d)
            {
                const float headP = (lane < N) ? w.b.in0[kHist - d + lane] * gainAt(lane, true) : 0.0f;
                uint32_t hi, lo;
                SplitHalf2(headP * sx, 0.0f, hi, lo);
                uint16_t *xh0 = reinterpret_cast<uint16_t*>(&w.b.xh[0][0]) + 64u + lane;
                xh0[0] = uint16_t(hi); xh0[kXhHalves] = uint16_t(lo);
            }
            const uint32_t i00 = lane + d;
            const float g0s = gainAt(i00, true) * sx;
            const float gls = __builtin_fmaf(mainStep, float(i00), gbase) * sx;
#pragma unroll
            for(int j = 0; j < kW16Outs; j += 2)
            {
                const float ga = (j == 0) ? g0s : __builtin_fmaf(step64, float(j), gls);
                const float gb = __builtin_fmaf(step64, float(j + 1), gls);
                float p0 = outs[j] * ga, p1 = outs[j + 1] * gb;
                if(!FULL || j + 2 == kW16Outs)
                {
                    if(i00 + 64u * uint32_t(j) >= N) p0 = 0.0f;
                    if(i00 + 64u * uint32_t(j + 1) >= N) p1 = 0.0f;
                }
                uint32_t hi, lo;
                SplitHalf2(p0, p1, hi, lo);
                xz[64 * j] = uint16_t(hi); xz[kXhHalves + 64 * j] = uint16_t(lo);
                xz[64 * (j + 1)] = uint16_t(hi >> 16); xz[kXhHalves + 64 * (j + 1)] = uint16_t(lo >> 16);
            }
        };

#pragma unroll
        for(int e = 0; e < 2; ++e)
        {
            const uint32_t d = tail.tgtDelay[e];
            if(N == uint32_t(kLine)) buildEar(d, std::true_type{}); else buildEar(d, std::false_type{});
            uint16_t *xz = reinterpret_cast<uint16_t*>(&w.b.xh[0][0]);
            if(e == 0) stamp2(1);
            const float invH = W16StageResponse(w.b.hr, e == 0 ? hT.x : hT.y, lane);
            WaveSync();
            if(e == 0) stamp2(2);
            FirMfmaEar<5, false>(accM[e], w.b.xh, w.b.hr, invX * invH, lane);
            if(e == 0) stamp2(3);
            if(oldPass)
            {
                const uint32_t od = tail.oldDelay[e];
                float xo = 0.0f;
                if(lane < fademix) xo = w.b.in0[kHist - od + lane] * (oldStep * float(fademix - lane));
                float sxo, invXo;
                HalfScale(WaveMaxBits(__builtin_bit_cast(uint32_t, __builtin_fabsf(xo))), sxo, invXo);
                invXo = __builtin_bit_cast(float, __builtin_amdgcn_readfirstlane(__builtin_bit_cast(int, invXo)));
                uint32_t hi, lo;
                SplitHalf2(xo * sxo, 0.0f, hi, lo);
                WaveSync();
                xz[0 * kXhHalves + 64u + lane] = uint16_t(hi); xz[1 * kXhHalves + 64u + lane] = uint16_t(lo);
                if(lane < 40u) { w.b.xh[0][64u + lane] = 0u; w.b.xh[1][64u + lane] = 0u; }
                const float invHO = W16StageResponse(w.b.hro, e == 0 ? hO.x : hO.y, lane);
                WaveSync();
                FirMfmaEar<1, true>(accM[e], w.b.xh, w.b.hro, invXo * invHO, lane);
            }
            WaveSync();
            stamp(3 + e);
        }
    }

    if(active)
    {
        if(dirty && (counter == 0 || fademix))
        {
            if(lane < irStride) reinterpret_cast<f2*>(L.hrtfOld + size_t{v} * irStride * 2)[lane] = hT;
        }
        if(lane == 0)
        {
            VoiceCtl &c = L.ctl[v];
            if(counter == 0 || fademix) { c.hrtfOldDelay[0] = tail.tgtDelay[0]; c.hrtfOldDelay[1] = tail.tgtDelay[1]; }
            c.hrtfOldGain = todo ? endGain : gainAfterBlend;
            uint32_t flags = (head.flags | kFlagFading) & ~kFlagDelayed;
            if(counter == 0 || fademix) flags &= ~kFlagHrtfDirty;
            c.flags = flags;
            if(!playing) c.playState = OALGPU_VOICE_STOPPED;
            else
            {
                int32_t bufPosInt = head.position;
                uint32_t bufPosFrac = head.positionFrac + head.step * (N - outPos);
                const uint32_t samplesDone = bufPosFrac >> kFracBits;
                bufPosInt = AddSat(bufPosInt, int32_t(samplesDone));
                bufPosFrac &= kFracMask;
                if(bufferItem >= 0 && bufPosInt > 0 && (head.flags & kFlagQueue))
                {
                    uint32_t buffersDone = 0;
                    const int32_t before = bufferItem;
                    AdvanceQueue(L.buffers, bufferItem, head.loopBuffer, bufPosInt, buffersDone);
                    if(buffersDone) L.queueDone[v] += buffersDone;
                    if(bufferItem >= 0 && bufferItem != before) c.buf = L.buffers[bufferItem];
                }
                else if(bufferItem >= 0 && bufPosInt > 0)
                {
                    if(looping)
                    {
                        uint32_t pos = uint32_t(bufPosInt);
                        if(pos >= buf.loopEnd)
                        {
                            pos = ((pos - buf.loopStart) % (buf.loopEnd - buf.loopStart)) + buf.loopStart;
                            bufPosInt = int32_t(pos);
                        }
                    }
                    else if(uint32_t(bufPosInt) >= buf.sampleLen)
                        bufferItem = -1;
                }
                c.position = bufPosInt;
                c.positionFrac = bufPosFrac;
                c.curBuffer = bufferItem;
                if(bufferItem < 0)
                {
                    c.loopBuffer = -1;
                    c.playState = OALGPU_VOICE_STOPPING;
                }
            }
        }
    }

    if(!RES && next.map && haveVoice)
    {
        __builtin_amdgcn_fence(__ATOMIC_RELEASE, "workgroup");
        if(next.rows && irStride <= 64u) InstallPair(L, next.map, next.recs, next.rows, v, v, false, lane);
        else
        {
            const int32_t ri = __builtin_amdgcn_readfirstlane(next.map[v]);
            if(ri >= 0) ApplyNextRecord(L, next.recs[ri], lane);
        }
    }
    stamp(5);
    {
        WaveSync();
        f2 *dump = w.dump;
        const uint32_t jc = lane & 15u, q4 = lane >> 4;
#pragma unroll
        for(int T = 0; T < 4; ++T)
#pragma unroll
            for(int r = 0; r < 4; ++r)
                dump[17u * (16u * uint32_t(T) + jc) + 4u * q4 + uint32_t(r)] = f2{accM[0][T][r], accM[1][T][r]};
        if(jc < 4u)
        {
#pragma unroll
            for(int r = 0; r < 4; ++r) dump[17u * (64u + jc) + 4u * q4 + uint32_t(r)] = f2{accM[0][4][r], accM[1][4][r]};
        }
        __syncthreads();
        f2 *ph = reinterpret_cast<f2*>(L.partHrtf) + size_t{group} * (kLine + kHrirLen);
        if constexpr (RES)
            ph = reinterpret_cast<f2*>(next.res.partBase + size_t{upd % kResidentSets} * next.res.setStride) + size_t{group} * (kLine + kHrirLen);
        for(uint32_t k = t; k < uint32_t(kLine + kHrirLen); k += uint32_t(kW16Threads))
        {
            f2 s = {0.0f, 0.0f};
            if(k < 64u * 17u)
            {
                const uint32_t at = k + (k >> 4);
                s = sm.w[0].dump[at];
#pragma unroll
                for(int ww = 1; ww < WAVES; ++ww) { const f2 o = sm.w[ww].dump[at]; s.x += o.x; s.y += o.y; }
            }
            if constexpr (RES) StorePartialCoherent(&ph[k], s);
            else StorePartial(&ph[k], s);
        }
    }
    stamp(6);
    if constexpr (!RES) break;
    else
    {
        asm volatile("s_waitcnt vmcnt(0)" ::: "memory");
        __syncthreads();
        if(t == 0)
        {
            __hip_atomic_fetch_add(next.res.counters + 16u * (kRcArrive0 + upd % kResidentSets), 1u, __ATOMIC_RELAXED, __HIP_MEMORY_SCOPE_AGENT);
            if((group & 127u) == 0u)
                __hip_atomic_fetch_add(next.res.counters + 16u * kRcBusy, uint32_t(__builtin_amdgcn_s_memrealtime()) - sm.res[6], __ATOMIC_RELAXED, __HIP_MEMORY_SCOPE_AGENT);
        }
        ++upd;
    }
    }
}

}

bool Wave16Applies(const DeviceLayout &L)
{
    if(!(L.hrtf && L.firMfma && L.irStride >= 8 && L.irStride <= 64 && L.nfc == nullptr)) return false;
    if(L.numSends == 0) return L.accLines == 0;
    return L.numSends <= 6 && L.mixLines >= 1 && L.mixLines <= 32 && L.wetChannels <= 32u;
}
uint32_t Wave16WavesFor(uint32_t voices, uint32_t cus)
{
    for(uint32_t w : {4u, 8u}) if((voices + w - 1u) / w <= cus) return w;
    return 16u;
}
uint32_t Wave16Groups(const DeviceLayout &L) { return (L.numVoices + L.wave16 - 1u) / L.wave16; }
const char *Wave16KernelName(const DeviceLayout &L)
{
    if(L.numSends) return L.wave16 == 16u ? "VoiceWave16Kernel<16, sends>" : (L.wave16 == 8u ? "VoiceWave16Kernel<8, sends>" : "VoiceWave16Kernel<4, sends>");
    return L.wave16 == 16u ? "VoiceWave16Kernel<16>" : (L.wave16 == 8u ? "VoiceWave16Kernel<8>" : "VoiceWave16Kernel<4>");
}

hipError_t LaunchVoiceWave16(hipStream_t s, const DeviceLayout &L, uint32_t samplesToDo, const WaveProf *prof, hipEvent_t evStart, hipEvent_t evStop,
    const ParamRecord *nextRecs, const int32_t *nextMap, const float *nextRows)
{
    const Next16 next{nextRecs, nextMap, nextRows, ResidentArgs{}};
    const WaveProf none{nullptr, 0u};
    const dim3 grid(Wave16Groups(L)), block(L.wave16 * 64u);
    const W16Sends S{L.sfilt, L.sendTgt, L.sendCur, L.streams, L.lineGains, L.numSends, L.wetChannels, L.lineStride, L.streamsPerVoice};
#define OALGPU_W16_LAUNCH(P, W, SD, PA) hipExtLaunchKernelGGL((VoiceWave16Kernel<P, W, SD>), grid, block, 0, s, evStart, evStop, 0u, WaveArgsHrtf{L}, samplesToDo, next, PA, S)
    if(L.numSends)
    {
        const Next16 noNext{nullptr, nullptr, nullptr, ResidentArgs{}};
        if(L.wave16 == 16u) hipExtLaunchKernelGGL((VoiceWave16Kernel<false, 16, true>), grid, block, 0, s, evStart, nullptr, 0u, WaveArgsHrtf{L}, samplesToDo, noNext, none, S);
        else if(L.wave16 == 8u) hipExtLaunchKernelGGL((VoiceWave16Kernel<false, 8, true>), grid, block, 0, s, evStart, nullptr, 0u, WaveArgsHrtf{L}, samplesToDo, noNext, none, S);
        else hipExtLaunchKernelGGL((VoiceWave16Kernel<false, 4, true>), grid, block, 0, s, evStart, nullptr, 0u, WaveArgsHrtf{L}, samplesToDo, noNext, none, S);
        if(hipError_t e = hipGetLastError(); e != hipSuccess) return e;
        return LaunchStreamRowsMix(s, L, samplesToDo, L.wave16, evStop);
    }
    if(prof)
    {
        if(L.wave16 == 16u) OALGPU_W16_LAUNCH(true, 16, false, *prof); else if(L.wave16 == 8u) OALGPU_W16_LAUNCH(true, 8, false, *prof); else OALGPU_W16_LAUNCH(true, 4, false, *prof);
    }
    else
    {
        if(L.wave16 == 16u) OALGPU_W16_LAUNCH(false, 16, false, none); else if(L.wave16 == 8u) OALGPU_W16_LAUNCH(false, 8, false, none); else OALGPU_W16_LAUNCH(false, 4, false, none);
    }
#undef OALGPU_W16_LAUNCH
    return hipGetLastError();
}

hipError_t LaunchVoiceWave16Resident(hipStream_t s, const DeviceLayout &L, const ResidentArgs &args, hipEvent_t evStart, hipEvent_t evStop)
{
    const Next16 next{nullptr, nullptr, nullptr, args};
    const WaveProf none{nullptr, 0u};
    hipExtLaunchKernelGGL((VoiceWave16Kernel<false, 16, false, true>), dim3(Wave16Groups(L)), dim3(1024), 0, s, evStart, evStop, 0u, WaveArgsHrtf{L}, 0u, next, none, W16Sends{});
    return hipGetLastError();
}
int Wave16ResidentGroupsPerCu()
{
    int n = 0;
    if(hipOccupancyMaxActiveBlocksPerMultiprocessor(&n, VoiceWave16Kernel<false, 16, false, true>, 1024, 0) != hipSuccess) { (void)hipGetLastError(); return 0; }
    return n;
}

}
```

### openal-soft_amd/oalgpu/__init__.py

```python
import ctypes as C
import os

import numpy as np

PKG_DIR = os.path.dirname(os.path.dirname(os.path.abspath(__file__)))
LIB_PATH = os.path.join(PKG_DIR, "liboalgpu.so")

BUFFER_LINE = 1024
MAX_PAD = 48
HRTF_HIST = 64
HRIR_LEN = 128
MAX_SENDS = 6
(OUT_I8, OUT_U8, OUT_I16, OUT_U16, OUT_I32, OUT_U32, OUT_F32) = range(7)
MAX_OUT = 32
MAX_AMBI = 25
MATH_EXACT, MATH_FAST = 0, 1
(RS_POINT, RS_LINEAR, RS_SPLINE, RS_GAUSSIAN, RS_FAST_BSINC12, RS_BSINC12, RS_FAST_BSINC24,
 RS_BSINC24, RS_FAST_BSINC48, RS_BSINC48) = range(10)
FMT_UBYTE, FMT_SHORT, FMT_INT, FMT_FLOAT, FMT_DOUBLE, FMT_MULAW, FMT_ALAW = range(7)
FMT_DTYPES = {FMT_UBYTE: np.uint8, FMT_SHORT: np.int16, FMT_INT: np.int32, FMT_FLOAT: np.float32,
              FMT_DOUBLE: np.float64, FMT_MULAW: np.uint8, FMT_ALAW: np.uint8}
VOICE_STOPPED, VOICE_PLAYING, VOICE_STOPPING, VOICE_PENDING = range(4)

f32p = C.POINTER(C.c_float)
MOVE_DTYPE = np.dtype([("voice", np.uint32), ("hrtf_ev", np.float32), ("hrtf_az", np.float32), ("hrtf_dist", np.float32),
                       ("hrtf_spread", np.float32), ("hrtf_gain", np.float32)])
u32p = C.POINTER(C.c_uint32)


class OalgpuError(RuntimeError):
    pass


class BsincTable(C.Structure):
    _fields_ = [("scaleBase", C.c_float), ("scaleRange", C.c_float), ("m", C.c_uint32 * 16),
                ("filterOffset", C.c_uint32 * 16), ("tab", f32p), ("tablen", C.c_size_t)]


class InterpState(C.Structure):
    _fields_ = [("kind", C.c_int32), ("table", C.c_int32), ("sf", C.c_float), ("m", C.c_uint32),
                ("l", C.c_uint32), ("filter_offset", C.c_uint32)]


class Biquad(C.Structure):
    _fields_ = [(n, C.c_float) for n in ("z1", "z2", "b0", "b1", "b2", "a1", "a2", "tb0", "tb1",
                                         "tb2", "ta1", "ta2")] + [("counter", C.c_int32)]

    def as_tuple(self):
        return tuple(getattr(self, n) for n, _ in self._fields_)


class Splitter(C.Structure):
    _fields_ = [("coeff", C.c_float), ("lp_z1", C.c_float), ("lp_z2", C.c_float),
                ("ap_z1", C.c_float)]


class HrtfInfo(C.Structure):
    _fields_ = [(n, C.c_uint32) for n in ("sample_rate", "ir_size", "num_fields", "num_elevs",
                                          "num_irs")]


class ContextDesc(C.Structure):
    _fields_ = [("device", C.c_int32), ("math_mode", C.c_int32), ("sample_rate", C.c_uint32),
                ("num_dry_channels", C.c_uint32), ("num_real_channels", C.c_uint32),
                ("num_aux_sends", C.c_uint32), ("num_slots", C.c_uint32),
                ("wet_channels", C.c_uint32), ("hrtf", C.c_int32), ("max_voices", C.c_uint32),
                ("max_buffers", C.c_uint32), ("voices_per_group", C.c_uint32), ("flags", C.c_uint32)]


class VoiceEvent(C.Structure):
    _fields_ = [("voice", C.c_uint32), ("play_state", C.c_int32), ("has_buffer", C.c_int32), ("current_buffer", C.c_int32),
                ("buffers_done", C.c_uint32), ("position", C.c_int32), ("position_frac", C.c_uint32), ("fading", C.c_int32)]


CTX_FIR_VALU, CTX_PROFILE, CTX_SERIAL, CTX_STREAM_ROWS, CTX_APPLY_IN_VOICE_KERNEL, CTX_FUSED_REDUCE = 1, 2, 4, 8, 16, 32
CTX_RESIDENT = 64
CTX_SLICE_LINES = 128
CTX_WAVE_PAIRS = 256
CTX_ROW_SLICES = 512


class VoiceDesc(C.Structure):
    _fields_ = [("buffer", C.c_int32), ("looping", C.c_int32), ("position", C.c_int32),
                ("position_frac", C.c_uint32), ("frequency", C.c_uint32)]


class FilterParams(C.Structure):
    _fields_ = [("active", C.c_int32), ("gain_hf", C.c_float), ("hf_norm", C.c_float),
                ("gain_lf", C.c_float), ("lf_norm", C.c_float)]


class VoiceParams(C.Structure):
    _fields_ = [("step", C.c_uint32), ("resampler", C.c_int32), ("direct_filter", FilterParams),
                ("dry_gains", C.c_float * MAX_OUT),
                ("hrtf_ev", C.c_float), ("hrtf_az", C.c_float), ("hrtf_dist", C.c_float),
                ("hrtf_spread", C.c_float), ("hrtf_gain", C.c_float),
                ("send_slot", C.c_int32 * MAX_SENDS), ("send_filter", FilterParams * MAX_SENDS),
                ("send_gains", (C.c_float * MAX_AMBI) * MAX_SENDS)]


class VoiceState(C.Structure):
    _fields_ = [("play_state", C.c_int32), ("position", C.c_int32), ("position_frac", C.c_uint32),
                ("has_buffer", C.c_int32), ("fading", C.c_int32),
                ("prev_samples", C.c_float * MAX_PAD), ("dry_current", C.c_float * MAX_OUT),
                ("hrtf_old_gain", C.c_float), ("hrtf_old_delay", C.c_uint32 * 2),
                ("hrtf_history", C.c_float * HRTF_HIST),
                ("direct_lp", Biquad), ("direct_hp", Biquad),
                ("send_current", (C.c_float * MAX_AMBI) * MAX_SENDS),
                ("send_lp", Biquad * MAX_SENDS), ("send_hp", Biquad * MAX_SENDS)]


def _fp(a):
    return a.ctypes.data_as(f32p)


def _load(path=LIB_PATH):
    if not os.path.exists(path):
        raise OalgpuError(f"{path} is missing: build it with __graft_entry__.build() "
                          "(hipcc --offload-arch=gfx950); there is no fallback path")
    L = C.CDLL(path)
    L.oalgpu_version.restype = C.c_char_p
    L.oalgpu_last_error.restype = C.c_char_p
    L.oalgpu_bsinc_table_get.argtypes = [C.c_int, C.POINTER(BsincTable)]
    L.oalgpu_cubic_table_get.argtypes = [C.c_int, f32p]
    L.oalgpu_prepare_resampler.argtypes = [C.c_int, C.c_uint32, C.POINTER(InterpState)]
    L.oalgpu_biquad_reset.argtypes = [C.POINTER(Biquad)]
    L.oalgpu_biquad_reset.restype = None
    L.oalgpu_biquad_set_params_from_slope.argtypes = [C.POINTER(Biquad), C.c_int, C.c_float,
                                                      C.c_float, C.c_float]
    L.oalgpu_biquad_set_params_from_slope.restype = None
    L.oalgpu_splitter_init.argtypes = [C.POINTER(Splitter), C.c_float]
    L.oalgpu_splitter_init.restype = None
    L.oalgpu_resample.argtypes = [C.c_int, C.c_int, C.c_int, C.c_uint32, f32p, C.c_size_t,
                                  C.c_uint32, f32p, C.c_size_t]
    L.oalgpu_mix.argtypes = [C.c_int, f32p, C.c_size_t, f32p, C.c_size_t, f32p, f32p, C.c_size_t,
                             C.c_size_t]
    L.oalgpu_mix_hrtf.argtypes = [C.c_int, C.c_int, f32p, f32p, C.c_uint32, f32p, u32p, C.c_float,
                                  C.c_float, C.c_size_t]
    L.oalgpu_mix_hrtf_blend.argtypes = [C.c_int, C.c_int, f32p, f32p, C.c_uint32, f32p, u32p,
                                        C.c_float, f32p, u32p, C.c_float, C.c_size_t]
    L.oalgpu_mix_direct_hrtf.argtypes = [C.c_int, C.c_int, f32p, f32p, f32p, C.c_size_t, f32p,
                                         C.POINTER(Splitter), f32p, f32p, C.c_size_t, C.c_size_t]
    L.oalgpu_biquad_dual_process.argtypes = [C.c_int, C.POINTER(Biquad), C.POINTER(Biquad), f32p,
                                             f32p, C.c_size_t]
    L.oalgpu_context_create.argtypes = [C.POINTER(ContextDesc), C.POINTER(C.c_void_p)]
    L.oalgpu_context_destroy.argtypes = [C.c_void_p]
    L.oalgpu_context_destroy.restype = None
    L.oalgpu_hrtf_load_mhr.argtypes = [C.c_void_p, C.c_char_p, C.c_size_t]
    L.oalgpu_hrtf_info_get.argtypes = [C.c_void_p, C.POINTER(HrtfInfo)]
    L.oalgpu_hrtf_raw.argtypes = [C.c_void_p, f32p, C.POINTER(C.c_uint8), C.POINTER(C.c_uint16),
                                  C.POINTER(C.c_uint16), f32p, C.POINTER(C.c_uint8)]
    L.oalgpu_hrtf_get_coeffs.argtypes = [C.c_void_p, f32p, C.c_size_t, f32p, u32p]
    L.oalgpu_set_direct_hrtf.argtypes = [C.c_void_p, f32p, f32p, C.c_float, C.c_uint32]
    L.oalgpu_buffer_register.argtypes = [C.c_void_p, C.c_void_p, C.c_int, C.c_uint32, C.c_uint32,
                                         C.c_uint32, C.c_uint32]
    L.oalgpu_voice_init.argtypes = [C.c_void_p, C.c_uint32, C.POINTER(VoiceDesc)]
    L.oalgpu_voice_set_params.argtypes = [C.c_void_p, u32p, C.c_void_p, C.c_size_t]
    L.oalgpu_voice_set_state.argtypes = [C.c_void_p, C.c_uint32, C.c_int]
    L.oalgpu_param_block_create.argtypes = [C.c_void_p, u32p, C.c_void_p, C.c_size_t, C.POINTER(C.c_void_p)]
    L.oalgpu_param_block_apply.argtypes = [C.c_void_p, C.c_void_p]
    L.oalgpu_param_block_destroy.argtypes = [C.c_void_p]
    L.oalgpu_param_block_destroy.restype = None
# ... 920 lines not shown
```

Measured before the change: 113.5 million.

## Cache pre-split half-precision HRTF responses per voice across updates

```diff
diff --git a/include/oalgpu.h b/include/oalgpu.h
--- a/include/oalgpu.h
+++ b/include/oalgpu.h
@@ -129,6 +129,7 @@
 #define OALGPU_CTX_SLICE_LINES 128u
 #define OALGPU_CTX_WAVE_PAIRS 256u
 #define OALGPU_CTX_ROW_SLICES 512u
+#define OALGPU_CTX_RESTAGE_RESPONSES 1024u
 #define OALGPU_CTX_SERIAL   4u
 
 int  oalgpu_context_create(const oalgpu_context_desc *desc, oalgpu_context **out);
diff --git a/openal-soft_amd/csrc/api.hip b/openal-soft_amd/csrc/api.hip
--- a/openal-soft_amd/csrc/api.hip
+++ b/openal-soft_amd/csrc/api.hip
@@ -160,6 +160,7 @@
     L.numGroups = std::max<uint32_t>(1u, (desc->max_voices + vpg - 1u) / vpg);
     L.waveVoices = 0;
     L.firMfma = (desc->flags & OALGPU_CTX_FIR_VALU) ? 0u : 1u;
+    L.restageResponses = (desc->flags & OALGPU_CTX_RESTAGE_RESPONSES) ? 1u : 0u;
     c->serialOnly = (desc->flags & OALGPU_CTX_SERIAL) != 0;
     c->res.enabled = (desc->flags & OALGPU_CTX_RESIDENT) != 0 && !(desc->flags & (OALGPU_CTX_PROFILE | OALGPU_CTX_SERIAL));
     c->useWave = WaveKernelApplies(c->exact, L);
@@ -238,6 +239,7 @@
         c->prof.times = c->phaseTimes.p;
     }
     L.hrtfOld = nullptr; L.hrtfTgt = nullptr;
+    L.hrtfSplit = nullptr;
 
     HIP_TRY(c->dSplit.alloc(L.numDry)); HIP_TRY(c->dSplit.zero());
     HIP_TRY(c->dSplit2.alloc(L.numDry)); HIP_TRY(c->dSplit2.zero());
diff --git a/openal-soft_amd/csrc/api_context.hpp b/openal-soft_amd/csrc/api_context.hpp
--- a/openal-soft_amd/csrc/api_context.hpp
+++ b/openal-soft_amd/csrc/api_context.hpp
@@ -144,6 +144,7 @@
     BufferTable buf;
     DevBuf<VoiceCtl> ctl;
     DevBuf<float> prev, hrtfOld, hrtfTgt, hist, gainCur, gainTgt, sendCur, sendTgt;
+    DevBuf<uint32_t> hrtfSplit;
     DevBuf<BiquadSlot> dfilt, sfilt;
     DevBuf<float> partLines, partLines2, partHrtf, partHrtf2, bus, streams;
     DevBuf<uint32_t> lineGains;
diff --git a/openal-soft_amd/csrc/api_hrtf.hip b/openal-soft_amd/csrc/api_hrtf.hip
--- a/openal-soft_amd/csrc/api_hrtf.hip
+++ b/openal-soft_amd/csrc/api_hrtf.hip
@@ -51,6 +51,7 @@
         const size_t n = size_t{L.numVoices} * L.irStride * 2;
         HIP_TRY(c->hrtfOld.alloc(n)); HIP_TRY(c->hrtfOld.zero()); L.hrtfOld = c->hrtfOld.p;
         HIP_TRY(c->hrtfTgt.alloc(n)); HIP_TRY(c->hrtfTgt.zero()); L.hrtfTgt = c->hrtfTgt.p;
+        HIP_TRY(c->hrtfSplit.alloc(size_t{L.numVoices} * SplitVoiceDwords(L.irStride))); HIP_TRY(c->hrtfSplit.zero()); L.hrtfSplit = c->hrtfSplit.p;
         if(!c->directSet) c->dIrSize = h.irSize;
     }
     if(toStreamRows)
diff --git a/openal-soft_amd/csrc/api_voices.hip b/openal-soft_amd/csrc/api_voices.hip
--- a/openal-soft_amd/csrc/api_voices.hip
+++ b/openal-soft_amd/csrc/api_voices.hip
@@ -257,7 +257,7 @@
             b->mapVoices = uint32_t(map.size());
             if((c->res.enabled || (c->desc.flags & OALGPU_CTX_APPLY_IN_VOICE_KERNEL)) && c->L.hrtf && c->L.hrirs && c->L.irStride <= 64u)
             {
-                HIP_TRY(b->rows.alloc(count * size_t{c->L.irStride} * 2));
+                HIP_TRY(b->rows.alloc(count * size_t{BlendRowDwords(c->L.irStride)}));
                 HIP_TRY(b->rows.zero());
                 LaunchBlendRows(c->stream, c->L, b->recs.p, uint32_t(count), b->rows.p);
                 HIP_TRY(hipGetLastError());
diff --git a/openal-soft_amd/csrc/dev_wave.hpp b/openal-soft_amd/csrc/dev_wave.hpp
--- a/openal-soft_amd/csrc/dev_wave.hpp
+++ b/openal-soft_amd/csrc/dev_wave.hpp
@@ -27,6 +27,7 @@
     __builtin_amdgcn_fence(__ATOMIC_ACQUIRE, "wavefront");
 }
 
+typedef uint32_t u2 __attribute__((ext_vector_type(2)));
 typedef uint32_t u4 __attribute__((ext_vector_type(4)));
 typedef const u4 __attribute__((address_space(4))) cu4;
 
@@ -283,6 +284,14 @@
     const uint32_t ab = a > b ? a : b, cd = c > d ? c : d;
     return ab > cd ? ab : cd;
 }
+__device__ __forceinline__ uint32_t SplitResponse(float h, float &inv)
+{
+    float sh;
+    HalfScale(WaveMaxBits(__builtin_bit_cast(uint32_t, __builtin_fabsf(h))), sh, inv);
+    uint32_t hi, lo;
+    SplitHalf2(h * sh, 0.0f, hi, lo);
+    return (hi & 0xffffu) | (lo << 16);
+}
 
 constexpr int kBqSeg = 17;
 struct S2 { float a, b; };
diff --git a/openal-soft_amd/csrc/kernels.hpp b/openal-soft_amd/csrc/kernels.hpp
--- a/openal-soft_amd/csrc/kernels.hpp
+++ b/openal-soft_amd/csrc/kernels.hpp
@@ -94,6 +94,8 @@
     float *prev;
     BiquadSlot *dfilt;
     float *hrtfOld, *hrtfTgt, *hist;
+    uint32_t *hrtfSplit;
+    uint32_t restageResponses;
     float *gainCur, *gainTgt;
     BiquadSlot *sfilt;
     float *sendCur, *sendTgt;
@@ -113,6 +115,16 @@
     const float *hrirs;
 };
 
+constexpr uint32_t kSplitTarget = 1u, kSplitOld = 2u;
+__host__ __device__ inline uint32_t SplitVoiceDwords(uint32_t irStride) { return 4u * irStride + 8u; }
+__host__ __device__ inline uint32_t *SplitRows(uint32_t *split, uint32_t irStride, uint32_t v, uint32_t set)
+{ return split + size_t{v} * SplitVoiceDwords(irStride) + set * 2u * irStride; }
+__host__ __device__ inline float *SplitInv(uint32_t *split, uint32_t irStride, uint32_t v)
+{ return reinterpret_cast<float*>(split + size_t{v} * SplitVoiceDwords(irStride) + 4u * irStride); }
+__host__ __device__ inline uint32_t *SplitValid(uint32_t *split, uint32_t irStride, uint32_t v)
+{ return split + size_t{v} * SplitVoiceDwords(irStride) + 4u * irStride + 4u; }
+__host__ __device__ inline uint32_t BlendRowDwords(uint32_t irStride) { return 4u * irStride + 4u; }
+
 __host__ __device__ inline size_t BusWetOffset(const DeviceLayout &L) { return size_t{L.numDry + L.numReal} * kLine; }
 __host__ __device__ inline size_t BusAccumOffset(const DeviceLayout &L)
 { return BusWetOffset(L) + size_t{L.numSlots} * L.wetChannels * kLine; }
@@ -134,6 +146,7 @@
         x = L.hrirs[size_t{i3} * (kHrirLen * 2) + e] * w3 + x;
         __builtin_nontemporal_store((e < live) ? x : 0.0f, &L.hrtfTgt[size_t{v} * L.irStride * 2 + e]);
     }
+    if(lane == 0) *SplitValid(L.hrtfSplit, L.irStride, v) &= ~kSplitTarget;
 }
 
 __device__ __forceinline__ void ApplyRecordWave(const DeviceLayout &L, const ParamRecord &r, uint32_t lane)
diff --git a/openal-soft_amd/csrc/voice_kernel.hip b/openal-soft_amd/csrc/voice_kernel.hip
--- a/openal-soft_amd/csrc/voice_kernel.hip
+++ b/openal-soft_amd/csrc/voice_kernel.hip
@@ -1,5 +1,6 @@
 #include <hip/hip_ext.h>
 #include "kernels.hpp"
+#include "dev_wave.hpp"
 
 #pragma clang fp contract(off)
 
@@ -149,6 +150,7 @@
             L.hrtfOld[size_t{v} * L.irStride * 2 + k] = 0.0f;
             L.hrtfTgt[size_t{v} * L.irStride * 2 + k] = 0.0f;
         }
+        if(t == 0) *SplitValid(L.hrtfSplit, L.irStride, v) = 0u;
     }
     else if(t < L.numDry)
     {
@@ -176,6 +178,8 @@
     const uint32_t i0 = r.hrtfIdx[0], i1 = r.hrtfIdx[1], i2 = r.hrtfIdx[2], i3 = r.hrtfIdx[3];
     const float w0 = r.hrtfW[0], w1 = r.hrtfW[1], w2 = r.hrtfW[2], w3 = r.hrtfW[3];
     const uint32_t live = ((L.irSize + 1u) & ~1u) * 2u;
+    float *row = rows + size_t{blockIdx.x} * BlendRowDwords(L.irStride);
+    float x0 = 0.0f, x1 = 0.0f;
     for(uint32_t e = lane; e < L.irStride * 2; e += 64)
     {
         float x = (e < 2) ? r.hrtfPass : 0.0f;
@@ -183,8 +187,19 @@
         x = L.hrirs[size_t{i1} * (kHrirLen * 2) + e] * w1 + x;
         x = L.hrirs[size_t{i2} * (kHrirLen * 2) + e] * w2 + x;
         x = L.hrirs[size_t{i3} * (kHrirLen * 2) + e] * w3 + x;
-        rows[size_t{blockIdx.x} * L.irStride * 2 + e] = (e < live) ? x : 0.0f;
-    }
+        x = (e < live) ? x : 0.0f;
+        row[e] = x;
+        if(e < 64u) x0 = x; else if(e < 128u) x1 = x;
+    }
+    const int src = int((2u * lane) & 63u);
+    const float a0 = __shfl(x0, src), a1 = __shfl(x1, src), b0 = __shfl(x0, src + 1), b1 = __shfl(x1, src + 1);
+    const bool tap = lane < L.irStride;
+    const float hL = tap ? (lane < 32u ? a0 : a1) : 0.0f, hR = tap ? (lane < 32u ? b0 : b1) : 0.0f;
+    float inv0, inv1;
+    const uint32_t s0 = SplitResponse(hL, inv0), s1 = SplitResponse(hR, inv1);
+    uint32_t *split = reinterpret_cast<uint32_t*>(row) + L.irStride * 2;
+    if(tap) { split[2 * lane] = s0; split[2 * lane + 1] = s1; }
+    if(lane < 4) row[L.irStride * 4 + lane] = (lane == 0) ? inv0 : (lane == 1 ? inv1 : 0.0f);
 }
 void LaunchBlendRows(hipStream_t s, const DeviceLayout &L, const ParamRecord *recs, uint32_t count, float *rows)
 {
@@ -234,6 +249,7 @@
     const float *src = coeffs + size_t{blockIdx.x} * (kHrirLen * 2);
     for(uint32_t e = lane; e < L.irStride * 2; e += 64)
         L.hrtfTgt[size_t{v} * L.irStride * 2 + e] = (e < live) ? src[e] : 0.0f;
+    if(lane == 0) *SplitValid(L.hrtfSplit, L.irStride, v) &= ~kSplitTarget;
 }
 
 void LaunchApplyTargets(hipStream_t s, const DeviceLayout &L, const TargetRecord *recs, const float *coeffs, uint32_t count)
@@ -777,7 +793,7 @@
                     if(t == 0)
                     {
                         VoiceCtl &c = L.ctl[v];
-                        if(counter == 0 || fademix) { c.hrtfOldDelay[0] = dL; c.hrtfOldDelay[1] = dR; }
+                        if(counter == 0 || fademix) { c.hrtfOldDelay[0] = dL; c.hrtfOldDelay[1] = dR; *SplitValid(L.hrtfSplit, irStride, v) &= ~kSplitOld; }
                         c.hrtfOldGain = todo ? endGain : gainAfterBlend;
                     }
                     continue;
diff --git a/openal-soft_amd/csrc/voice_wave.hip b/openal-soft_amd/csrc/voice_wave.hip
--- a/openal-soft_amd/csrc/voice_wave.hip
+++ b/openal-soft_amd/csrc/voice_wave.hip
@@ -219,9 +219,11 @@
     uint32_t *startDelay, *queueDone;
     float *partHrtf;
     const float *hrirs;
+    uint32_t *hrtfSplit;
     explicit WaveArgsHrtf(const DeviceLayout &L) : numVoices{L.numVoices}, waveVoices{L.waveVoices}, irStride{L.irStride}, pad{L.irSize},
         tables{L.tables}, buffers{L.buffers}, ctl{L.ctl}, prev{L.prev}, dfilt{L.dfilt}, hrtfOld{L.hrtfOld}, hrtfTgt{L.hrtfTgt},
-        hist{L.hist}, ambi{L.ambi}, startDelay{L.startDelay}, queueDone{L.queueDone}, partHrtf{L.partHrtf}, hrirs{L.hrirs} { }
+        hist{L.hist}, ambi{L.ambi}, startDelay{L.startDelay}, queueDone{L.queueDone}, partHrtf{L.partHrtf}, hrirs{L.hrirs},
+        hrtfSplit{L.restageResponses ? nullptr : L.hrtfSplit} { }
 };
 
 struct NextBlock { const ParamRecord *recs; const int32_t *map; const float *rows; ResidentArgs res; };
@@ -284,6 +286,7 @@
             x = L.hrirs[size_t{i3} * (kHrirLen * 2) + e] * w3 + x;
             L.hrtfTgt[size_t{v} * L.irStride * 2 + e] = (e < live) ? x : 0.0f;
         }
+        if(lane == 0 && L.hrtfSplit) *SplitValid(L.hrtfSplit, L.irStride, v) &= ~kSplitTarget;
     }
 }
 __device__ __forceinline__ void ApplyNextRecord(const WaveArgsHrtf &L, const ParamRecord &r, uint32_t lane) { ApplyRecordLean(L, r, lane); }
@@ -313,18 +316,25 @@
     const uint32_t irStride = L.irStride;
     RecScalars sA{}, sB{};
     f2 rowA = {0.0f, 0.0f}, rowB = {0.0f, 0.0f};
-    uint32_t flA = 0u, flB = 0u;
+    u2 splA = {0u, 0u}, splB = {0u, 0u};
+    float invA = 0.0f, invB = 0.0f;
+    uint32_t flA = 0u, flB = 0u, vlA = 0u, vlB = 0u;
+    const uint32_t rowDw = BlendRowDwords(irStride);
     if(doA)
     {
         sA = LoadRecScalars(recs[riA]);
-        if(lane < irStride) rowA = reinterpret_cast<const f2*>(rows + size_t{uint32_t(riA)} * irStride * 2u)[lane];
-        if(lane == 0) flA = L.ctl[vA].flags;
+        const float *row = rows + size_t{uint32_t(riA)} * rowDw;
+        if(lane < irStride) { rowA = reinterpret_cast<const f2*>(row)[lane]; splA = reinterpret_cast<const u2*>(row + irStride * 2u)[lane]; }
+        if(lane < 2u) invA = row[irStride * 4u + lane];
+        if(lane == 0) { flA = L.ctl[vA].flags; if(L.hrtfSplit) vlA = *SplitValid(L.hrtfSplit, irStride, vA); }
     }
     if(doB)
     {
         sB = LoadRecScalars(recs[riB]);
-        if(lane < irStride) rowB = reinterpret_cast<const f2*>(rows + size_t{uint32_t(riB)} * irStride * 2u)[lane];
-        if(lane == 0) flB = L.ctl[vB].flags;
+        const float *row = rows + size_t{uint32_t(riB)} * rowDw;
+        if(lane < irStride) { rowB = reinterpret_cast<const f2*>(row)[lane]; splB = reinterpret_cast<const u2*>(row + irStride * 2u)[lane]; }
+        if(lane < 2u) invB = row[irStride * 4u + lane];
+        if(lane == 0) { flB = L.ctl[vB].flags; if(L.hrtfSplit) vlB = *SplitValid(L.hrtfSplit, irStride, vB); }
     }
     const bool fLane = lane >= 1u && lane <= 4u;
     const bool fB = lane >= 3u, fHp = ((lane - 1u) & 1u) != 0u;
@@ -333,7 +343,7 @@
     float tb0 = 0.0f, tb1 = 0.0f, tb2 = 0.0f, ta1 = 0.0f, ta2 = 0.0f;
     int32_t fcounter = 0;
     if(fOn) { tb0 = fp->tb0; tb1 = fp->tb1; tb2 = fp->tb2; ta1 = fp->ta1; ta2 = fp->ta2; fcounter = fp->counter; }
-    auto installCtl = [&](uint32_t v, const RecScalars &r, uint32_t flagsOld, f2 row)
+    auto installCtl = [&](uint32_t v, const RecScalars &r, uint32_t flagsOld, f2 row, u2 spl, float inv, uint32_t validOld)
     {
         VoiceCtl &ctl = L.ctl[v];
         if(lane == 0)
@@ -352,10 +362,19 @@
                 ctl.hrtfTgtGain = r.gain;
             }
         }
-        if(!r.keepHrtf && lane < irStride) reinterpret_cast<f2*>(L.hrtfTgt + size_t{v} * irStride * 2u)[lane] = row;
+        if(!r.keepHrtf)
+        {
+            if(lane < irStride) reinterpret_cast<f2*>(L.hrtfTgt + size_t{v} * irStride * 2u)[lane] = row;
+            if(L.hrtfSplit)
+            {
+                if(lane < irStride) reinterpret_cast<u2*>(SplitRows(L.hrtfSplit, irStride, v, 0u))[lane] = spl;
+                if(lane < 2u) SplitInv(L.hrtfSplit, irStride, v)[lane] = inv;
+                if(lane == 0) *SplitValid(L.hrtfSplit, irStride, v) = validOld | kSplitTarget;
+            }
+        }
     };
-    if(doA) installCtl(vA, sA, flA, rowA);
-    if(doB) installCtl(vB, sB, flB, rowB);
+    if(doA) installCtl(vA, sA, flA, rowA, splA, invA, vlA);
+    if(doB) installCtl(vB, sB, flB, rowB, splB, invB, vlB);
     if(fOn)
     {
         float c[5];
@@ -1224,6 +1243,7 @@
                 const float *tg = L.hrtfTgt + size_t{v} * irStride * 2;
                 float *od = L.hrtfOld + size_t{v} * irStride * 2;
                 for(uint32_t k = lane; k < irStride * 2; k += 64) od[k] = tg[k];
+                if(L.hrtfSplit && lane == 0) *SplitValid(L.hrtfSplit, irStride, v) &= ~kSplitOld;
             }
             if(lane == 0)
             {
diff --git a/openal-soft_amd/csrc/voice_wave16.hip b/openal-soft_amd/csrc/voice_wave16.hip
--- a/openal-soft_amd/csrc/voice_wave16.hip
+++ b/openal-soft_amd/csrc/voice_wave16.hip
@@ -160,18 +160,20 @@
 __device__ __forceinline__ float W16ReadLaneF(float v, int l)
 { return __builtin_bit_cast(float, __builtin_amdgcn_readlane(__builtin_bit_cast(int, v), l)); }
 
-__device__ __forceinline__ float W16StageResponse(uint32_t (&hr)[2][kHrDw], float h, uint32_t lane)
-{
-    float sh, inv;
-    HalfScale(WaveMaxBits(__builtin_bit_cast(uint32_t, __builtin_fabsf(h))), sh, inv);
-    uint32_t hi, lo;
-    SplitHalf2(h * sh, 0.0f, hi, lo);
+__device__ __forceinline__ void W16StageResponse(uint32_t (&hr)[2][kHrDw], uint32_t s, uint32_t lane)
+{
     uint32_t *hz32 = &hr[0][0];
     for(uint32_t k = lane; k < uint32_t(2 * kHrDw); k += 64) hz32[k] = 0u;
     uint16_t *hz = reinterpret_cast<uint16_t*>(&hr[0][0]);
     const uint32_t u = 80u - lane;
-    hz[0 * kHrHalves + u] = uint16_t(hi); hz[1 * kHrHalves + u] = uint16_t(lo);
-    return __builtin_bit_cast(float, __builtin_amdgcn_readfirstlane(__builtin_bit_cast(int, inv)));
+    hz[0 * kHrHalves + u] = uint16_t(s); hz[1 * kHrHalves + u] = uint16_t(s >> 16);
+}
+__device__ __forceinline__ void W16SplitRow(u2 &row, float &invs, uint32_t at, uint32_t lane)
+{
+    const f2 h = __builtin_bit_cast(f2, row);
+    float i0, i1;
+    row.x = SplitResponse(h.x, i0); row.y = SplitResponse(h.y, i1);
+    invs = lane == at ? i0 : (lane == at + 1u ? i1 : invs);
 }
 
 __device__ __forceinline__ uint32_t W16VoiceOf(uint32_t group, uint32_t wave, uint32_t waves)
@@ -313,6 +315,8 @@
     const VoiceHead head = LoadHeadScalar(L.ctl + v);
     const BufferItem buf = LoadCtlBufferScalar(L.ctl + v);
     const VoiceTail tail = LoadTailScalar(L.ctl + v);
+    constexpr uint32_t kSplitRestage = 1u << 31;
+    const uint32_t splitKept = L.hrtfSplit ? *(cu32*)(uintptr_t)SplitValid(L.hrtfSplit, irStride, v) : kSplitRestage;
     asm volatile("" ::: "memory");
     const VoiceHead headK = LoadHeadScalar(L.ctl + (keyVoice < L.numVoices ? keyVoice : lastVoice));
     asm volatile("" ::: "memory");
@@ -449,7 +453,8 @@
     uint32_t counter = 0, fademix = 0, todo = 0;
     float endGain = 0.0f, gainAfterBlend = 0.0f;
     float fstv = 0.0f, histv = 0.0f;
-    f2 hT = {0.0f, 0.0f};
+    u2 rT = {0u, 0u};
+    float invs = 0.0f;
     int32_t bufferItem = head.curBuffer;
     if constexpr (SENDS)
     {
@@ -493,7 +498,12 @@
         __builtin_amdgcn_s_setprio(1);
         fstv = (lane < 32u) ? reinterpret_cast<const float*>(L.dfilt + size_t{v} * 2)[lane] : 0.0f;
         histv = L.hist[size_t{v} * kHist + lane];
-        hT = (lane < irStride) ? reinterpret_cast<const f2*>(L.hrtfTgt + size_t{v} * irStride * 2)[lane] : f2{0.0f, 0.0f};
+        {
+            const u2 *kept = reinterpret_cast<const u2*>(SplitRows(L.hrtfSplit, irStride, v, 0u));
+            const u2 *fp32 = reinterpret_cast<const u2*>(L.hrtfTgt + size_t{v} * irStride * 2);
+            if(lane < irStride) rT = ((splitKept & kSplitTarget) ? kept : fp32)[lane];
+            if(!(splitKept & kSplitRestage) && lane < 4u) invs = SplitInv(L.hrtfSplit, irStride, v)[lane];
+        }
         WaveSync();
 
         auto toLine = [&]()
@@ -699,7 +709,13 @@
         const float oldStep = fademix ? oldGain / float(fademix) : 0.0f;
         const bool merged = !dirty;
         const bool oldPass = !merged && oldOn;
-        const f2 hO = (oldPass && lane < irStride) ? reinterpret_cast<const f2*>(L.hrtfOld + size_t{v} * irStride * 2)[lane] : f2{0.0f, 0.0f};
+        u2 rO = {0u, 0u};
+        if(oldPass && lane < irStride)
+        {
+            const u2 *kept = reinterpret_cast<const u2*>(SplitRows(L.hrtfSplit, irStride, v, 1u));
+            const u2 *fp32 = reinterpret_cast<const u2*>(L.hrtfOld + size_t{v} * irStride * 2);
+            rO = ((splitKept & kSplitOld) ? kept : fp32)[lane];
+        }
         const float gbase = gainAfterBlend - mainStep * float(fademix);
         auto gainAt = [&](uint32_t i, bool mayFade)
         {
@@ -764,6 +780,16 @@
             }
         };
 
+        if(!(splitKept & kSplitTarget))
+        {
+            W16SplitRow(rT, invs, 0u, lane);
+            if(!(splitKept & kSplitRestage))
+            {
+                if(lane < irStride) reinterpret_cast<u2*>(SplitRows(L.hrtfSplit, irStride, v, 0u))[lane] = rT;
+                if(lane < 2u) SplitInv(L.hrtfSplit, irStride, v)[lane] = invs;
+            }
+        }
+        if(oldPass && !(splitKept & kSplitOld)) W16SplitRow(rO, invs, 2u, lane);
 #pragma unroll
         for(int e = 0; e < 2; ++e)
         {
@@ -771,7 +797,8 @@
             if(N == uint32_t(kLine)) buildEar(d, std::true_type{}); else buildEar(d, std::false_type{});
             uint16_t *xz = reinterpret_cast<uint16_t*>(&w.b.xh[0][0]);
             if(e == 0) stamp2(1);
-            const float invH = W16StageResponse(w.b.hr, e == 0 ? hT.x : hT.y, lane);
+            W16StageResponse(w.b.hr, e == 0 ? rT.x : rT.y, lane);
+            const float invH = W16ReadLaneF(invs, e);
             WaveSync();
             if(e == 0) stamp2(2);
             FirMfmaEar<5, false>(accM[e], w.b.xh, w.b.hr, invX * invH, lane);
@@ -789,7 +816,8 @@
                 WaveSync();
                 xz[0 * kXhHalves + 64u + lane] = uint16_t(hi); xz[1 * kXhHalves + 64u + lane] = uint16_t(lo);
                 if(lane < 40u) { w.b.xh[0][64u + lane] = 0u; w.b.xh[1][64u + lane] = 0u; }
-                const float invHO = W16StageResponse(w.b.hro, e == 0 ? hO.x : hO.y, lane);
+                W16StageResponse(w.b.hro, e == 0 ? rO.x : rO.y, lane);
+                const float invHO = W16ReadLaneF(invs, 2 + e);
                 WaveSync();
                 FirMfmaEar<1, true>(accM[e], w.b.xh, w.b.hro, invXo * invHO, lane);
             }
@@ -798,12 +826,22 @@
         }
     }
 
+    f2 hCopy = {0.0f, 0.0f};
+    uint32_t copyTaps = 0u;
     if(active)
     {
         if(dirty && (counter == 0 || fademix))
         {
-            if(lane < irStride) reinterpret_cast<f2*>(L.hrtfOld + size_t{v} * irStride * 2)[lane] = hT;
-        }
+            copyTaps = irStride;
+            if(lane < irStride) hCopy = reinterpret_cast<const f2*>(L.hrtfTgt + size_t{v} * irStride * 2)[lane];
+            if(!(splitKept & kSplitRestage))
+            {
+                if(lane < irStride) reinterpret_cast<u2*>(SplitRows(L.hrtfSplit, irStride, v, 1u))[lane] = rT;
+                if(lane < 2u) SplitInv(L.hrtfSplit, irStride, v)[2u + lane] = invs;
+            }
+        }
+        const uint32_t splitNow = splitKept | kSplitTarget | (copyTaps ? kSplitOld : 0u);
+        if(!(splitKept & kSplitRestage) && splitNow != splitKept && lane == 0) *SplitValid(L.hrtfSplit, irStride, v) = splitNow;
         if(lane == 0)
         {
             VoiceCtl &c = L.ctl[v];
@@ -897,6 +935,7 @@
             else StorePartial(&ph[k], s);
         }
     }
+    if(lane < copyTaps) reinterpret_cast<f2*>(L.hrtfOld + size_t{v} * irStride * 2)[lane] = hCopy;
     stamp(6);
     if constexpr (!RES) break;
     else
diff --git a/openal-soft_amd/oalgpu/__init__.py b/openal-soft_amd/oalgpu/__init__.py
--- a/openal-soft_amd/oalgpu/__init__.py
+++ b/openal-soft_amd/oalgpu/__init__.py
@@ -78,6 +78,7 @@
 CTX_SLICE_LINES = 128
 CTX_WAVE_PAIRS = 256
 CTX_ROW_SLICES = 512
+CTX_RESTAGE_RESPONSES = 1024
 
 
 class VoiceDesc(C.Structure):
```

New measurement: 109.8 million. 0.967x the previous value.
